# multicom-toolbox/Chromosome3D

Hardware: AMD Instinct MI355X
Metric: SA-steps/sec (replica-steps/s, 20 replicas of chr1_500kb in all: 20 per GPU, weak scaling; regions of 20 steps inside the first 2172 of the schedule's 5172: MD and FIRE steps in front of the final minimisation); wall-clock per chromosome (higher is better)
Workload: dtype f32

## Files before the change

chromosome3d_amd/csrc/c3d_api.cpp:

```cpp
#include <hip/hip_runtime.h>

#include <algorithm>
#include <atomic>
#include <cmath>
#include <cstdio>
#include <cstdlib>
#include <chrono>
#include <cstring>
#include <condition_variable>
#include <map>
#include <mutex>
#include <string>
#include <thread>
#include <tuple>
#include <vector>

#include "../../include/c3d.h"
#include "c3d_host.h"
#include "c3d_internal.h"

using c3d::fail;

namespace {

#define HIP_TRY(expr)                                                                          \
    do {                                                                                       \
        hipError_t e__ = (expr);                                                               \
        if (e__ != hipSuccess)                                                                 \
            return fail(C3D_ERR_HIP, std::string(#expr) + ": " + hipGetErrorString(e__));      \
    } while (0)

template <class T>
struct DevTmp {
    T* p = nullptr;
    ~DevTmp() { if (p) (void)hipFree(p); }
};

struct Op {
    c3d::DevStep p;
    int stage;
    bool counted;
};

struct KernelRecord {
    enum Family { NONE, STEP, LBFGS_EVAL, PAIRS_SYM, STEP64, LBFGS_EVAL64, CLUSTER } family = NONE;
    c3d::StepForm step{};
    c3d::Form64 f64{};
    int pot = 0, rpw = 0, nb = 0, wl = 0;
    bool rs1 = false, late = false, tp = false;
};

inline void philox4x32(const uint32_t ctr_in[4], const uint32_t key_in[2], uint32_t out[4]) {
    uint32_t c[4] = {ctr_in[0], ctr_in[1], ctr_in[2], ctr_in[3]};
    uint32_t k[2] = {key_in[0], key_in[1]};
    for (int r = 0; r < 10; ++r) {
        const uint64_t p0 = (uint64_t)0xD2511F53u * c[0];
        const uint64_t p1 = (uint64_t)0xCD9E8D57u * c[2];
        const uint32_t n0 = (uint32_t)(p1 >> 32) ^ c[1] ^ k[0];
        const uint32_t n1 = (uint32_t)p1;
        const uint32_t n2 = (uint32_t)(p0 >> 32) ^ c[3] ^ k[1];
        const uint32_t n3 = (uint32_t)p0;
        c[0] = n0; c[1] = n1; c[2] = n2; c[3] = n3;
        k[0] += 0x9E3779B9u;
        k[1] += 0xBB67AE85u;
    }
    memcpy(out, c, sizeof(c));
}
inline double u01(uint32_t u) { return ((double)u + 0.5) * (1.0 / 4294967296.0); }
void normals4(uint64_t seed, uint32_t replica, uint32_t bead, uint32_t purpose, double g[4]) {
    const uint32_t ctr[4] = {bead, purpose, 0u, 0u};
    const uint32_t key[2] = {(uint32_t)(seed & 0xFFFFFFFFu) ^ (replica * 0x9E3779B9u), (uint32_t)(seed >> 32) + replica};
    uint32_t r[4];
    philox4x32(ctr, key, r);
    const double two_pi = 6.283185307179586476925286766559;
    double a = sqrt(-2.0 * log(u01(r[0]))), b = two_pi * u01(r[1]);
    g[0] = a * cos(b); g[1] = a * sin(b);
    a = sqrt(-2.0 * log(u01(r[2]))); b = two_pi * u01(r[3]);
    g[2] = a * cos(b); g[3] = a * sin(b);
}

}

struct c3d_ctx {
    int device = 0;
    hipStream_t stream = nullptr;
    static constexpr int kMaxGroups = 4;
    int ngroups = 2;
    hipStream_t gstream[kMaxGroups] = {nullptr, nullptr, nullptr, nullptr};
    hipEvent_t gev[kMaxGroups] = {nullptr, nullptr, nullptr, nullptr};
    hipEvent_t fork_ev = nullptr;
    hipEvent_t ev0 = nullptr, ev1 = nullptr;
    hipEvent_t kev0 = nullptr, kev1 = nullptr;
    int kernel_timing = 0;
    double last_kernel_ms = 0;
    double last_host_launch_us = 0, last_host_sync_us = 0;
    int event_timing = 1;
    bool ev1_recorded = false;

    int n = 0, npad = 0, ntiles = 0, nrep = 0, R = 0;
    c3d_model model;
    std::vector<c3d_stage> stages;
    c3d_fire_params fire;
    float gtol = 0.0f;
    int check_every = 250;
    bool narrow_columns = true;
    bool zero_weight = false;
    bool use_graph = true;
    int rpw = 2;
    int stage_dma = 1;
    int graph_chunk = 256;
    int precision = 32;
    c3d::Buffers64 b64;
    int sym = 0;
    float* d_sym_scratch = nullptr;
    int2* d_sym_tiles = nullptr;
    int start_mode = 0;
    int resident = -1;
    int resident_min_ops = 4;
    double spin_wait_us = 400.0;
    long spin_completions = 0;

    std::vector<int32_t> h_dist10;
    c3d::DevBuffers buf{};
    int eval_rpw = 4;
    bool pair_targets = true;
    bool wide_tiles = true;
    int max_beads = 5120;
    int embed_max_beads = C3D_EMBED_MAX_BEADS_DEFAULT;
    int embed_form = 0;
    int embed_batch = 0;
    int last_embed_form = 0, last_embed_batches = 0;
    int f64_max_beads = C3D_F64_MAX_BEADS_DEFAULT;
    int f64_column_chunk = 0;
    std::vector<int32_t> r_i, r_j, r_t10;
    int column_chunk = 0;
    float* d_feval = nullptr;
    size_t rep_floats = 0;
    bool have_targets = false, have_replicas = false;

    std::vector<Op> program;
    size_t pc = 0;
    int parity = 0;
    long steps_done = 0;
    std::map<std::tuple<long, int, int, int>, hipGraphExec_t> graphs;

    bool inject_timeout = false;
    int resident_fallbacks = 0;
    int resident_skip = 0;
    int resident_backoff = 0;
    int num_cus = 0, num_xcc = 0;
    int cluster_late = -1;
    int cluster_geom = 0;
    int xcd_base = 0, xcd_count = 8;
    bool inject_misplaced = false;
    bool static_place = true;
    int placement_mismatches = 0;
    bool inject_incomplete = false;
    int cluster_incomplete = 0;

    int cluster = -1;
    bool cl_ok = false;
    c3d::ClusterPlan cl_plan{};
    void* d_crec = nullptr;
    size_t crec_bytes = 0;
    static constexpr unsigned kClaimSets = 4096;
    static constexpr unsigned kClaimWords = 16;
    unsigned* d_claim = nullptr;
    unsigned cl_seq = 0;
    c3d::StepRun* d_prog = nullptr;
    size_t prog_cap = 0;
    bool prog_dirty = true;
    std::vector<int> op_run, op_skip;
    std::vector<c3d::StepRun> prog_runs;
    unsigned* h_tmo = nullptr;
    void* h_stage = nullptr;
    void* d_score = nullptr;
    size_t d_score_bytes = 0;
    size_t h_stage_bytes = 0;
    struct IfRanks {
        std::thread worker;
        std::vector<double> matrix, rank;
        size_t m = 0;
        double mean = 0, saa = 0;
        int n = 0, range = 0;
        bool valid = false;
        void join() { if (worker.joinable()) worker.join(); }
        void release() {
            join();
            valid = false;
            std::vector<double>().swap(matrix);
            std::vector<double>().swap(rank);
        }
    } ifr;
    int bb_steps = 1000;
    bool final_bb = true;
    int prefetch_ranks = 1;
    unsigned* h_tmo_dev = nullptr;

    long rank_prefetch_hits = 0;
    int device_ranks = 0;
    long device_rank_runs = 0, score_wide_runs = 0;
    long compare_runs = 0;
    long f64_evals = 0;
    long superpose_runs = 0, rmsd_table_runs = 0;
    long k1_recomputed = 0, k1_patched = 0;
    long graph_captures = 0, graph_launches = 0, step_launches = 0, resident_launches = 0, cluster_launches = 0;
    bool has_two_point = false;
    bool has_lbfgs = false;
    int lbfgs_mem = 5;
    c3d::LbfgsBuffers lb{};
    bool f64_lbfgs = false;
    c3d::LbfgsBuffers64 lb64{};
    long lbfgs_steps = 0;
    int lbfgs_parity = -1;
    int last_path = 0;
    KernelRecord ran;

    double last_ms = 0;
    long last_steps = 0, last_launches = 0;
    uint64_t seed = 82364;
    uint32_t first_rep = 0;
};

namespace {

template <class T>
void dev_free(T*& p) {
    if (!p) return;
    const hipError_t e = hipFree(p);
    if (e != hipSuccess) (void)fail(C3D_ERR_HIP, std::string("hipFree: ") + hipGetErrorString(e));
    p = nullptr;
}

void free_replica_buffers(c3d_ctx* c) {
    for (int k = 0; k < 2; ++k) {
        dev_free(c->buf.X[k]); dev_free(c->buf.V[k]); dev_free(c->buf.P[k]); dev_free(c->buf.S[k]);
    }
    dev_free(c->d_crec);
    c->crec_bytes = 0; c->cl_ok = false;
    dev_free(c->buf.Vinit); dev_free(c->buf.E); dev_free(c->d_feval);
    dev_free(c->d_sym_scratch); dev_free(c->d_sym_tiles);
    dev_free(c->lb.hist); dev_free(c->lb.part); dev_free(c->lb.S[0]); dev_free(c->lb.S[1]);
    dev_free(c->lb64.hist); dev_free(c->lb64.part); dev_free(c->lb64.S[0]); dev_free(c->lb64.S[1]);
    c->lbfgs_parity = -1;
    dev_free(c->b64.T); dev_free(c->b64.t10); dev_free(c->b64.Vinit); dev_free(c->b64.F);
    for (int k = 0; k < 2; ++k) { dev_free(c->b64.X[k]); dev_free(c->b64.V[k]); dev_free(c->b64.P[k]); dev_free(c->b64.S[k]); }
    c->have_replicas = false;
}
void drop_graphs(c3d_ctx* c) {
    for (auto& kv : c->graphs) (void)hipGraphExecDestroy(kv.second);
    c->graphs.clear();
}
void release_context(c3d_ctx* c) {
    for (hipStream_t s : c->gstream) if (s) (void)hipStreamSynchronize(s);
    drop_graphs(c);
    free_replica_buffers(c);
    dev_free(c->buf.tgt); dev_free(c->buf.tgs2);
    dev_free(c->d_prog); dev_free(c->d_claim); dev_free(c->d_score);
    if (c->h_tmo) (void)hipHostFree(c->h_tmo);
    if (c->h_stage) (void)hipHostFree(c->h_stage);
    for (hipEvent_t e : {c->ev0, c->ev1, c->kev0, c->kev1, c->fork_ev}) if (e) (void)hipEventDestroy(e);
    for (hipEvent_t e : c->gev) if (e) (void)hipEventDestroy(e);
    for (hipStream_t s : c->gstream) if (s && s != c->stream) (void)hipStreamDestroy(s);
    if (c->stream) (void)hipStreamDestroy(c->stream);
}

c3d::DevModel dev_model(const c3d_ctx* c) {
    c3d::DevModel m{};
    const c3d_model& h = c->model;
    m.n = c->n; m.npad = c->npad; m.ntiles = c->ntiles; m.nrep = c->nrep;
    m.rep_base = 0; m.nrep_g = c->nrep;
    m.rpw = c->rpw;
    m.stage_dma = c->stage_dma;
    m.noe_pot = h.noe_pot; m.ang_mode = h.ang_mode; m.rep_sep = h.rep_sep;
    m.mexp = h.msoexp == 2 ? 2 : 1;
    m.rs = h.rswitch;
    m.tail_c = h.asym * h.rswitch;
    m.tail_b = (m.tail_c - 2.0f * h.rswitch) * h.rswitch * h.rswitch;
    m.mrs = h.mrswitch; m.nmrs = -h.mrswitch;
    m.inv_rs = 1.0f / h.rswitch; m.nm_rs = -h.mrswitch / h.rswitch;
    if (h.noe_pot == 3 && h.msoexp == 2 && h.masym == 0.0f && m.tail_b == 0.0f && m.tail_c == 2.0f * m.rs) {
        m.noe_pot = 4;
        m.inv_rs = 1.0f / h.mrswitch; m.nm_rs = h.rswitch / h.mrswitch;
    }
    {
        const int cols_last = c->n - (c->npad - 256);
        int wl = cols_last / 64, nleft = cols_last - 64 * wl;
        if (wl == 0 || nleft > 8) { wl = std::min(4, wl + 1); nleft = 0; }
        if (!c->narrow_columns || c->npad > 1024) { wl = 4; nleft = 0; }
        m.wl = wl; m.nleft = nleft; m.jl0 = c->npad - 256 + 64 * wl;
    }
    m.mtail_c = h.masym;
    m.mtail_b = (m.mtail_c - 2.0f * h.mrswitch) * h.mrswitch * h.mrswitch * (m.mexp == 2 ? h.mrswitch : 1.0f);
    m.k_bond2 = 2.0f * h.k_bond; m.b0 = h.b0;
    m.k_ang2 = 2.0f * h.k_ang; m.a0 = h.a0;
    m.acc = c3d::kAccel / h.mass;
    const int ndf = std::max(3 * c->n - 3, 1);
    m.t_fac = h.mass / c3d::kAccel / ((float)ndf * c3d::kBoltz);
    m.fbeta = h.fbeta;
    m.inv_n = 1.0f / (float)c->n;
    return m;
}
c3d::DevFire dev_fire(const c3d_ctx* c) {
    c3d::DevFire f;
    f.dt_start = c->fire.dt_start; f.dt_max = c->fire.dt_max; f.f_inc = c->fire.f_inc; f.f_dec = c->fire.f_dec;
    f.alpha_start = c->fire.alpha_start; f.f_alpha = c->fire.f_alpha; f.max_step = c->fire.max_step;
    f.n_min = c->fire.n_min;
    return f;
}
float clamp_scale(const c3d_ctx* c) { return dev_model(c).noe_pot == 4 ? c->model.mrswitch : c->model.rswitch; }
c3d::DevStep dev_step(const c3d_ctx* c, int kind, float dt, float w_all, float w_vdw, float repel_s, float t_bath) {
    c3d::DevStep p;
    p.kind = kind; p.dt = dt; p.w_all = w_all;
    p.w_noe2n = -2.0f * w_all * c->model.s_noe;
    p.w_rep4 = 4.0f * w_vdw * c->model.k_rep;
    const float rr = repel_s * c->model.r0_rep;
    p.rep_r2 = rr * rr;
    p.inv_rep_r2 = rr > 0.0f ? 1.0f / p.rep_r2 : 0.0f;
    p.w_rep4r2 = p.w_rep4 * p.rep_r2;
    p.w_rs = p.w_noe2n * clamp_scale(c);
    p.kq = p.w_rs != 0.0f ? p.w_rep4r2 / p.w_rs : 0.0f;
    p.t_bath = t_bath;
    return p;
}

bool is_two_point(int kind) { return kind == 5 || kind == 6; }
bool is_lbfgs(int kind) { return kind == 8 || kind == 9; }

void build_program(c3d_ctx* c) {
    c->program.clear();
    int prev_kind = -1;
    for (size_t s = 0; s < c->stages.size(); ++s) {
        const c3d_stage& st = c->stages[s];
        if (st.kind == 2 || st.kind == 5 || st.kind == 8) {
            const bool lbfgs = st.kind == 8;
            const int nbb = (st.kind == 5 && c->final_bb) || lbfgs ? std::min(st.nsteps, c->bb_steps) : 0;
            for (int k = 0; k < st.nsteps; ++k) {
                const int kind = k < nbb ? (k == 0 ? (lbfgs ? 9 : 6) : (lbfgs ? 8 : 5)) : (k == nbb ? 3 : 2);
                c->program.push_back({dev_step(c, kind, 0.0f, st.w_all, st.w_vdw, st.repel_s, 0.0f), (int)s, true});
            }
        } else {
            if (prev_kind == 2 || prev_kind == 5 || prev_kind == 8 || prev_kind == -1)
                c->program.push_back({dev_step(c, 4, 0.0f, st.w_all, st.w_vdw, st.repel_s, st.t_bath), (int)s, false});
            for (int k = 0; k < st.nsteps; ++k)
                c->program.push_back({dev_step(c, st.kind, st.dt, st.w_all, st.w_vdw, st.repel_s, st.t_bath), (int)s, true});
        }
        prev_kind = st.kind;
    }
    c->pc = 0;
    c->zero_weight = false;
    for (const Op& op : c->program) c->zero_weight = c->zero_weight || op.p.w_rs == 0.0f;
    c->has_two_point = false;
    for (const Op& op : c->program) c->has_two_point = c->has_two_point || is_two_point(op.p.kind);
    c->has_lbfgs = false;
    for (const Op& op : c->program) c->has_lbfgs = c->has_lbfgs || is_lbfgs(op.p.kind);
    drop_graphs(c);
    c->prog_runs.clear();
    c->op_run.assign(c->program.size(), 0);
    c->op_skip.assign(c->program.size(), 0);
    for (size_t k = 0; k < c->program.size(); ++k) {
        const c3d::DevStep& p = c->program[k].p;
        if (!c->prog_runs.empty() && memcmp(&c->prog_runs.back().p, &p, sizeof(p)) == 0) ++c->prog_runs.back().count;
        else c->prog_runs.push_back({p, 1});
        c->op_run[k] = (int)c->prog_runs.size() - 1;
        c->op_skip[k] = c->prog_runs.back().count - 1;
    }
    c->prog_dirty = true;
}

enum Stale : unsigned { STALE_REPLICAS = 1, STALE_GRAPHS = 2, STALE_PAIR_TARGETS = 4, STALE_PROGRAM = 8 };
void drop_stale(c3d_ctx* c, unsigned stale) {
    if (stale & STALE_REPLICAS) free_replica_buffers(c);
    if (stale & STALE_PAIR_TARGETS) dev_free(c->buf.tgs2);
    if (stale & STALE_PROGRAM) build_program(c);
    else if (stale & STALE_GRAPHS) drop_graphs(c);
}

int upload_targets(c3d_ctx* c, const std::vector<float>& enc) {
    dev_free(c->buf.tgt); dev_free(c->buf.tgs2);
    HIP_TRY(hipMalloc(&c->buf.tgt, sizeof(float) * enc.size()));
    HIP_TRY(hipMemcpyAsync(c->buf.tgt, enc.data(), sizeof(float) * enc.size(), hipMemcpyHostToDevice, c->stream));
    HIP_TRY(hipStreamSynchronize(c->stream));
    return C3D_OK;
}

void set_dims(c3d_ctx* c, int n) {
    c->n = n;
    c->npad = (n + 255) / 256 * 256;
    c->ntiles = (n + c3d::kTileRows - 1) / c3d::kTileRows;
    c->rep_floats = (size_t)3 * c->npad;
}

void pack(const c3d_ctx* c, const float* aos, std::vector<float>& soa, bool pad_far) {
    soa.assign(c->rep_floats * c->nrep, 0.0f);
    for (int r = 0; r < c->nrep; ++r) {
        float* base = soa.data() + c->rep_floats * r;
        for (int comp = 0; comp < 3; ++comp) {
            for (int i = 0; i < c->n; ++i) base[(size_t)comp * c->npad + i] = aos[((size_t)r * c->n + i) * 3 + comp];
            if (pad_far)
                for (int i = c->n; i < c->npad; ++i) base[(size_t)comp * c->npad + i] = c3d::kPadCoord * (float)(comp + 1) + 16.0f * (float)(i - c->n);
        }
    }
}
void unpack(const c3d_ctx* c, const float* soa, float* aos) {
    for (int r = 0; r < c->nrep; ++r) {
        const float* base = soa + c->rep_floats * r;
        for (int comp = 0; comp < 3; ++comp)
            for (int i = 0; i < c->n; ++i) aos[((size_t)r * c->n + i) * 3 + comp] = base[(size_t)comp * c->npad + i];
    }
}

void group_range(const c3d_ctx* c, int g, int& base, int& count) {
    const int G = std::min(c->ngroups, std::max(c->nrep, 1));
    const int q = c->nrep / G, r = c->nrep % G;
    base = g * q + std::min(g, r);
    count = q + (g < r ? 1 : 0);
}
int active_groups(const c3d_ctx* c) { return std::min(c->ngroups, std::max(c->nrep, 1)); }

enum Unit : unsigned {
    UNIT_DEVICE = 0, UNIT_SCORE, UNIT_CLUSTER_BASE, UNIT_EMBED, UNIT_F64, UNIT_SYM,
    UNIT_CLUSTER_P0, UNIT_CLUSTER_TP0 = UNIT_CLUSTER_P0 + 5, UNIT_COUNT = UNIT_CLUSTER_TP0 + 5
};
constexpr unsigned unit_bit(unsigned u) { return 1u << u; }
constexpr unsigned kUnitsDefault = unit_bit(UNIT_DEVICE) | unit_bit(UNIT_SCORE) | unit_bit(UNIT_CLUSTER_P0 + 4) | unit_bit(UNIT_CLUSTER_TP0 + 4);
constexpr unsigned kUnitsAll = (1u << UNIT_COUNT) - 1u;
constexpr int kMaxDevices = 64;
class LaunchGate {
    std::mutex mu;
    std::condition_variable cv;
    int launching = 0, loads_waiting = 0;
    bool loading = false;
public:
    void lock_shared() {
        std::unique_lock<std::mutex> lk(mu);
        cv.wait(lk, [&] { return !loading && loads_waiting == 0; });
        ++launching;
    }
    void unlock_shared() {
        std::lock_guard<std::mutex> lk(mu);
        if (--launching == 0) cv.notify_all();
    }
    void lock() {
        std::unique_lock<std::mutex> lk(mu);
        ++loads_waiting;
        cv.wait(lk, [&] { return !loading && launching == 0; });
        --loads_waiting;
        loading = true;
    }
    void unlock() {
        std::lock_guard<std::mutex> lk(mu);
        loading = false;
        cv.notify_all();
    }
};
struct Units {
    LaunchGate rw;
    std::atomic<unsigned> loaded[kMaxDevices];
    std::atomic<long> loads{0};
    Units() { for (auto& a : loaded) a.store(0); }
};
Units g_units;
thread_local int t_entry_depth = 0;

const char* unit_name(unsigned u) {
    static const char* const names[] = {"per-step + K1", "scoring", "multi-step planner", "embedding", "fp64", "symmetric tiles"};
    if (u < UNIT_CLUSTER_P0) return names[u];
    return u < UNIT_CLUSTER_TP0 ? "multi-step (k_cluster)" : "multi-step (k_cluster_tp)";
}
hipError_t load_one_unit(unsigned u) {
    switch (u) {
        case UNIT_DEVICE: return c3d::preload_device_unit();
        case UNIT_SCORE: return c3d::preload_score_unit();
        case UNIT_CLUSTER_BASE: return c3d::preload_cluster_base_unit();
        case UNIT_EMBED: return c3d::preload_embed_unit();
        case UNIT_F64: return c3d::preload_f64_unit();
        case UNIT_SYM: return c3d::preload_sym_unit();
        default: break;
    }
    if (u >= UNIT_CLUSTER_TP0 && u < UNIT_COUNT) return c3d::preload_cluster_unit((int)(u - UNIT_CLUSTER_TP0), true);
    if (u >= UNIT_CLUSTER_P0 && u < UNIT_CLUSTER_TP0) return c3d::preload_cluster_unit((int)(u - UNIT_CLUSTER_P0), false);
    return hipErrorInvalidValue;
}
int ensure_units(int device, unsigned mask) {
    if (device < 0 || device >= kMaxDevices) return fail(C3D_ERR_INVALID, "device index beyond the 64 this build keeps code-object state for");
    mask &= kUnitsAll;
    if ((g_units.loaded[device].load(std::memory_order_acquire) & mask) == mask) return C3D_OK;
    if (t_entry_depth > 0) return fail(C3D_ERR_HIP, "internal: a code object is wanted inside an entry that did not name it");
    std::lock_guard<LaunchGate> lk(g_units.rw);
    HIP_TRY(hipSetDevice(device));
    for (unsigned u = 0; u < UNIT_COUNT; ++u) {
        if (!(mask & unit_bit(u)) || (g_units.loaded[device].load(std::memory_order_relaxed) & unit_bit(u))) continue;
        const hipError_t e = load_one_unit(u);
        if (e != hipSuccess) return fail(C3D_ERR_HIP, std::string("loading the code object of the ") + unit_name(u) + " kernels: " + hipGetErrorString(e));
        g_units.loaded[device].fetch_or(unit_bit(u), std::memory_order_release);
        g_units.loads.fetch_add(1);
    }
    return C3D_OK;
}
unsigned units_wanted(const c3d_ctx* c) {
    unsigned m = unit_bit(UNIT_DEVICE) | unit_bit(UNIT_SCORE);
    const int pot = std::min(std::max(dev_model(c).noe_pot, 0), 4);
    if (c->cluster != 0 && c->resident != 0 && c->precision != 64)
        m |= unit_bit(UNIT_CLUSTER_P0 + (unsigned)pot) | unit_bit(UNIT_CLUSTER_TP0 + (unsigned)pot);
    if (c->precision == 64) m |= unit_bit(UNIT_F64);
    if (c->sym > 0) m |= unit_bit(UNIT_SYM);
    return m;
}
struct Entry {
    int rc = C3D_OK;
    bool locked = false;
    Entry(const c3d_ctx* c, unsigned extra, bool launches) {
        if (hipSetDevice(c->device) != hipSuccess) { rc = fail(C3D_ERR_HIP, "hipSetDevice failed"); return; }
        if (launches) rc = ensure_units(c->device, units_wanted(c) | extra);
        if (rc != C3D_OK) return;
        if (t_entry_depth++ == 0) { g_units.rw.lock_shared(); locked = true; }
    }
    ~Entry() {
        if (rc != C3D_OK) return;
        --t_entry_depth;
        if (locked) g_units.rw.unlock_shared();
    }
    Entry(const Entry&) = delete;
    Entry& operator=(const Entry&) = delete;
};
#define C3D_ENTRY(c, extra)                 \
    Entry entry__((c), (extra), true);      \
    if (entry__.rc != C3D_OK) return entry__.rc
#define C3D_GATE(c)                         \
    Entry entry__((c), 0u, false);          \
    if (entry__.rc != C3D_OK) return entry__.rc

int drop_stale_gated(c3d_ctx* c, unsigned stale) {
    const bool device_side = ((stale & STALE_REPLICAS) && (c->buf.X[0] || c->b64.t10)) || ((stale & STALE_PAIR_TARGETS) && c->buf.tgs2) ||
                             ((stale & (STALE_GRAPHS | STALE_PROGRAM)) && !c->graphs.empty());
    if (!device_side) { drop_stale(c, stale); return C3D_OK; }
    C3D_GATE(c);
    drop_stale(c, stale);
    return C3D_OK;
}

bool use_sym(const c3d_ctx* c) {
    return c->sym > 0 && c->d_sym_scratch && !c3d::general_tail(dev_model(c));
}

void model_host64(const c3d_ctx* c, double (&mh)[15]) {
    const c3d_model& h = c->model;
    const double v[15] = {h.s_noe, h.rswitch, h.asym, h.masym, h.mrswitch, h.k_bond, h.b0, h.k_ang, h.a0, h.r0_rep, h.k_rep, h.mass, h.fbeta,
                          (double)h.min_sep, (double)h.msoexp};
    for (int k = 0; k < 15; ++k) mh[k] = v[k];
}
int build_targets64(c3d_ctx* c) {
    double mh[15];
    model_host64(c, mh);
    hipError_t e = c3d::launch_targets64(dev_model(c), mh, c->model.min_sep, c->b64.t10, c->b64.T, c->stream);
    if (e != hipSuccess) return fail(C3D_ERR_HIP, std::string("fp64 targets: ") + hipGetErrorString(e));
    HIP_TRY(hipStreamSynchronize(c->stream));
    return C3D_OK;
}


int ensure_lbfgs(c3d_ctx* c) {
    if (c->lb.hist) return C3D_OK;
    const size_t hist = c3d::lbfgs_hist_floats(c->npad) * c->nrep, part = (size_t)c->nrep * c->ntiles * c3d::kLbfgsQ;
    HIP_TRY(hipMalloc(&c->lb.hist, sizeof(float) * hist));
    HIP_TRY(hipMalloc(&c->lb.part, sizeof(float) * part));
    for (int k = 0; k < 2; ++k) HIP_TRY(hipMalloc(&c->lb.S[k], sizeof(c3d::LbfgsState) * c->nrep));
    HIP_TRY(hipMemsetAsync(c->lb.hist, 0, sizeof(float) * hist, c->stream));
    HIP_TRY(hipMemsetAsync(c->lb.part, 0, sizeof(float) * part, c->stream));
    for (int k = 0; k < 2; ++k) HIP_TRY(hipMemsetAsync(c->lb.S[k], 0, sizeof(c3d::LbfgsState) * c->nrep, c->stream));
    HIP_TRY(hipStreamSynchronize(c->stream));
    return C3D_OK;
}

int ensure_lbfgs64(c3d_ctx* c) {
    if (c->lb64.hist) return C3D_OK;
    const size_t hist = c3d::lbfgs_hist_floats(c3d::cols64(c->n)) * c->nrep, part = (size_t)c->nrep * c->ntiles * c3d::kLbfgsQ;
    HIP_TRY(hipMalloc(&c->lb64.hist, sizeof(double) * hist));
    HIP_TRY(hipMalloc(&c->lb64.part, sizeof(double) * part));
    for (int k = 0; k < 2; ++k) HIP_TRY(hipMalloc(&c->lb64.S[k], sizeof(c3d::LbfgsState) * c->nrep));
    HIP_TRY(hipMemsetAsync(c->lb64.hist, 0, sizeof(double) * hist, c->stream));
    HIP_TRY(hipMemsetAsync(c->lb64.part, 0, sizeof(double) * part, c->stream));
    for (int k = 0; k < 2; ++k) HIP_TRY(hipMemsetAsync(c->lb64.S[k], 0, sizeof(c3d::LbfgsState) * c->nrep, c->stream));
    HIP_TRY(hipStreamSynchronize(c->stream));
    return C3D_OK;
}

int ensure_pair_targets(c3d_ctx* c, const c3d::DevModel& m) {
    if (c->buf.tgs2 || !c->pair_targets || !c3d::pair_targets_fit(m) || c->npad <= 1024 || !c->buf.tgt) return C3D_OK;
    HIP_TRY(hipMalloc(&c->buf.tgs2, sizeof(float) * c3d::pair_targets_floats(c->n, c->npad)));
    hipError_t e = c3d::launch_pair_targets(m, c->buf.tgt, c->buf.tgs2, c->stream);
    if (e != hipSuccess) return fail(C3D_ERR_HIP, std::string("pair targets: ") + hipGetErrorString(e));
    HIP_TRY(hipStreamSynchronize(c->stream));
    return C3D_OK;
}
KernelRecord op_kernel(const c3d_ctx* c, const c3d::DevModel& m, const Op& op) {
    KernelRecord k;
    if (c->precision == 64) {
        double mh[15];
        model_host64(c, mh);
        k.family = is_lbfgs(op.p.kind) ? KernelRecord::LBFGS_EVAL64 : KernelRecord::STEP64;
        k.f64 = c3d::form64(m.noe_pot, mh, c->stages[op.stage].w_all, c->n, c->f64_column_chunk);
    } else if (!is_lbfgs(op.p.kind) && use_sym(c)) {
        k.family = KernelRecord::PAIRS_SYM;
        k.pot = c3d::device_pot(m.noe_pot);
        k.rs1 = c3d::sym_rs1(m);
    } else {
        k.family = is_lbfgs(op.p.kind) ? KernelRecord::LBFGS_EVAL : KernelRecord::STEP;
        k.step = c3d::step_form(m, op.p, c->wide_tiles, c->pair_targets, c->buf.tgs2 != nullptr, c->column_chunk);
    }
    return k;
}
int launch_op(c3d_ctx* c, const Op& op, int g, int par) {
    c3d::DevModel m = dev_model(c);
    group_range(c, g, m.rep_base, m.nrep_g);
    if (c->precision == 64) {
        const c3d_stage& st = c->stages[op.stage];
        double mh[15];
        model_host64(c, mh);
        const double fh[7] = {c->fire.dt_start, c->fire.dt_max, c->fire.f_inc, c->fire.f_dec, c->fire.alpha_start, c->fire.f_alpha, c->fire.max_step};
        const double sh[6] = {(double)op.p.kind, st.dt, st.w_all, st.w_vdw, st.repel_s, st.t_bath};
        if (is_lbfgs(op.p.kind)) {
            hipError_t e = c3d::launch_lbfgs_eval64(m, mh, sh, c->b64, c->lb64, par, c->lbfgs_mem, c->f64_column_chunk, c->gstream[g]);
            if (e == hipSuccess) e = c3d::launch_lbfgs_move64(m, mh, sh, fh, c->fire.n_min, c->b64, c->lb64, par, c->lbfgs_mem, c->gstream[g]);
            if (e != hipSuccess) return fail(C3D_ERR_HIP, std::string("fp64 L-BFGS step launch: ") + hipGetErrorString(e));
            return C3D_OK;
        }
        hipError_t e64 = c3d::launch_step64(m, mh, sh, fh, c->fire.n_min, c->b64, par, c->f64_column_chunk, c->gstream[g]);
        if (e64 != hipSuccess) return fail(C3D_ERR_HIP, std::string("fp64 step launch: ") + hipGetErrorString(e64));
        return C3D_OK;
    }
    const KernelRecord k = op_kernel(c, m, op);
    if (k.family == KernelRecord::LBFGS_EVAL) {
        hipError_t e = c3d::launch_lbfgs_eval(m, op.p, c->buf, c->lb, par, c->lbfgs_mem, k.step, c->gstream[g]);
        if (e == hipSuccess) e = c3d::launch_lbfgs_move(m, op.p, dev_fire(c), c->buf, c->lb, par, c->lbfgs_mem, c->gstream[g]);
        if (e != hipSuccess) return fail(C3D_ERR_HIP, std::string("L-BFGS step launch: ") + hipGetErrorString(e));
        return C3D_OK;
    }
    hipError_t e = k.family == KernelRecord::PAIRS_SYM
                       ? c3d::launch_step_sym(m, op.p, dev_fire(c), c->buf, par, c->d_sym_tiles, c->d_sym_scratch, c->gstream[g])
                       : c3d::launch_step(m, op.p, dev_fire(c), c->buf, par, k.step, c->gstream[g]);
    if (e != hipSuccess) return fail(C3D_ERR_HIP, std::string("step launch: ") + hipGetErrorString(e));
    return C3D_OK;
}

int plan_cluster(c3d_ctx* c) {
    c3d::DevModel m = dev_model(c);
    m.nrep = c->nrep; m.nrep_g = c->nrep; m.rep_base = 0;
    c->cl_ok = false;
    if (!c3d::cluster_plan(m, c->num_cus, c->num_xcc, c->cluster_geom, c->cluster_late, c->xcd_count, &c->cl_plan)) return C3D_OK;
    c->cl_plan.device = c->device;
    const size_t bytes = c3d::cluster_record_bytes(m, c->cl_plan);
    if (!c->d_crec || bytes > c->crec_bytes) {
        if (c->d_crec) { HIP_TRY(hipStreamSynchronize(c->stream)); dev_free(c->d_crec); }
        c->crec_bytes = 0;
        HIP_TRY(hipMalloc(&c->d_crec, bytes));
        c->crec_bytes = bytes;
    }
    c->cl_seq = 0;
    c->cl_ok = true;
    return C3D_OK;
}

bool cluster_ok(c3d_ctx* c) {
    if (!c->resident || !c->cluster || !c->cl_ok || !c->d_crec) return false;
    return !c3d::general_tail(dev_model(c));
}

bool launch_was_abandoned(c3d_ctx* c, unsigned done_mark) {
    if (c->h_tmo[2]) { c->h_tmo[2] = 0; c->static_place = false; ++c->placement_mismatches; }
    const bool complete = c->h_tmo[1] == done_mark;
    if (!*c->h_tmo && complete) { c->resident_backoff = 0; return false; }
    if (!*c->h_tmo) ++c->cluster_incomplete;
    *c->h_tmo = 0;
    c->resident_backoff = std::min(4096, std::max(4, 2 * c->resident_backoff));
    c->resident_skip = c->resident_backoff;
    ++c->resident_fallbacks;
    return true;
}
void account_ops(c3d_ctx* c, size_t nops) {
    c->parity ^= 1;
    for (size_t k = 0; k < nops; ++k)
        if (c->program[c->pc + k].counted) { ++c->steps_done; ++c->last_steps; }
    c->last_launches += 1;
    c->pc += nops;
}


int run_cluster(c3d_ctx* c, size_t nops, bool* ran) {
    if (c->prog_dirty) {
        if (c->prog_runs.size() > c->prog_cap) {
            if (c->d_prog) { HIP_TRY(hipStreamSynchronize(c->stream)); dev_free(c->d_prog); }
            c->prog_cap = std::max<size_t>(c->prog_runs.size(), 256);
            HIP_TRY(hipMalloc(&c->d_prog, sizeof(c3d::StepRun) * c->prog_cap));
        }
        HIP_TRY(hipMemcpyAsync(c->d_prog, c->prog_runs.data(), sizeof(c3d::StepRun) * c->prog_runs.size(), hipMemcpyHostToDevice, c->stream));
        HIP_TRY(hipStreamSynchronize(c->stream));
        c->prog_dirty = false;
    }
    const unsigned seq = c->cl_seq % c3d_ctx::kClaimSets;
    if (seq == 0) {
        HIP_TRY(hipMemsetAsync(c->d_crec, 0, c->crec_bytes, c->stream));
        HIP_TRY(hipMemsetAsync(c->d_claim, 0, sizeof(unsigned) * c3d_ctx::kClaimWords * c3d_ctx::kClaimSets, c->stream));
    }
    ++c->cl_seq;
    if (c->inject_timeout) { *c->h_tmo = 1; c->inject_timeout = false; }
    c->h_tmo[1] = 0;
    const c3d::DevModel m = dev_model(c);
    c3d::ClusterPlan pl = c->cl_plan;
    if (c->inject_incomplete) { ++pl.expected; c->inject_incomplete = false; }
    if (c->kernel_timing) { pl.t0 = c->kev0; pl.t1 = c->kev1; }
    pl.static_place = c->static_place ? (c->inject_misplaced ? 2 : 1) : 0;
    pl.xcd_base = c->xcd_base;
    pl.two_point = false;
    for (size_t k = 0; k < nops && !pl.two_point; ++k) pl.two_point = is_two_point(c->program[c->pc + k].p.kind);
    c->inject_misplaced = false;
    c->h_tmo[2] = 0;
    const auto h0 = std::chrono::steady_clock::now();
    hipError_t e = c3d::launch_cluster(m, dev_fire(c), pl, c3d::anneal_io(c->buf, c->parity), c->buf.tgt, c->d_crec, c->d_prog,
                                       c->op_run[c->pc], c->op_skip[c->pc], (int)nops, seq << 20, c->h_tmo_dev,
                                       c->d_claim + c3d_ctx::kClaimWords * seq, c->stream);
    if (e != hipSuccess) return fail(C3D_ERR_HIP, std::string("cluster launch: ") + hipGetErrorString(e));
    if (c->event_timing) HIP_TRY(hipEventRecord(c->ev1, c->stream));
    const auto h1 = std::chrono::steady_clock::now();
    bool marked = false;
    if (c->spin_wait_us > 0 && !c->kernel_timing) {
        const unsigned mark = (seq << 20) | 1u;
        for (;;) {
            if (__atomic_load_n(&c->h_tmo[1], __ATOMIC_ACQUIRE) == mark) { marked = true; break; }
            if (__atomic_load_n(&c->h_tmo[0], __ATOMIC_RELAXED) || __atomic_load_n(&c->h_tmo[2], __ATOMIC_RELAXED)) break;
            if (std::chrono::duration<double, std::micro>(std::chrono::steady_clock::now() - h1).count() > c->spin_wait_us) break;
            __builtin_ia32_pause();
        }
    }
    if (!marked) HIP_TRY(hipStreamSynchronize(c->stream));
    else ++c->spin_completions;
    const auto h2 = std::chrono::steady_clock::now();
    c->last_host_launch_us += std::chrono::duration<double, std::micro>(h1 - h0).count();
    c->last_host_sync_us += std::chrono::duration<double, std::micro>(h2 - h1).count();
    c->ev1_recorded = true;
    ++c->cluster_launches;
    if (c->kernel_timing) {
        float kms = 0;
        HIP_TRY(hipEventElapsedTime(&kms, c->kev0, c->kev1));
        c->last_kernel_ms += kms;
    }
    if (launch_was_abandoned(c, (seq << 20) | 1u)) { *ran = false; c->ev1_recorded = false; return C3D_OK; }
    *ran = true;
    c->last_path = 2;
    KernelRecord& k = c->ran;
    k = KernelRecord();
    k.family = KernelRecord::CLUSTER;
    k.pot = c3d::device_pot(m.noe_pot); k.rpw = pl.rpw; k.nb = m.npad / 256; k.wl = m.wl; k.late = pl.late_tiles != 0; k.tp = pl.two_point;
    account_ops(c, nops);
    return C3D_OK;
}

int run_ops_segment(c3d_ctx* c, size_t nops, bool zero_w, bool lbfgs = false);

int run_ops(c3d_ctx* c, size_t nops) {
    const bool p64 = c->precision == 64;
    if (p64 ? !c->has_lbfgs : (!c->zero_weight && !c->has_two_point && !c->has_lbfgs)) return run_ops_segment(c, nops, false);
    const size_t end = c->pc + nops;
    while (c->pc < end) {
        const c3d::DevStep& p0 = c->program[c->pc].p;
        const bool z = !p64 && p0.w_rs == 0.0f, tp = !p64 && is_two_point(p0.kind), lb = is_lbfgs(p0.kind);
        size_t k = 1;
        while (c->pc + k < end) {
            const c3d::DevStep& p = c->program[c->pc + k].p;
            if ((!p64 && p.w_rs == 0.0f) != z || (!p64 && is_two_point(p.kind)) != tp || is_lbfgs(p.kind) != lb) break;
            ++k;
        }
        const int rc = run_ops_segment(c, k, z, lb);
        if (rc) return rc;
    }
    return C3D_OK;
}

int ensure_group_streams(c3d_ctx* c, int G) {
    for (int g = 1; g < G && g < c3d_ctx::kMaxGroups; ++g) {
        if (c->gstream[g]) continue;
        HIP_TRY(hipStreamCreateWithFlags(&c->gstream[g], hipStreamNonBlocking));
        HIP_TRY(hipEventCreateWithFlags(&c->gev[g], hipEventDisableTiming));
    }
    return C3D_OK;
}

int run_ops_segment(c3d_ctx* c, size_t nops, bool zero_w, bool lbfgs) {
    if (nops == 0) return C3D_OK;
    if (c->precision == 64 || zero_w || lbfgs) { }
    else if (c->resident_skip > 0 && c->resident < 1) --c->resident_skip;
    else if (nops >= (size_t)c->resident_min_ops && nops < ((size_t)1 << 20)) {
        bool ran = false;
        int rc = C3D_OK;
        if (cluster_ok(c)) rc = run_cluster(c, nops, &ran);
        if (rc != C3D_OK || ran) return rc;
    }
    c->last_path = 0;
    c->ev1_recorded = false;
    if (c->precision != 64 && (!use_sym(c) || lbfgs)) {
        if (int rc = ensure_pair_targets(c, dev_model(c))) return rc;
    }
    if (lbfgs)
        if (int rc = c->precision == 64 ? ensure_lbfgs64(c) : ensure_lbfgs(c)) return rc;
    const int G = active_groups(c);
    if (int rc = ensure_group_streams(c, G)) return rc;
    if (G > 1) {
        HIP_TRY(hipEventRecord(c->fork_ev, c->stream));
        for (int g = 1; g < G; ++g) HIP_TRY(hipStreamWaitEvent(c->gstream[g], c->fork_ev, 0));
    }
    size_t done = 0;
    while (done < nops) {
        const size_t chunk = std::min<size_t>(nops - done, c->use_graph ? (size_t)c->graph_chunk : nops - done);
        if (!c->use_graph || chunk < 4) {
            for (int g = 0; g < G; ++g) {
                int par = c->parity;
                for (size_t k = 0; k < chunk; ++k) {
                    int rc = launch_op(c, c->program[c->pc + k], g, par);
                    if (rc) return rc;
                    par ^= 1;
                }
            }
        } else {
            const Op& first = c->program[c->pc];
            const Op& last = c->program[c->pc + chunk - 1];
            long sig = (long)c->pc;
            if ((first.p.kind == 2 || first.p.kind == 5 || first.p.kind == 8) && last.p.kind == first.p.kind && first.stage == last.stage)
                sig = -(long)(first.stage + 1) - (first.p.kind == 5 ? 1000000L : first.p.kind == 8 ? 2000000L : 0L);
            if (c->graphs.size() >= 2048) {
                for (int g = 0; g < G; ++g) HIP_TRY(hipStreamSynchronize(c->gstream[g]));
                drop_graphs(c);
            }
            for (int g = 0; g < G; ++g) {
                const auto key = std::make_tuple(sig, (int)chunk, c->parity, g);
                auto it = c->graphs.find(key);
                if (it == c->graphs.end()) {
                    hipGraph_t gr = nullptr;
                    HIP_TRY(hipStreamBeginCapture(c->gstream[g], hipStreamCaptureModeThreadLocal));
                    int par = c->parity;
                    int rc = C3D_OK;
                    for (size_t k = 0; k < chunk && rc == C3D_OK; ++k) { rc = launch_op(c, c->program[c->pc + k], g, par); par ^= 1; }
                    hipError_t ce = hipStreamEndCapture(c->gstream[g], &gr);
                    if (rc) { if (gr) (void)hipGraphDestroy(gr); return rc; }
                    if (ce != hipSuccess) return fail(C3D_ERR_HIP, std::string("hipStreamEndCapture: ") + hipGetErrorString(ce));
                    hipGraphExec_t ge = nullptr;
                    hipError_t ie = hipGraphInstantiate(&ge, gr, nullptr, nullptr, 0);
                    (void)hipGraphDestroy(gr);
                    if (ie != hipSuccess) return fail(C3D_ERR_HIP, std::string("hipGraphInstantiate: ") + hipGetErrorString(ie));
                    it = c->graphs.emplace(key, ge).first;
                    ++c->graph_captures;
                }
                HIP_TRY(hipGraphLaunch(it->second, c->gstream[g]));
                ++c->graph_launches;
            }
        }
        c->step_launches += (long)chunk * G;
        if (lbfgs) { c->lbfgs_steps += (long)chunk; c->lbfgs_parity = c->parity ^ (int)(chunk & 1); }
        if (chunk & 1) c->parity ^= 1;
        for (size_t k = 0; k < chunk; ++k)
            if (c->program[c->pc + k].counted) { ++c->steps_done; ++c->last_steps; }
        c->last_launches += (long)chunk;
        c->pc += chunk;
        done += chunk;
    }
    for (int g = 1; g < G; ++g) {
        HIP_TRY(hipEventRecord(c->gev[g], c->gstream[g]));
        HIP_TRY(hipStreamWaitEvent(c->stream, c->gev[g], 0));
    }
    if (c->precision == 64) {
        hipError_t e = c3d::launch_export64(dev_model(c), c->b64, c->parity, c->buf.X[c->parity], c->buf.V[c->parity], c->buf.P[c->parity], c->stream);
        if (e != hipSuccess) return fail(C3D_ERR_HIP, std::string("fp64 export: ") + hipGetErrorString(e));
        c->last_path = 3;
// ... 42 lines not shown
    const float* h = static_cast<const float*>(c->h_stage);
    double worst = 0;
    for (int r = 0; r < c->nrep; ++r) {
        double ff = 0;
        for (int t = 0; t < nparts; ++t) ff += h[((size_t)r * nparts + t) * 4 + 1];
        const double rms = sqrt(ff / (3.0 * c->n));
        if (!(rms <= worst)) worst = rms;
    }
    *out = worst;
    return C3D_OK;
}

int partials_finite(c3d_ctx* c, bool* ok) {
    const size_t cnt = (size_t)c->nrep * c->ntiles * 4;
    if (int rc = read_back(c, c->buf.P[c->parity], sizeof(float) * cnt)) return rc;
    const float* h = static_cast<const float*>(c->h_stage);
    *ok = true;
    for (size_t k = 0; k < cnt; ++k) if (!std::isfinite(h[k])) { *ok = false; break; }
    return C3D_OK;
}

int import64(c3d_ctx* c) {
    hipError_t e = c3d::launch_import64(dev_model(c), c->buf.X[c->parity], c->b64, c->stream);
    if (e != hipSuccess) return fail(C3D_ERR_HIP, std::string("fp64 import: ") + hipGetErrorString(e));
    HIP_TRY(hipStreamSynchronize(c->stream));
    return C3D_OK;
}

}

extern "C" int c3d_device_count(void) {
    int n = 0;
    if (hipGetDeviceCount(&n) != hipSuccess) return 0;
    return n;
}

extern "C" void c3d_default_model(c3d_model* m) {
    if (!m) return;
    m->min_sep = 5; m->noe_pot = 3; m->rep_sep = 2; m->ang_mode = 1;
    m->s_noe = 10.0f; m->rswitch = 0.5f; m->asym = 2.0f;
    m->k_bond = 500.0f; m->b0 = 3.93f;
    m->k_ang = 15.0f; m->a0 = 5.55f;
    m->r0_rep = 5.25f; m->k_rep = 4.0f;
    m->mass = 100.0f; m->fbeta = 10.0f;
    m->mrswitch = 10.0f; m->masym = 0.0f; m->msoexp = 2;
}
extern "C" void c3d_default_fire(c3d_fire_params* f) {
    if (!f) return;
    f->dt_start = 0.002f; f->dt_max = 0.02f; f->f_inc = 1.1f; f->f_dec = 0.5f;
    f->alpha_start = 0.1f; f->f_alpha = 0.99f; f->max_step = 0.5f; f->n_min = 5;
}
extern "C" int c3d_default_schedule(c3d_stage* st, int cap, int min_steps) {
    std::vector<c3d_stage> v;
    v.push_back({2, 200, 0.0f, 1.0f, 20.0f, 0.5f, 0.0f});
    const float hot_t = 2000.0f, hot_dt = 0.003f;
    const int hot_n[5] = {125, 125, 125, 500, 125};
    const float hot_w[5] = {0.1f, 0.2f, 0.2f, 0.4f, 1.0f};
    const float hot_v[5] = {20.0f, 20.0f, 0.01f, 0.003f, 0.003f};
    const float hot_r[5] = {0.5f, 0.5f, 0.9f, 0.9f, 0.9f};
    for (int k = 0; k < 5; ++k) v.push_back({0, hot_n[k], hot_dt, hot_w[k], hot_v[k], hot_r[k], hot_t});
    const int ncycle = (int)(hot_t / 25.0f);
    const int nstep = 1000 / ncycle;
    const double vdw_step = pow(4.0 / 0.003, 1.0 / ncycle);
    const double rad_step = (1.0 - 0.85) / ncycle;
    double radius = 1.0, kv = 0.003, bath = hot_t;
    for (int i = 0; i <= ncycle; ++i) {
        v.push_back({1, nstep, 0.005f, 1.0f, (float)kv, (float)radius, (float)bath});
        radius = std::max(0.85, radius - rad_step);
        kv = std::min(4.0, kv * vdw_step);
        bath -= 25.0;
    }
    v.push_back({5, min_steps, 0.0f, 1.0f, 1.0f, 0.85f, 0.0f});
    if (st) for (int k = 0; k < (int)v.size() && k < cap; ++k) st[k] = v[k];
    return (int)v.size();
}

static std::atomic<int> g_preload{1};

extern "C" int c3d_set_process_option(const char* key, double value) {
    if (!key) return fail(C3D_ERR_INVALID, "c3d_set_process_option: null key");
    if (!strcmp(key, "preload")) {
        if (value != 0 && value != 1 && value != 2) return fail(C3D_ERR_INVALID, "c3d_set_process_option: preload is 0, 1 or 2");
        g_preload.store((int)value);
        return C3D_OK;
    }
    return fail(C3D_ERR_INVALID, std::string("c3d_set_process_option: unknown key ") + key);
}

extern "C" int c3d_create(int device, c3d_ctx** out) {
    if (!out) return fail(C3D_ERR_INVALID, "c3d_create: null out");
    int ndev = 0;
    if (hipGetDeviceCount(&ndev) != hipSuccess || ndev < 1)
        return fail(C3D_ERR_NO_DEVICE, "no HIP device visible: libc3d has no CPU fallback");
    if (device < 0 || device >= ndev) return fail(C3D_ERR_INVALID, "c3d_create: device index out of range");
    HIP_TRY(hipSetDevice(device));
    hipDeviceProp_t prop;
    HIP_TRY(hipGetDeviceProperties(&prop, device));
    if (strncmp(prop.gcnArchName, "gfx950", 6) != 0)
        return fail(C3D_ERR_NO_DEVICE, std::string("device is ") + prop.gcnArchName + ", libc3d is built for gfx950 only");
    int num_xcc = 0;
    if (hipDeviceGetAttribute(&num_xcc, hipDeviceAttributeNumberOfXccs, device) != hipSuccess) num_xcc = 0;
    if (const int pre = g_preload.load())
        if (const int rc = ensure_units(device, pre >= 2 ? kUnitsAll : kUnitsDefault)) return rc;
    c3d_ctx* c = new c3d_ctx();
    c->device = device;
    c->num_cus = prop.multiProcessorCount;
    c->num_xcc = num_xcc;
    c3d_default_model(&c->model);
    c3d_default_fire(&c->fire);
    c->stages.resize(c3d_default_schedule(nullptr, 0, 3000));
    c3d_default_schedule(c->stages.data(), (int)c->stages.size(), 3000);
    Entry gate(c, 0u, false);
    if (gate.rc != C3D_OK) { delete c; return gate.rc; }
    bool ok = hipStreamCreateWithFlags(&c->stream, hipStreamNonBlocking) == hipSuccess &&
              hipEventCreate(&c->ev0) == hipSuccess && hipEventCreate(&c->ev1) == hipSuccess &&
              hipEventCreate(&c->kev0) == hipSuccess && hipEventCreate(&c->kev1) == hipSuccess &&
              hipEventCreateWithFlags(&c->fork_ev, hipEventDisableTiming) == hipSuccess;
    c->gstream[0] = c->stream;
    ok = ok && hipHostMalloc(reinterpret_cast<void**>(&c->h_tmo), 64, hipHostMallocMapped) == hipSuccess;
    if (ok) {
        *c->h_tmo = 0;
        ok = hipHostGetDevicePointer(reinterpret_cast<void**>(&c->h_tmo_dev), c->h_tmo, 0) == hipSuccess &&
             hipMalloc(&c->d_claim, sizeof(unsigned) * c3d_ctx::kClaimWords * c3d_ctx::kClaimSets) == hipSuccess;
        c->h_tmo[1] = 0;
    }
    if (!ok) {
        c3d_destroy(c);
        return fail(C3D_ERR_HIP, "cannot create HIP stream/events");
    }
    *out = c;
    return C3D_OK;
}

extern "C" void c3d_destroy(c3d_ctx* c) {
    if (!c) return;
    c->ifr.release();
    {
        Entry gate(c, 0u, false);
        release_context(c);
    }
    delete c;
}

extern "C" int c3d_set_model(c3d_ctx* c, const c3d_model* m) {
    if (!c || !m) return fail(C3D_ERR_INVALID, "c3d_set_model: null argument");
    const int msoexp = m->msoexp == 0 ? 2 : m->msoexp;
    if (m->mass <= 0 || m->rswitch <= 0 || m->min_sep < 1 || m->rep_sep < 1 || m->rep_sep > 3 || m->noe_pot < 0 || m->noe_pot > 3 || m->mrswitch <= 0 || (msoexp != 1 && msoexp != 2))
        return fail(C3D_ERR_INVALID, "c3d_set_model: parameter out of range");
    if (c->have_targets && m->min_sep != c->model.min_sep)
        return fail(C3D_ERR_INVALID, "c3d_set_model: min_sep must be set before the targets are built");
    const bool targets64 = c->precision == 64 && c->b64.T;
    Entry entry(c, 0u, targets64);
    if (entry.rc != C3D_OK) return entry.rc;
    c->model = *m;
    c->model.msoexp = msoexp;
    drop_stale(c, STALE_PAIR_TARGETS | STALE_PROGRAM);
    if (c->have_replicas)
        if (int rc = plan_cluster(c)) return rc;
    return targets64 ? build_targets64(c) : C3D_OK;
}

extern "C" int c3d_set_schedule(c3d_ctx* c, const c3d_stage* st, int n_stages, const c3d_fire_params* fire, float gtol,
                                int check_every) {
    if (!c || !st || n_stages < 1) return fail(C3D_ERR_INVALID, "c3d_set_schedule: bad arguments");
    for (int k = 0; k < n_stages; ++k) {
        if (st[k].kind < 0 || (st[k].kind > 2 && st[k].kind != 5 && st[k].kind != 8) || st[k].nsteps < 0) return fail(C3D_ERR_INVALID, "c3d_set_schedule: bad stage");
        if (st[k].kind == 8 && c->precision == 64 && !c->f64_lbfgs)
            return fail(C3D_ERR_INVALID, "c3d_set_schedule: a stage of kind 8 (L-BFGS) has no fp64 form; set precision 32 first");
    }
    c->stages.assign(st, st + n_stages);
    if (fire) c->fire = *fire;
    c->gtol = gtol;
    if (check_every > 0) c->check_every = check_every;
    return drop_stale_gated(c, STALE_PROGRAM);
}

extern "C" int c3d_set_option(c3d_ctx* c, const char* key, double value) {
    if (!c || !key) return fail(C3D_ERR_INVALID, "c3d_set_option: null argument");
    unsigned stale = 0;
    if (!strcmp(key, "use_graph")) c->use_graph = value != 0;
    else if (!strcmp(key, "rows_per_wave")) {
        if (value != 1 && value != 2 && value != 4) return fail(C3D_ERR_INVALID, "rows_per_wave must be 1, 2 or 4");
        c->rpw = (int)value;
        stale = STALE_GRAPHS;
    } else if (!strcmp(key, "replica_groups")) {
        if (value < 1 || value > c3d_ctx::kMaxGroups) return fail(C3D_ERR_INVALID, "replica_groups must be 1..4");
        c->ngroups = (int)value;
        stale = STALE_GRAPHS;
    } else if (!strcmp(key, "event_timing")) c->event_timing = value != 0;
    else if (!strcmp(key, "kernel_timing")) c->kernel_timing = value != 0;
    else if (!strcmp(key, "resident")) { c->resident = value < 0 ? -1 : (value != 0); c->resident_skip = 0; }
    else if (!strcmp(key, "precision")) {
        if (value != 32 && value != 64) return fail(C3D_ERR_INVALID, "precision must be 32 or 64");
        if (value == 64 && !c->f64_lbfgs)
            for (const c3d_stage& st : c->stages)
                if (st.kind == 8) return fail(C3D_ERR_INVALID, "precision 64: the schedule holds a stage of kind 8 (L-BFGS), which has no fp64 form");
        c->precision = (int)value;
        stale = STALE_REPLICAS | STALE_GRAPHS;
    } else if (!strcmp(key, "eval_rows_per_wave")) {
        if (value != 2 && value != 4 && value != -2) return fail(C3D_ERR_INVALID, "eval_rows_per_wave must be 4, 2 (packed pair term) or -2 (two rows per wave, scalar pair term)");
        c->eval_rpw = (int)value;
    } else if (!strcmp(key, "pair_targets")) { c->pair_targets = value != 0; stale = STALE_PAIR_TARGETS | STALE_GRAPHS; }
    else if (!strcmp(key, "wide_tiles")) { c->wide_tiles = value != 0; stale = STALE_GRAPHS; }
    else if (!strcmp(key, "symmetric")) { c->sym = value > 0; stale = STALE_REPLICAS | STALE_GRAPHS; }
    else if (!strcmp(key, "start")) {
        if (value != 0 && value != 1) return fail(C3D_ERR_INVALID, "start must be 0 (random coil) or 1 (extended strand)");
        c->start_mode = (int)value;
    } else if (!strcmp(key, "cluster")) c->cluster = value < 0 ? -1 : (value != 0);
    else if (!strcmp(key, "resident_inject_timeout")) c->inject_timeout = value != 0;
    else if (!strcmp(key, "narrow_columns")) { c->narrow_columns = value != 0; stale = STALE_REPLICAS | STALE_GRAPHS; }
    else if (!strcmp(key, "cluster_static_placement")) { c->static_place = value != 0; c->inject_misplaced = value == 2; }
    else if (!strcmp(key, "cluster_inject_incomplete")) c->inject_incomplete = value != 0;
    else if (!strcmp(key, "cluster_num_xcc")) { c->num_xcc = (int)value; stale = STALE_REPLICAS; }
    else if (!strcmp(key, "prefetch_ranks")) c->prefetch_ranks = value != 0;
    else if (!strcmp(key, "device_ranks")) {
        if (value != -1 && value != 0 && value != 1)
            return fail(C3D_ERR_INVALID, "device_ranks is 0 (the device beyond 5120 beads), 1 (the device for every symmetric matrix) or -1 (the host)");
        c->device_ranks = (int)value;
    }
    else if (!strcmp(key, "final_minimiser_steps")) {
        if (value < 2) return fail(C3D_ERR_INVALID, "c3d_set_option: final_minimiser_steps >= 2");
        c->bb_steps = (int)value;
        stale = STALE_PROGRAM;
    } else if (!strcmp(key, "final_minimiser")) {
        if (value != 0 && value != 1) return fail(C3D_ERR_INVALID, "c3d_set_option: final_minimiser is 0 (FIRE) or 1 (two-point step size)");
        c->final_bb = value != 0;
        stale = STALE_PROGRAM;
    } else if (!strcmp(key, "lbfgs_memory")) {
        if (value != (int)value || value < 1 || value > c3d::kLbfgsMaxPairs) return fail(C3D_ERR_INVALID, "c3d_set_option: lbfgs_memory is 1..8");
        c->lbfgs_mem = (int)value;
        stale = STALE_GRAPHS;
    } else if (!strcmp(key, "cluster_xcd_count")) {
        const int v = (int)value;
        if (v < 1 || v > 8 || c->xcd_base + v > 8) return fail(C3D_ERR_INVALID, "cluster_xcd_count: 1..8, and cluster_xcd_base + cluster_xcd_count <= 8");
        c->xcd_count = v;
        stale = STALE_REPLICAS;
    } else if (!strcmp(key, "cluster_xcd_base")) {
        const int v = (int)value;
        if (v < 0 || v + c->xcd_count > 8) return fail(C3D_ERR_INVALID, "cluster_xcd_base: 0 .. 8 - cluster_xcd_count");
        c->xcd_base = v;
    } else if (!strcmp(key, "cluster_late_tiles")) { c->cluster_late = value != 0 ? -1 : 0; stale = STALE_REPLICAS; }
    else if (!strcmp(key, "cluster_geometry")) {
        if (value < 0 || value > 1699) return fail(C3D_ERR_INVALID, "cluster_geometry = 100 compute waves + 10 rows per wave + helper waves");
        c->cluster_geom = (int)value;
        stale = STALE_REPLICAS;
    } else if (!strcmp(key, "spin_wait_us")) c->spin_wait_us = value < 0 ? 0 : value;
    else if (!strcmp(key, "resident_min_ops")) c->resident_min_ops = value < 1 ? 1 : (int)value;
    else if (!strcmp(key, "stage_dma")) { c->stage_dma = value != 0; stale = STALE_GRAPHS; }
    else if (!strcmp(key, "max_beads")) {
        if (value != (int)value || value < C3D_MAX_BEADS_DEFAULT || value > C3D_MAX_BEADS_LIMIT)
            return fail(C3D_ERR_INVALID, "max_beads must be an integer from 5120 to 16384");
        c->max_beads = (int)value;
    } else if (!strcmp(key, "embed_max_beads")) {
        if (value != (int)value || value < C3D_EMBED_MAX_BEADS_DEFAULT || value > C3D_EMBED_MAX_BEADS_LIMIT)
            return fail(C3D_ERR_INVALID, "embed_max_beads must be an integer from 4549 to 16384");
        c->embed_max_beads = (int)value;
    } else if (!strcmp(key, "f64_max_beads")) {
        if (value != (int)value || value < C3D_F64_MAX_BEADS_DEFAULT || value > C3D_F64_MAX_BEADS_LIMIT)
            return fail(C3D_ERR_INVALID, "f64_max_beads must be an integer from 2560 to 16384");
        c->f64_max_beads = (int)value;
    } else if (!strcmp(key, "f64_lbfgs")) {
        if (value != 0 && value != 1) return fail(C3D_ERR_INVALID, "f64_lbfgs must be 0 or 1");
        if (value == 0 && c->precision == 64)
            for (const c3d_stage& st : c->stages)
                if (st.kind == 8) return fail(C3D_ERR_INVALID, "f64_lbfgs: precision is 64 and the schedule holds a stage of kind 8 (L-BFGS); change one of them first");
        c->f64_lbfgs = value != 0;
    } else if (!strcmp(key, "f64_column_chunk")) {
        if (value != (int)value || (value != 0 && !c3d::column_chunk64_valid((int)value)))
            return fail(C3D_ERR_INVALID, "f64_column_chunk must be 0 (by size), 256, 512 or 1024");
        c->f64_column_chunk = (int)value;
        stale = STALE_GRAPHS;
    } else if (!strcmp(key, "embed_form")) {
        if (value != 0 && value != 1) return fail(C3D_ERR_INVALID, "embed_form is 0 (k_dg_eig while it fits, tiled beyond) or 1 (tiled)");
        c->embed_form = (int)value;
    } else if (!strcmp(key, "embed_batch")) {
        if (value != (int)value || value < 0) return fail(C3D_ERR_INVALID, "embed_batch is 0 (by the scratch budget) or a number of replicas");
        c->embed_batch = (int)value;
    } else if (!strcmp(key, "column_chunk")) {
        if (value != (int)value || (value != 0 && !c3d::column_chunk_valid((int)value)))
            return fail(C3D_ERR_INVALID, "column_chunk must be 0 (the library's choice), 256, 1024 or 2048");
        c->column_chunk = (int)value;
        stale = STALE_GRAPHS;
    }
    else if (!strcmp(key, "graph_chunk")) {
        if (value < 8) return fail(C3D_ERR_INVALID, "graph_chunk must be >= 8");
        c->graph_chunk = (int)value & ~1;
        stale = STALE_GRAPHS;
    } else return fail(C3D_ERR_INVALID, std::string("unknown option ") + key);
    return drop_stale_gated(c, stale);
}

static constexpr int kDefaultMaxBeads = C3D_MAX_BEADS_DEFAULT;
static constexpr int kMaxBeadsLimit = C3D_MAX_BEADS_LIMIT;
static_assert(kDefaultMaxBeads == c3d::kMaxStagedCols, "the default limit is the staged form's");
static int too_many_beads(const c3d_ctx* c, const char* fn, int n) {
    char b[192];
    if (c->max_beads == kDefaultMaxBeads)
        snprintf(b, sizeof b, "%s: %d beads: more than %d are accepted only after c3d_set_option(\"max_beads\", n) (up to %d)", fn, n,
                 kDefaultMaxBeads, kMaxBeadsLimit);
    else
        snprintf(b, sizeof b, "%s: %d beads: more than max_beads = %d (the option goes up to %d)", fn, n, c->max_beads, kMaxBeadsLimit);
    return fail(C3D_ERR_INVALID, b);
}
static constexpr int kRankPrefetchBeads = 2048;

extern "C" int c3d_set_if_matrix(c3d_ctx* c, const double* IF, int n, double alpha, double K) {
    if (!c || !IF || n < 2) return fail(C3D_ERR_INVALID, "c3d_set_if_matrix: bad arguments");
    if (n > c->max_beads) return too_many_beads(c, "c3d_set_if_matrix", n);
    C3D_ENTRY(c, 0u);
    free_replica_buffers(c);
    set_dims(c, n);
    const size_t nn = (size_t)n * n;
    c->ifr.join();
    c->ifr.valid = false;
    if (c->prefetch_ranks && n <= kRankPrefetchBeads) {
        try {
            c->ifr.matrix.assign(IF, IF + nn);
            c->ifr.n = n; c->ifr.range = 3;
            c3d_ctx::IfRanks* const w = &c->ifr;
            c->ifr.worker = std::thread([w] {
                try { c3d::if_pair_ranks(w->matrix.data(), w->n, w->range, w->rank, w->m, w->mean, w->saa); w->valid = true; }
                catch (...) { w->valid = false; }
            });
        } catch (...) { c->ifr.release(); }
    } else {
        c->ifr.release();
    }
    DevTmp<double> dIF, dP, dpart;
    DevTmp<int32_t> ddist;
    DevTmp<unsigned char> dflags;
    DevTmp<unsigned> dnflag;
    const int npartial = 64;
    dev_free(c->buf.tgt); dev_free(c->buf.tgs2);
    c->have_targets = false;
    HIP_TRY(hipMalloc(&dIF.p, sizeof(double) * nn));
    HIP_TRY(hipMalloc(&dP.p, sizeof(double) * nn));
    HIP_TRY(hipMalloc(&dpart.p, sizeof(double) * npartial));
    HIP_TRY(hipMalloc(&ddist.p, sizeof(int32_t) * nn));
    HIP_TRY(hipMalloc(&dflags.p, nn));
    HIP_TRY(hipMalloc(&dnflag.p, sizeof(unsigned)));
    HIP_TRY(hipMalloc(&c->buf.tgt, sizeof(float) * (size_t)n * c->npad));
    HIP_TRY(hipMemcpyAsync(dIF.p, IF, sizeof(double) * nn, hipMemcpyHostToDevice, c->stream));
    HIP_TRY(hipMemsetAsync(dnflag.p, 0, sizeof(unsigned), c->stream));
    HIP_TRY(hipMemsetAsync(dflags.p, 0, nn, c->stream));
    hipError_t e = c3d::launch_if_to_target(dIF.p, n, c->npad, alpha, K, c->model.min_sep, c->model.rep_sep, dP.p, dpart.p,
                                            npartial, ddist.p, c->buf.tgt, dflags.p, dnflag.p, c->stream);
    if (e != hipSuccess) return fail(C3D_ERR_HIP, std::string("K1 launch: ") + hipGetErrorString(e));
    c->h_dist10.resize(nn);
    c->r_i.clear(); c->r_j.clear(); c->r_t10.clear();
    unsigned nflag = 0;
    HIP_TRY(hipMemcpyAsync(c->h_dist10.data(), ddist.p, sizeof(int32_t) * nn, hipMemcpyDeviceToHost, c->stream));
    HIP_TRY(hipMemcpyAsync(&nflag, dnflag.p, sizeof(unsigned), hipMemcpyDeviceToHost, c->stream));
    HIP_TRY(hipStreamSynchronize(c->stream));
    c->k1_recomputed = 0;
    if (nflag) {
        std::vector<unsigned char> flags(nn);
        HIP_TRY(hipMemcpyAsync(flags.data(), dflags.p, nn, hipMemcpyDeviceToHost, c->stream));
        HIP_TRY(hipStreamSynchronize(c->stream));
        double sum = 0.0;
        for (size_t k = 0; k < nn; ++k) sum += pow(IF[k], alpha);
        const double mean = sum / ((double)n * (double)n);
        for (size_t k = 0; k < nn; ++k) {
            if (!flags[k]) continue;
            double v = pow(IF[k], alpha) / mean;
            if (v == 0) continue;
            v = K / v;
            char b[64];
            snprintf(b, sizeof b, "%.1f", v);
            char* dot = strchr(b, '.');
            long long t = atoll(b) * 10 + (dot ? dot[1] - '0' : 0);
            if (t > 2000000000LL) t = 2000000000LL;
            ++c->k1_recomputed;
            if ((int32_t)t == c->h_dist10[k]) continue;
            c->h_dist10[k] = (int32_t)t;
            const int i = (int)(k / n), j = (int)(k % n);
            const int sep = i > j ? i - j : j - i;
            const float enc = (sep >= c->model.min_sep && t > 0) ? (float)((double)t / 10.0) : 0.0f;
            HIP_TRY(hipMemcpyAsync(c->buf.tgt + (size_t)i * c->npad + j, &enc, sizeof(float), hipMemcpyHostToDevice, c->stream));
            HIP_TRY(hipStreamSynchronize(c->stream));
            dev_free(c->buf.tgs2);
            ++c->k1_patched;
        }
    }
    int R = 0;
    for (int i = 0; i < n; ++i)
        for (int j = i + 1; j < n; ++j)
            if (j - i >= c->model.min_sep && c->h_dist10[(size_t)i * n + j] > 0) ++R;
    c->R = R;
    c->have_targets = true;
    build_program(c);
    return C3D_OK;
}

extern "C" int c3d_set_restraints(c3d_ctx* c, int n, int R, const int32_t* ri, const int32_t* rj, const int32_t* rt10) {
    if (!c || n < 2 || R < 0 || (R > 0 && (!ri || !rj || !rt10))) return fail(C3D_ERR_INVALID, "c3d_set_restraints: bad arguments");
    if (n > c->max_beads) return too_many_beads(c, "c3d_set_restraints", n);
    C3D_ENTRY(c, 0u);
    free_replica_buffers(c);
    c->ifr.release();
    set_dims(c, n);
    std::vector<float> enc((size_t)n * c->npad);
    std::fill(enc.begin(), enc.end(), 0.0f);
    for (int k = 0; k < R; ++k) {
        const int i = ri[k] - 1, j = rj[k] - 1;
        if (i < 0 || j < 0 || i >= n || j >= n || i == j) return fail(C3D_ERR_INVALID, "c3d_set_restraints: index out of range");
        if (rt10[k] <= 0) continue;
        const float t = (float)((double)rt10[k] / 10.0);
        enc[(size_t)i * c->npad + j] = c3d::encode_target_host(t);
        enc[(size_t)j * c->npad + i] = c3d::encode_target_host(t);
    }
    int rc = upload_targets(c, enc);
    if (rc) return rc;
    c->h_dist10.clear();
    {
        std::vector<std::pair<uint64_t, int>> key;
        key.reserve(R);
        for (int k = 0; k < R; ++k) {
            const int i = std::min(ri[k], rj[k]) - 1, j = std::max(ri[k], rj[k]) - 1;
            key.emplace_back((uint64_t)i * n + j, k);
        }
        std::sort(key.begin(), key.end());
        c->r_i.clear(); c->r_j.clear(); c->r_t10.clear();
        int32_t last = 0;
        for (size_t q = 0; q < key.size(); ++q) {
            if (rt10[key[q].second] > 0) last = rt10[key[q].second];
            if (q + 1 < key.size() && key[q + 1].first == key[q].first) continue;
            if (last > 0) { c->r_i.push_back((int32_t)(key[q].first / n)); c->r_j.push_back((int32_t)(key[q].first % n)); c->r_t10.push_back(last); }
            last = 0;
        }
    }
    c->R = R;
    c->have_targets = true;
    build_program(c);
    return C3D_OK;
}

extern "C" int c3d_get_dist10(c3d_ctx* c, int32_t* out) {
    if (!c || !out) return fail(C3D_ERR_INVALID, "c3d_get_dist10: null argument");
    if (c->h_dist10.empty()) return fail(C3D_ERR_INVALID, "c3d_get_dist10: targets were not built from an IF matrix");
    memcpy(out, c->h_dist10.data(), sizeof(int32_t) * c->h_dist10.size());
    return C3D_OK;
}
extern "C" int c3d_num_beads(const c3d_ctx* c) { return c ? c->n : 0; }
extern "C" int c3d_num_restraints(const c3d_ctx* c) { return c ? c->R : 0; }

extern "C" int c3d_init_replicas(c3d_ctx* c, int nrep, uint64_t seed, uint32_t first_replica) {
    if (!c || nrep < 1) return fail(C3D_ERR_INVALID, "c3d_init_replicas: bad arguments");
    if (!c->have_targets) return fail(C3D_ERR_INVALID, "c3d_init_replicas: set the IF matrix / restraints first");
    if (c->sym > 0 && c->npad > c3d::kMaxStagedCols && c->precision != 64)
        return fail(C3D_ERR_INVALID, "c3d_init_replicas: symmetric tiles stage a replica in LDS and take at most 5120 beads; set symmetric 0");
    if (c->precision == 64) {
        if (c->h_dist10.empty() && c->r_t10.empty())
            return fail(C3D_ERR_INVALID, "precision 64 needs targets built from an IF matrix (integer tenths)");
        if (c->n > c->f64_max_beads) {
            if (c->f64_max_beads == C3D_F64_MAX_BEADS_DEFAULT)
                return fail(C3D_ERR_INVALID, "precision 64: more than 2560 beads are accepted only after c3d_set_option(\"f64_max_beads\", n) (up to " +
                                                 std::to_string(C3D_F64_MAX_BEADS_LIMIT) + ")");
            return fail(C3D_ERR_INVALID, "precision 64: " + std::to_string(c->n) + " beads: more than f64_max_beads = " +
                                             std::to_string(c->f64_max_beads) + " (the option goes up to " + std::to_string(C3D_F64_MAX_BEADS_LIMIT) + ")");
        }
    }
    C3D_ENTRY(c, 0u);
    if (c->have_replicas && nrep != c->nrep) free_replica_buffers(c);
    c->nrep = nrep; c->seed = seed; c->first_rep = first_replica;
    const size_t nf = c->rep_floats * nrep;
    if (!c->have_replicas) {
        drop_graphs(c);
        for (int k = 0; k < 2; ++k) {
            HIP_TRY(hipMalloc(&c->buf.X[k], sizeof(float) * nf));
            HIP_TRY(hipMalloc(&c->buf.V[k], sizeof(float) * nf));
            HIP_TRY(hipMalloc(&c->buf.P[k], sizeof(float) * 4 * (size_t)nrep * c->ntiles * c3d::kTileRows));
            HIP_TRY(hipMalloc(&c->buf.S[k], sizeof(c3d::FireState) * nrep));
        }
        HIP_TRY(hipMalloc(&c->buf.Vinit, sizeof(float) * nf));
        HIP_TRY(hipMalloc(&c->buf.E, sizeof(double) * 4 * nrep));
        HIP_TRY(hipMalloc(&c->d_feval, sizeof(float) * nf));
        {
            c3d::DevModel m = dev_model(c);
            m.nrep = nrep; m.nrep_g = nrep; m.rep_base = 0;
            if (c->sym > 0) {
                int Q, G, od, dg;
                c3d::sym_geometry(m, &Q, &G, &od, &dg);
                std::vector<int2> tl((size_t)od + dg);
                c3d::sym_tile_list(m, tl.data());
                HIP_TRY(hipMalloc(&c->d_sym_tiles, sizeof(int2) * tl.size()));
                HIP_TRY(hipMemcpyAsync(c->d_sym_tiles, tl.data(), sizeof(int2) * tl.size(), hipMemcpyHostToDevice, c->stream));
                HIP_TRY(hipStreamSynchronize(c->stream));
                HIP_TRY(hipMalloc(&c->d_sym_scratch, sizeof(float) * c3d::sym_scratch_floats(m)));
            }
            if (int rc = plan_cluster(c)) return rc;
        }
        c->have_replicas = true;
    }
    const int n = c->n;
    std::vector<float> x((size_t)nrep * n * 3), v((size_t)nrep * n * 3);
    std::vector<double> v64(c->precision == 64 ? (size_t)nrep * n * 3 : 0);
    const double sigma = sqrt((double)c3d::kBoltz * 0.5 * (double)c3d::kAccel / (double)c->model.mass);
    for (int r = 0; r < nrep; ++r) {
        const uint32_t rid = first_replica + (uint32_t)r;
        std::vector<double> xd((size_t)3 * n);
        double px = 0, py = 0, pz = 0;
        for (int i = 0; i < n; ++i) {
            if (c->start_mode == 1) {
                const uint32_t ctr[4] = {(uint32_t)i, 2u, 0u, 0u};
                const uint32_t key[2] = {(uint32_t)(seed & 0xFFFFFFFFu) ^ (rid * 0x9E3779B9u), (uint32_t)(seed >> 32) + rid};
                uint32_t u[4];
                philox4x32(ctr, key, u);
                xd[3 * i] = (double)c->model.b0 * i; xd[3 * i + 1] = 0.5 * u01(u[0]); xd[3 * i + 2] = 0.5 * u01(u[1]);
                continue;
            }
            if (i > 0) {
                double g[4];
                normals4(seed, rid, (uint32_t)i, 0u, g);
                double nrm = sqrt(g[0] * g[0] + g[1] * g[1] + g[2] * g[2]);
                if (nrm < 1e-12) { g[0] = 1; g[1] = g[2] = 0; nrm = 1; }
                px += (double)c->model.b0 * g[0] / nrm; py += (double)c->model.b0 * g[1] / nrm; pz += (double)c->model.b0 * g[2] / nrm;
            }
            xd[3 * i] = px; xd[3 * i + 1] = py; xd[3 * i + 2] = pz;
        }
        double cx = 0, cy = 0, cz = 0;
        for (int i = 0; i < n; ++i) { cx += xd[3 * i]; cy += xd[3 * i + 1]; cz += xd[3 * i + 2]; }
        cx /= n; cy /= n; cz /= n;
        for (int i = 0; i < n; ++i) {
            x[((size_t)r * n + i) * 3 + 0] = (float)(xd[3 * i] - cx);
            x[((size_t)r * n + i) * 3 + 1] = (float)(xd[3 * i + 1] - cy);
            x[((size_t)r * n + i) * 3 + 2] = (float)(xd[3 * i + 2] - cz);
            double g[4];
            normals4(seed, rid, (uint32_t)i, 1u, g);
            v[((size_t)r * n + i) * 3 + 0] = (float)(sigma * g[0]);
            v[((size_t)r * n + i) * 3 + 1] = (float)(sigma * g[1]);
            v[((size_t)r * n + i) * 3 + 2] = (float)(sigma * g[2]);
            if (!v64.empty()) for (int k = 0; k < 3; ++k) v64[((size_t)r * n + i) * 3 + k] = sigma * g[k];
        }
// ... 161 lines not shown
static int need_f64_state(const c3d_ctx* c, const char* fn) {
    if (!c) return fail(C3D_ERR_INVALID, std::string(fn) + ": null context");
    if (c->precision != 64)
        return fail(C3D_ERR_INVALID, std::string(fn) + ": the context holds no fp64 state: its precision is 32 (set precision 64 before c3d_init_replicas)");
    if (!c->have_replicas || !c->b64.X[0])
        return fail(C3D_ERR_INVALID, std::string(fn) + ": the context holds no fp64 state yet: call c3d_init_replicas first");
    return C3D_OK;
}
static int get_soa64(c3d_ctx* c, const double* dev, double* aos) {
    const int n = c->n, np = c3d::cols64(n);
    if (int rc = read_back(c, dev, sizeof(double) * (size_t)c->nrep * 3 * np)) return rc;
    const double* h = static_cast<const double*>(c->h_stage);
    for (int r = 0; r < c->nrep; ++r)
        for (int comp = 0; comp < 3; ++comp) {
            const double* src = h + ((size_t)r * 3 + comp) * np;
            for (int i = 0; i < n; ++i) aos[((size_t)r * n + i) * 3 + comp] = src[i];
        }
    return C3D_OK;
}
extern "C" int c3d_get_coords_f64(c3d_ctx* c, double* xyz) {
    if (int rc = need_f64_state(c, "c3d_get_coords_f64")) return rc;
    if (!xyz) return fail(C3D_ERR_INVALID, "c3d_get_coords_f64: null buffer");
    C3D_ENTRY(c, unit_bit(UNIT_F64));
    return get_soa64(c, c->b64.X[c->parity], xyz);
}
extern "C" int c3d_get_velocities_f64(c3d_ctx* c, double* v) {
    if (int rc = need_f64_state(c, "c3d_get_velocities_f64")) return rc;
    if (!v) return fail(C3D_ERR_INVALID, "c3d_get_velocities_f64: null buffer");
    C3D_ENTRY(c, unit_bit(UNIT_F64));
    return get_soa64(c, c->b64.V[c->parity], v);
}
extern "C" int c3d_set_coords_f64(c3d_ctx* c, const double* xyz) {
    if (int rc = need_f64_state(c, "c3d_set_coords_f64")) return rc;
    if (!xyz) return fail(C3D_ERR_INVALID, "c3d_set_coords_f64: null buffer");
    const int n = c->n, np = c3d::cols64(n);
    const size_t cnt = (size_t)c->nrep * n * 3, n3 = (size_t)c->nrep * 3 * np;
    for (size_t k = 0; k < cnt; ++k)
        if (!std::isfinite(xyz[k])) return fail(C3D_ERR_INVALID, "c3d_set_coords_f64: non-finite coordinate; nothing was copied");
    C3D_ENTRY(c, unit_bit(UNIT_F64));
    HIP_TRY(hipStreamSynchronize(c->stream));
    if (int rc = ensure_stage(c, sizeof(double) * n3)) return rc;
    double* h = static_cast<double*>(c->h_stage);
    for (int r = 0; r < c->nrep; ++r)
        for (int comp = 0; comp < 3; ++comp) {
            double* dst = h + ((size_t)r * 3 + comp) * np;
            for (int i = 0; i < n; ++i) dst[i] = xyz[((size_t)r * n + i) * 3 + comp];
            for (int i = n; i < np; ++i) dst[i] = (double)c3d::kPadCoord * (comp + 1) + 16.0 * (i - n);
        }
    for (int k = 0; k < 2; ++k) {
        HIP_TRY(hipMemcpyAsync(c->b64.X[k], h, sizeof(double) * n3, hipMemcpyHostToDevice, c->stream));
        HIP_TRY(hipMemsetAsync(c->b64.V[k], 0, sizeof(double) * n3, c->stream));
    }
    hipError_t e = c3d::launch_export64(dev_model(c), c->b64, c->parity, c->buf.X[c->parity], c->buf.V[c->parity], c->buf.P[c->parity], c->stream);
    if (e != hipSuccess) return fail(C3D_ERR_HIP, std::string("fp64 export: ") + hipGetErrorString(e));
    HIP_TRY(hipStreamSynchronize(c->stream));
    return C3D_OK;
}

extern "C" long c3d_schedule_length(const c3d_ctx* c) {
    if (!c) return 0;
    long n = 0;
    for (const Op& op : c->program) n += op.counted;
    return n;
}
extern "C" long c3d_steps_done(const c3d_ctx* c) { return c ? c->steps_done : 0; }

extern "C" int c3d_run_steps(c3d_ctx* c, long nsteps, long* done) {
    if (!c || nsteps < 0) return fail(C3D_ERR_INVALID, "c3d_run_steps: bad arguments");
    if (!c->have_replicas) return fail(C3D_ERR_INVALID, "c3d_run_steps: call c3d_init_replicas first");
    C3D_ENTRY(c, 0u);
    size_t nops = 0;
    long counted = 0;
    while (c->pc + nops < c->program.size() && counted < nsteps) {
        counted += c->program[c->pc + nops].counted;
        ++nops;
    }
    int rc = begin_timing(c);
    if (rc) return rc;
    rc = run_ops(c, nops);
    if (rc) return rc;
    rc = end_timing(c);
    if (rc) return rc;
    if (done) *done = counted;
    return C3D_OK;
}

extern "C" int c3d_centre(c3d_ctx* c) {
    if (!c || !c->have_replicas) return fail(C3D_ERR_INVALID, "c3d_centre: bad state");
    C3D_ENTRY(c, 0u);
    hipError_t e = c3d::launch_centre(dev_model(c), c->buf, c->parity, c->stream);
    if (e != hipSuccess) return fail(C3D_ERR_HIP, std::string("centre launch: ") + hipGetErrorString(e));
    HIP_TRY(hipStreamSynchronize(c->stream));
    return C3D_OK;
}

extern "C" int c3d_run(c3d_ctx* c) {
    if (!c) return fail(C3D_ERR_INVALID, "c3d_run: null context");
    if (!c->have_replicas) return fail(C3D_ERR_INVALID, "c3d_run: call c3d_init_replicas first");
    C3D_ENTRY(c, 0u);
    int rc = begin_timing(c);
    if (rc) return rc;
    const int last_stage = (int)c->stages.size() - 1;
    const bool early = c->gtol > 0.0f && last_stage >= 0 && (c->stages[last_stage].kind == 2 || c->stages[last_stage].kind == 5 || c->stages[last_stage].kind == 8);
    size_t nfixed = c->program.size() - c->pc;
    if (early) {
        nfixed = 0;
        while (c->pc + nfixed < c->program.size() && c->program[c->pc + nfixed].stage != last_stage) ++nfixed;
    }
    rc = run_ops(c, nfixed);
    if (rc) return rc;
    if (early) {
        while (c->pc < c->program.size()) {
            const size_t chunk = std::min<size_t>((size_t)(c->check_every & ~1), c->program.size() - c->pc);
            rc = run_ops(c, chunk);
            if (rc) return rc;
            double rms = 0;
            rc = max_rms_force(c, &rms);
            if (rc) return rc;
            if (rms < c->gtol) break;
        }
        c->pc = c->program.size();
    }
    hipError_t e = c3d::launch_centre(dev_model(c), c->buf, c->parity, c->stream);
    if (e != hipSuccess) return fail(C3D_ERR_HIP, std::string("centre launch: ") + hipGetErrorString(e));
    c->ev1_recorded = false;
    rc = end_timing(c);
    if (rc) return rc;
    bool finite = true;
    rc = partials_finite(c, &finite);
    if (rc) return rc;
    if (!finite) return fail(C3D_ERR_DIVERGED, "c3d_run: the trajectory diverged (non-finite forces); reduce the time step or stiffness");
    return C3D_OK;
}

extern "C" int c3d_last_timing(const c3d_ctx* c, double* ms_total, long* steps, long* launches) {
    if (!c) return fail(C3D_ERR_INVALID, "c3d_last_timing: null context");
    if (ms_total) *ms_total = c->last_ms;
    if (steps) *steps = c->last_steps;
    if (launches) *launches = c->last_launches;
    return C3D_OK;
}

extern "C" int c3d_get_stat(const c3d_ctx* c, const char* key, double* value) {
    if (!c || !key || !value) return fail(C3D_ERR_INVALID, "c3d_get_stat: null argument");
    if (!strcmp(key, "graph_captures")) *value = (double)c->graph_captures;
    else if (!strcmp(key, "last_kernel_us")) *value = 1e3 * c->last_kernel_ms;
    else if (!strcmp(key, "last_host_launch_us")) *value = c->last_host_launch_us;
    else if (!strcmp(key, "last_host_sync_us")) *value = c->last_host_sync_us;
    else if (!strcmp(key, "graph_launches")) *value = (double)c->graph_launches;
    else if (!strcmp(key, "graphs_cached")) *value = (double)c->graphs.size();
    else if (!strcmp(key, "step_launches")) *value = (double)c->step_launches;
    else if (!strcmp(key, "resident_launches")) *value = (double)c->resident_launches;
    else if (!strcmp(key, "cluster_launches")) *value = (double)c->cluster_launches;
    else if (!strcmp(key, "resident_fallbacks")) *value = (double)c->resident_fallbacks;
    else if (!strcmp(key, "cluster_incomplete")) *value = (double)c->cluster_incomplete;
    else if (!strcmp(key, "spin_completions")) *value = (double)c->spin_completions;
    else if (!strcmp(key, "cluster_static_placement")) *value = c->static_place ? 1.0 : 0.0;
    else if (!strcmp(key, "cluster_placement_mismatches")) *value = (double)c->placement_mismatches;
    else if (!strcmp(key, "num_xcc")) *value = (double)c->num_xcc;
    else if (!strcmp(key, "rms_force")) {
        double rms = 0;
        if (!c->have_replicas) return fail(C3D_ERR_INVALID, "c3d_get_stat: rms_force needs replicas");
        C3D_ENTRY(c, 0u);
        const int rc = max_rms_force(const_cast<c3d_ctx*>(c), &rms);
        if (rc) return rc;
        *value = rms;
    }
    else if (!strcmp(key, "lbfgs_steps")) *value = (double)c->lbfgs_steps;
    else if (!strcmp(key, "lbfgs_resets")) {
        *value = 0;
        const c3d::LbfgsState* dev = c->lbfgs_parity < 0 ? nullptr : c->precision == 64 ? c->lb64.S[c->lbfgs_parity] : c->lb.S[c->lbfgs_parity];
        if (dev) {
            C3D_ENTRY(c, 0u);
            if (int rc = read_back(const_cast<c3d_ctx*>(c), dev, sizeof(c3d::LbfgsState) * c->nrep)) return rc;
            const c3d::LbfgsState* h = static_cast<const c3d::LbfgsState*>(c->h_stage);
            long r = 0;
            for (int k = 0; k < c->nrep; ++k) r += h[k].resets;
            *value = (double)r;
        }
    }
    else if (!strcmp(key, "k1_recomputed")) *value = (double)c->k1_recomputed;
    else if (!strcmp(key, "k1_patched")) *value = (double)c->k1_patched;
    else if (!strcmp(key, "last_path")) *value = (double)c->last_path;
    else if (!strcmp(key, "rank_prefetch_hits")) *value = (double)c->rank_prefetch_hits;
    else if (!strcmp(key, "device_rank_runs")) *value = (double)c->device_rank_runs;
    else if (!strcmp(key, "score_wide_runs")) *value = (double)c->score_wide_runs;
    else if (!strcmp(key, "compare_runs")) *value = (double)c->compare_runs;
    else if (!strcmp(key, "f64_evals")) *value = (double)c->f64_evals;
    else if (!strcmp(key, "superpose_runs")) *value = (double)c->superpose_runs;
    else if (!strcmp(key, "rmsd_table_runs")) *value = (double)c->rmsd_table_runs;
    else if (!strcmp(key, "cluster_xcd_count")) *value = (double)c->xcd_count;
    else if (!strcmp(key, "cluster_xcd_base")) *value = (double)c->xcd_base;
    else if (!strcmp(key, "cluster_ok")) *value = c->cl_ok ? 1.0 : 0.0;
    else if (!strcmp(key, "cluster_parts")) *value = c->cl_ok ? (double)c->cl_plan.parts : 0.0;
    else if (!strcmp(key, "cluster_rows_per_wave")) *value = c->cl_ok ? (double)c->cl_plan.rpw : 0.0;
    else if (!strcmp(key, "cluster_late_tiles")) *value = c->cl_ok ? (double)c->cl_plan.late_tiles : 0.0;
    else if (!strcmp(key, "cluster_compute_waves")) *value = c->cl_ok ? (double)c->cl_plan.cw : 0.0;
    else if (!strcmp(key, "cluster_helper_waves")) *value = c->cl_ok ? (double)c->cl_plan.helpers : 0.0;
    else if (!strcmp(key, "cluster_wgs_per_cu")) *value = c->cl_ok ? (double)c->cl_plan.wgs_per_cu : 0.0;
    else if (!strcmp(key, "replica_groups")) *value = (double)active_groups(c);
    else if (!strcmp(key, "embed_form")) *value = (double)c->last_embed_form;
    else if (!strcmp(key, "embed_batches")) *value = (double)c->last_embed_batches;
    else if (!strcmp(key, "units_loaded")) *value = (double)g_units.loads.load();
    else if (!strcmp(key, "units_loaded_mask")) *value = (double)g_units.loaded[c->device & (kMaxDevices - 1)].load();
    else return fail(C3D_ERR_INVALID, std::string("c3d_get_stat: unknown key ") + key);
    return C3D_OK;
}

extern "C" const char* c3d_step_kernel_name(const c3d_ctx* c) {
    static thread_local char buf[96];
    if (!c) return "";
    const KernelRecord& k = c->ran;
    auto tf = [](bool b) { return b ? "true" : "false"; };
    switch (k.family) {
        case KernelRecord::CLUSTER:
            snprintf(buf, sizeof(buf), "c3d::k_cluster%s<%d, %d, %d, %d, %s>", k.tp ? "_tp" : "", k.pot, k.rpw, k.nb, k.wl, tf(k.late));
            break;
        case KernelRecord::STEP64:
        case KernelRecord::LBFGS_EVAL64: {
            const char* kernel = k.family == KernelRecord::STEP64 ? "k64_step" : "k64_lbfgs_eval";
            if (k.f64.chunk) snprintf(buf, sizeof(buf), "c3d::%s_chunked<%d, %s, %s, %d>", kernel, k.f64.pot, tf(k.f64.gen), tf(k.f64.fold), k.f64.chunk);
            else snprintf(buf, sizeof(buf), "c3d::%s<%d, %s, %s>", kernel, k.f64.pot, tf(k.f64.gen), tf(k.f64.fold));
            break;
        }
        case KernelRecord::PAIRS_SYM: snprintf(buf, sizeof(buf), "c3d::k_pairs_sym<%d, %s, false>", k.pot, tf(k.rs1)); break;
        case KernelRecord::STEP:
        case KernelRecord::LBFGS_EVAL: {
            const char* kernel = k.family == KernelRecord::STEP ? "k_step" : "k_lbfgs_eval";
            if (k.step.chunk) {
                if (k.step.wide) snprintf(buf, sizeof(buf), "c3d::%s_chunked<4, false, 4, 16, true, %d>", kernel, k.step.chunk);
                else snprintf(buf, sizeof(buf), "c3d::%s_chunked<%d, %s, %d, 8, false, %d>", kernel, k.step.pot, tf(k.step.gen), k.step.rpw, k.step.chunk);
            } else if (k.step.wide) snprintf(buf, sizeof(buf), "c3d::%s<4, false, 4, false, 16, true>", kernel);
            else snprintf(buf, sizeof(buf), "c3d::%s<%d, %s, %d, %s, 8, false>", kernel, k.step.pot, tf(k.step.gen), k.step.rpw, tf(k.step.nc));
            break;
        }
        default: return "";
    }
    return buf;
}

extern "C" int c3d_eval(c3d_ctx* c, float w_all, float w_vdw, float repel_s, float* F, double* e) {
    if (!c || !c->have_replicas) return fail(C3D_ERR_INVALID, "c3d_eval: bad state");
    C3D_ENTRY(c, 0u);
    const c3d::DevModel m = dev_model(c);
    const c3d::DevStep p = dev_step(c, 3, 0.0f, w_all, w_vdw, repel_s, 0.0f);
    if (F) {
        hipError_t err = c3d::launch_eval_forces(m, p, c->buf, c->parity, c->d_feval, c3d::general_step(m, p), c->eval_rpw,
                                                 c3d::column_chunk_for(m, c->column_chunk), c->stream);
        if (err != hipSuccess) return fail(C3D_ERR_HIP, std::string("eval launch: ") + hipGetErrorString(err));
        int rc = get_soa(c, c->d_feval, F);
        if (rc) return rc;
    }
    if (e) {
        const double rr = (double)repel_s * (double)c->model.r0_rep;
        hipError_t err = c3d::launch_energy(m, p, c->buf, c->parity, c->model.s_noe, c->model.k_rep, rr * rr, c->stream);
        if (err != hipSuccess) return fail(C3D_ERR_HIP, std::string("energy launch: ") + hipGetErrorString(err));
        if (int rc = read_back(c, c->buf.E, sizeof(double) * 4 * (size_t)c->nrep)) return rc;
        const double* h = static_cast<const double*>(c->h_stage);
        for (int r = 0; r < c->nrep; ++r) for (int k = 0; k < 3; ++k) e[3 * r + k] = h[4 * r + k];
    }
    return C3D_OK;
}

extern "C" int c3d_eval_f64(c3d_ctx* c, double w_all, double w_vdw, double repel_s, double* F, double* e) {
    if (int rc = need_f64_state(c, "c3d_eval_f64")) return rc;
    if (!F && !e) return fail(C3D_ERR_INVALID, "c3d_eval_f64: F and e are both NULL");
    C3D_ENTRY(c, unit_bit(UNIT_F64));
    const size_t n3 = (size_t)c->nrep * 3 * c3d::cols64(c->n);
    if (!c->b64.F) HIP_TRY(hipMalloc(&c->b64.F, sizeof(double) * (n3 + 4 * (size_t)c->nrep)));
    const c3d::DevModel m = dev_model(c);
    double mh[15];
    model_host64(c, mh);
    if (F) {
        const double sh[6] = {3.0, 0.0, w_all, w_vdw, repel_s, 0.0};
        hipError_t err = c3d::launch_eval_forces64(m, mh, sh, c->b64, c->parity, c->f64_column_chunk, c->b64.F, c->stream);
        if (err != hipSuccess) return fail(C3D_ERR_HIP, std::string("fp64 eval launch: ") + hipGetErrorString(err));
        if (int rc = get_soa64(c, c->b64.F, F)) return rc;
    }
    if (e) {
        const double rr = repel_s * (double)c->model.r0_rep;
        hipError_t err = c3d::launch_energy64(m, mh, rr * rr, c->b64, c->parity, c->b64.F + n3, c->stream);
        if (err != hipSuccess) return fail(C3D_ERR_HIP, std::string("fp64 energy launch: ") + hipGetErrorString(err));
        if (int rc = read_back(c, c->b64.F + n3, sizeof(double) * 4 * (size_t)c->nrep)) return rc;
        const double* h = static_cast<const double*>(c->h_stage);
        for (int r = 0; r < c->nrep; ++r) for (int k = 0; k < 3; ++k) e[3 * r + k] = h[4 * r + k];
    }
    ++c->f64_evals;
    return C3D_OK;
}

extern "C" int c3d_get_energies(c3d_ctx* c, double* e) {
    if (!c || !e) return fail(C3D_ERR_INVALID, "c3d_get_energies: null argument");
    float repel_s = 0.85f;
    if (!c->stages.empty()) repel_s = c->stages.back().repel_s;
    return c3d_eval(c, 1.0f, 1.0f, repel_s, nullptr, e);
}

struct ScoreScratch {
    size_t rank = 0, xr = 0, part = 0, hist = 0, below = 0, ovf = 0, box = 0, keys = 0, saa = 0, asym = 0, total = 0;
};
static ScoreScratch score_layout(int n, int nrep, unsigned nbins, size_t key_slots) {
    auto up = [](size_t b) { return (b + 255) & ~(size_t)255; };
    const size_t b_rank = up(sizeof(double) * (size_t)n * n), b_xr = up(sizeof(double) * 3 * (size_t)n * nrep), b_part = up(sizeof(double) * 4 * (size_t)n * nrep),
                 b_hist = up(sizeof(unsigned) * (size_t)nbins * nrep);
    ScoreScratch L;
    L.xr = b_rank; L.part = L.xr + b_xr; L.hist = L.part + b_part; L.below = L.hist + b_hist; L.ovf = L.below + b_hist;
// ... 454 lines not shown
```

chromosome3d_amd/csrc/c3d_cluster.hip:

```cpp
#include <hip/hip_ext.h>
#include <atomic>
#include <type_traits>
#include <cstdio>
#include <cstdlib>

#include "c3d_step_core.h"

namespace c3d {

typedef unsigned u32x4 __attribute__((ext_vector_type(4)));
constexpr int kClMaxThreads = 1024;

#ifdef C3D_STAMPS
__device__ unsigned long long g_cstamps[64][8];
__device__ unsigned long long g_pstamps[8];
#define CSTAMP(k) do { if (stamper) g_cstamps[s & 63][k] = __builtin_amdgcn_s_memrealtime(); } while (0)
#define CSTAMP_C(k) do { if (cstamper) g_cstamps[s & 63][k] = __builtin_amdgcn_s_memrealtime(); } while (0)
#else
#define CSTAMP(k) do { } while (0)
#define CSTAMP_C(k) do { } while (0)
#endif

template <int POT, int RPW, int NB, int WL, bool LATE, bool TWO>
__device__ __forceinline__ void cluster_body(
    const float* __restrict__ tgt, unsigned* __restrict__ claim, const StepRun* __restrict__ runs, const int P, const int CW, const int NH,
    const int static_place, const int nbeads, const int run0, const int skip0, const int nsteps,
    const unsigned tag_base, u32x4* __restrict__ rec, volatile unsigned* __restrict__ timeout, const unsigned expected,
    const AnnealIO& io, const DevModel& m, const DevFire& fp) {
    constexpr int NPAD = 256 * NB;
    constexpr int MAXT = NPAD / 8;
    constexpr int KUMAX = NB > 2 ? 3 : 2;
    extern __shared__ __attribute__((aligned(16))) float smem[];
    float* xs = smem;
    float* ys = smem + NPAD;
    float* zs = smem + 2 * NPAD;
    float* ps = smem + 3 * NPAD;
    float* fbuf = ps + 4 * MAXT;
    float* cbuf = fbuf + 3 * 64;
    float* lbuf = cbuf + 3 * 64;
    float* lcon = lbuf + 3 * 64;
    float* dump = lcon + 3 * 4 * 2 * 64;
    int* s_slot = reinterpret_cast<int*>(dump + 4);
#ifdef C3D_STAMPS
    const unsigned long long t_entry = __builtin_amdgcn_s_memrealtime();
#endif
    const int tid = threadIdx.x, lane = tid & 63, wave = tid >> 6;
    const int nthreads = (CW + NH) * 64;
    const int RW = CW * RPW;

    const int xcc = (int)(__builtin_amdgcn_s_getreg((3 << 11) | 20) & 0x7);
    const int sp_mode = static_place & 0xff, xcd0 = (static_place >> 8) & 0xff, nxcd = (static_place >> 16) & 0xff;
    int slot;
    if (sp_mode) {
        const unsigned off = ((unsigned)xcc - blockIdx.x + (sp_mode == 2 && blockIdx.x == 0 ? 1u : 0u)) & 7u;
        if (tid == 0) atomicOr(&claim[9], 1u << off);
        slot = (int)(blockIdx.x >> 3);
    } else {
        if (tid == 0) *s_slot = (int)atomicAdd(&claim[xcc], 1u);
        __syncthreads();
        slot = *s_slot;
    }
    const int lxcd = xcc - xcd0;
    const int lrep = lxcd + nxcd * (slot / P), part = slot % P;
#ifdef C3D_STAMPS
    const unsigned long long t_placed = __builtin_amdgcn_s_memrealtime();
#endif
    const bool is_compute = wave >= NH, is_h0 = wave == 0;
    const int cwave = wave - NH;
    const int wg_row0 = part * RW;
    const int row0 = wg_row0 + cwave * RPW;
    const StepRun first_run = runs[run0];
    float4 traw[RPW][NB];
#pragma unroll
    for (int r = 0; r < RPW; ++r)
#pragma unroll
        for (int jb = 0; jb < NB; ++jb) {
            float4 t = make_float4(0, 0, 0, 0);
            if (is_compute) {
                const float* trow = tgt + (size_t)min(row0 + r, nbeads - 1) * NPAD + 256 * jb;
                if (jb < NB - 1 || WL == 4) t = *reinterpret_cast<const float4*>(trow + 4 * lane);
                else if constexpr (WL == 3) {
                    struct F3 { float a, b, c; };
                    const F3 q = *reinterpret_cast<const F3*>(trow + 3 * lane);
                    t = make_float4(q.a, q.b, q.c, 0.0f);
                } else if constexpr (WL == 2) {
                    const float2 q = *reinterpret_cast<const float2*>(trow + 2 * lane);
                    t = make_float4(q.x, q.y, 0.0f, 0.0f);
                } else t = make_float4(trow[lane], 0.0f, 0.0f, 0.0f);
            }
            traw[r][jb] = t;
        }
    if (lxcd < 0 || lxcd >= nxcd || lrep >= m.nrep_g) return;
    const int rep = m.rep_base + lrep;
    const bool solo = P == 1;
    if (!is_compute) __builtin_amdgcn_s_setprio(3);

    const size_t roff = (size_t)rep * 3 * NPAD;
    const int hrow = wg_row0 + lane;
    const bool hfin = is_h0 && lane < RW && hrow < m.n;
#define C3D_HROW_INDEX const size_t ix = roff + hrow, iy = ix + NPAD, iz = iy + NPAD
    constexpr int rec_stride = NPAD + NPAD / 4;
    constexpr int KT = (MAXT + 63) / 64;
    constexpr bool late = LATE;
    const int gthreads = late ? nthreads - 64 : nthreads;
    const int gtid = late ? tid - 64 : tid;
    const int units = late ? m.n : m.n + 2 * m.ntiles;
    const int ku = (units + gthreads - 1) / gthreads;
    const auto rsrc = __builtin_amdgcn_make_buffer_rsrc(rec, 0, (int)(sizeof(u32x4) * 2 * m.nrep_g * rec_stride), 0x00020000);

    float vcx = 0.0f, vcy = 0.0f, vcz = 0.0f;
    FireState st;
    float4 cin[2], pin4 = make_float4(0, 0, 0, 0);
    {
        const float* xin = io.xin;
        const float* pin = io.pin;
        const float* vin = io.vin;
#pragma unroll
        for (int k = 0; k < 2; ++k) {
            const int b = 4 * (tid + k * nthreads);
            cin[k] = b < 3 * NPAD ? *reinterpret_cast<const float4*>(xin + roff + b) : make_float4(0, 0, 0, 0);
        }
        if (tid < m.ntiles) pin4 = reinterpret_cast<const float4*>(pin)[(size_t)rep * m.ntiles + tid];
        if (hfin) { C3D_HROW_INDEX; vcx = vin[ix]; vcy = vin[iy]; vcz = vin[iz]; }
        st = io.sin[rep];
    }
    float* const lc = lcon + (size_t)((wave >= 1 && wave <= 3) ? wave - 1 : 0) * (4 * 2 * 64);
    if (!is_compute && !is_h0 && wave <= 3 && m.nleft > 0) {
        for (int q = 0; q < 4; ++q) {
            const int k = 8 * (wave - 1) + 8 * (NH - 1) * q + (lane >> 3), c = lane & 7;
            float b = 0.0f, a = 0.0f;
            if (k < RW && c < m.nleft && wg_row0 + k < m.n) {
                const float t = tgt[(size_t)(wg_row0 + k) * NPAD + m.jl0 + c];
                b = t * m.inv_rs;
                a = t > 0.0f ? m.inv_rs : 0.0f;
            }
            lc[(2 * q) * 64 + lane] = b; lc[(2 * q + 1) * 64 + lane] = a;
        }
    }
#pragma unroll
    for (int k = 0; k < 2; ++k) {
        const int b = 4 * (tid + k * nthreads);
        if (b < 3 * NPAD) *reinterpret_cast<float4*>(smem + b) = cin[k];
    }
    if (tid < m.ntiles) reinterpret_cast<float4*>(ps)[tid] = pin4;
    if (tid < 3 * 64) lbuf[tid] = 0.0f;
#ifdef C3D_STAMPS
    asm volatile("s_waitcnt lgkmcnt(0)" ::: "memory");
    const unsigned long long t_coords = __builtin_amdgcn_s_memrealtime();
#endif
    constexpr bool PK = POT == 4;
    float4 tv[PK ? 1 : RPW][NB];
    PairConsts2<PK ? RPW : 1, NB> pc;
    float4* const mw = reinterpret_cast<float4*>(dump + 8) + (size_t)(is_compute ? cwave : 0) * (RPW * NB * 64);
    if constexpr (PK) {
        pair_consts2_build<RPW, NB>(m, traw, is_compute, lane, pc, mw);
    } else {
        DevStep p0{};
#pragma unroll
        for (int r = 0; r < RPW; ++r)
#pragma unroll
            for (int jb = 0; jb < NB; ++jb) {
                tv[r][jb] = pair_b<false>(m, traw[r][jb]);
                if (is_compute) mw[(r * NB + jb) * 64 + lane] = pair_a<false>(m, p0, traw[r][jb]);
            }
    }
#ifdef C3D_STAMPS
    asm volatile("s_waitcnt vmcnt(0) lgkmcnt(0)" ::: "memory");
    const unsigned long long t_targets = __builtin_amdgcn_s_memrealtime();
#endif
    int gsrc[KUMAX], gda[KUMAX], gdb[KUMAX], gdc[KUMAX];
    const int dump_off = (int)(dump - smem);
#pragma unroll
    for (int k = 0; k < KUMAX; ++k) {
        const int u = min(max(gtid + gthreads * k, 0), units - 1);
        int src, da, db = dump_off, dc = dump_off;
        if (u < m.n) { src = u; da = u; db = NPAD + u; dc = 2 * NPAD + u; }
        else {
            const int j = u - m.n, t = j >> 1;
            src = NPAD + j;
            if ((j & 1) == 0) { da = 3 * NPAD + 4 * t; db = da + 1; dc = da + 2; }
            else da = 3 * NPAD + 4 * t + 3;
        }
        if (gtid < 0 || gtid + gthreads * k >= units) da = db = dc = dump_off;
        gsrc[k] = src; gda[k] = da; gdb[k] = db; gdc[k] = dc;
    }

#ifdef C3D_STAMPS
    const bool stamper = lrep == 0 && part == 0 && is_h0 && lane == 0;
    const bool cstamper = lrep == 0 && part == 0 && cwave == 0 && lane == 0;
    if (stamper) { g_pstamps[0] = t_entry; g_pstamps[1] = __builtin_amdgcn_s_memrealtime(); g_pstamps[6] = t_placed; }
    if (cstamper) { g_pstamps[4] = t_targets; g_pstamps[5] = t_coords; }
#endif
    auto role_loop = [&](auto role) {
    constexpr int ROLE = decltype(role)::value;
    int s = 0;
    StepRun cur = first_run;
    for (int run = run0;; ++run) {
      if (run != run0) cur = runs[run];
      const DevStep p = cur.p;
      const int count = cur.count;
      const bool needs_partials = p.kind == 0 || p.kind == 1 || p.kind == 2 || (TWO && p.kind == 5);
      for (int it = run == run0 ? skip0 : 0; it < count; ++it, ++s) {
#ifdef C3D_STAMPS
        if (cstamper && s == 0) g_pstamps[7] = __builtin_amdgcn_s_memrealtime();
#endif
        __syncthreads();
        CSTAMP(0);
#ifdef C3D_STAMPS
        if (stamper && s == 0) g_pstamps[2] = __builtin_amdgcn_s_memrealtime();
#endif
        CSTAMP_C(6);

        float hx0 = 0.0f, hy0 = 0.0f, hz0 = 0.0f;
        StepScalars sc;
        sc.lam = 1.0f; sc.cmx = sc.cmy = sc.cmz = 0.0f; sc.keep = 0.0f; sc.mix = 0.0f;
        if constexpr (ROLE == 0) {
            if (p.kind != 4) {
                float Fx, Fy, Fz;
                if constexpr (PK) tile_pair_sums_pk<RPW, NB, WL>(m, p, pc, mw, xs, ys, zs, row0, lane, Fx, Fy, Fz);
                else tile_pair_sums_reg<POT, RPW, NB, WL, 1>(m, p, tv, mw, xs, ys, zs, row0, lane, Fx, Fy, Fz);
                if (lane < RPW) {
                    const int k = cwave * RPW + lane;
                    fbuf[k] = Fx; fbuf[64 + k] = Fy; fbuf[128 + k] = Fz;
                }
                CSTAMP_C(7);
            }
        } else if constexpr (ROLE == 1) {
            if (p.kind != 2 && !(TWO && p.kind == 5)) { st.dt = fp.dt_start; st.alpha = fp.alpha_start; st.npos = 0; st.pad = 0; }
            float4 psum = make_float4(0, 0, 0, 0);
            if (needs_partials) {
                if (late && !solo && s > 0) {
                    const unsigned tagp = tag_base + (unsigned)s;
                    const int basep = ((s & 1) * m.nrep_g + lrep) * rec_stride + NPAD;
                    u32x4 a[KT], b[KT];
                    unsigned spins = 0;
                    for (;;) {
                        bool ok = true;
                        asm volatile("" ::: "memory");
#pragma unroll
                        for (int k = 0; k < KT; ++k) {
                            const int t = min(lane + 64 * k, m.ntiles - 1);
                            a[k] = __builtin_amdgcn_raw_buffer_load_b128(rsrc, (basep + 2 * t) * 16, 0, 16);
                            b[k] = __builtin_amdgcn_raw_buffer_load_b128(rsrc, (basep + 2 * t + 1) * 16, 0, 16);
                        }
#pragma unroll
                        for (int k = 0; k < KT; ++k) ok &= a[k].x == tagp && b[k].x == tagp;
                        if (__all(ok)) break;
                        __builtin_amdgcn_s_sleep(1);
                        ++spins;
                        if (spins > (1u << 18) || ((spins & 1023u) == 0 && *timeout != 0u)) {
                            if (lane == 0) *timeout = 1u;
                            return;
                        }
                    }
#pragma unroll
                    for (int k = 0; k < KT; ++k)
                        if (lane + 64 * k < m.ntiles)
                            reinterpret_cast<float4*>(ps)[lane + 64 * k] = make_float4(__uint_as_float(a[k].y), __uint_as_float(a[k].z), __uint_as_float(a[k].w), __uint_as_float(b[k].y));
                }
                for (int t = lane; t < m.ntiles; t += 64) {
                    const float4 q = reinterpret_cast<const float4*>(ps)[t];
                    psum.x += q.x; psum.y += q.y; psum.z += q.z; psum.w += q.w;
                }
                psum = wave_sum4(psum);
                psum.x = __uint_as_float(__builtin_amdgcn_readfirstlane(__float_as_uint(psum.x)));
                psum.y = __uint_as_float(__builtin_amdgcn_readfirstlane(__float_as_uint(psum.y)));
                psum.z = __uint_as_float(__builtin_amdgcn_readfirstlane(__float_as_uint(psum.z)));
                psum.w = __uint_as_float(__builtin_amdgcn_readfirstlane(__float_as_uint(psum.w)));
            }
            sc = step_scalars<TWO>(m, p, fp, psum, st);
            if (lane < RW && hrow < NPAD) { hx0 = xs[hrow]; hy0 = ys[hrow]; hz0 = zs[hrow]; }
            CSTAMP(1);
        } else if (p.kind != 4) {
            for (int cb = 16 * (wave - 1); cb < RW; cb += 16 * (NH - 1)) {
                const int k = cb + (lane >> 2);
                float cx, cy, cz;
                chain_term(m, p, xs, ys, zs, wg_row0 + k, lane & 3, k < RW, cx, cy, cz);
                cx = quad_chain_sum(cx); cy = quad_chain_sum(cy); cz = quad_chain_sum(cz);
                if ((lane & 3) == 0 && k < RW) { cbuf[k] = cx; cbuf[64 + k] = cy; cbuf[128 + k] = cz; }
            }
            if (m.nleft > 0) {
                const PairK kk = pair_k(m, p);
                for (int q = 0; q < 4; ++q) {
                    const int k = 8 * (wave - 1) + 8 * (NH - 1) * q + (lane >> 3), c = lane & 7;
                    if (8 * (wave - 1) + 8 * (NH - 1) * q < RW) {
                        const bool active = k < RW && c < m.nleft && wg_row0 + k < m.n;
                        float lx, ly, lz;
                        leftover_terms<POT, false>(m, p, kk, xs, ys, zs, min(wg_row0 + k, m.n - 1), c, active, lc[(2 * q) * 64 + lane], lc[(2 * q + 1) * 64 + lane], lx, ly, lz);
                        if (c == 0 && k < RW) { lbuf[k] = lx; lbuf[64 + k] = ly; lbuf[128 + k] = lz; }
                    }
                }
            }
        }
        __syncthreads();
        CSTAMP(2);
        const bool last = s + 1 == nsteps;
        const unsigned tag = tag_base + (unsigned)s + 1u;
        const int base = (((s + 1) & 1) * m.nrep_g + lrep) * rec_stride;

        if constexpr (ROLE == 1) {
            float4 q = make_float4(0, 0, 0, 0);
            float xn = 0.0f, yn = 0.0f, zn = 0.0f;
            auto row_update = [&](auto kc) {
                constexpr int K = decltype(kc)::value;
                DevStep pk = p;
                pk.kind = K;
                if (hfin) {
                    float Fx = 0.0f, Fy = 0.0f, Fz = 0.0f;
                    if constexpr (K != 4) {
                        const float sx0 = fbuf[lane], sy0 = fbuf[64 + lane], sz0 = fbuf[128 + lane];
                        const float lx = lbuf[lane], ly = lbuf[64 + lane], lz = lbuf[128 + lane];
                        const float cx = cbuf[lane], cy = cbuf[64 + lane], cz = cbuf[128 + lane];
                        const bool lo = m.nleft > 0;
                        const float sx = lo ? sx0 + lx : sx0, sy = lo ? sy0 + ly : sy0, sz = lo ? sz0 + lz : sz0;
                        Fx = row_total<false>(pk, sx, cx);
                        Fy = row_total<false>(pk, sy, cy);
                        Fz = row_total<false>(pk, sz, cz);
                    }
                    float vx0 = vcx, vy0 = vcy, vz0 = vcz;
                    if constexpr (K == 3 || K == 6) { vx0 = vy0 = vz0 = 0.0f; }
                    else if constexpr (K == 4) { C3D_HROW_INDEX; const float* vinit = io.vinit; vx0 = vinit[ix]; vy0 = vinit[iy]; vz0 = vinit[iz]; }
                    finish_row(m, pk, fp, sc, st, Fx, Fy, Fz, hx0, hy0, hz0, vx0, vy0, vz0, xn, yn, zn, vcx, vcy, vcz, q);
                    if (!last && !solo) {
                        u32x4 o;
                        o.x = tag; o.y = __float_as_uint(xn); o.z = __float_as_uint(yn); o.w = __float_as_uint(zn);
                        __builtin_amdgcn_raw_buffer_store_b128(o, rsrc, (base + hrow) * 16, 0, 0);
                    }
                } else {
                    xn = hx0; yn = hy0; zn = hz0;
                }
            };
            bool two_point_step = false;
            if constexpr (TWO) {
                two_point_step = p.kind >= 5;
                if (p.kind == 5) row_update(std::integral_constant<int, 5>{});
                else if (p.kind == 6) row_update(std::integral_constant<int, 6>{});
            }
            if (!two_point_step) switch (p.kind) {
                case 0: row_update(std::integral_constant<int, 0>{}); break;
                case 1: row_update(std::integral_constant<int, 1>{}); break;
                case 2: row_update(std::integral_constant<int, 2>{}); break;
                case 3: row_update(std::integral_constant<int, 3>{}); break;
                default: row_update(std::integral_constant<int, 4>{}); break;
            }
            if (late && !last && !solo) { CSTAMP(4); __builtin_amdgcn_s_barrier(); }
            float4 t = q;
            t.x += dpp_mov<0xB1>(t.x); t.y += dpp_mov<0xB1>(t.y); t.z += dpp_mov<0xB1>(t.z); t.w += dpp_mov<0xB1>(t.w);
            t.x += dpp_mov<0x4E>(t.x); t.y += dpp_mov<0x4E>(t.y); t.z += dpp_mov<0x4E>(t.z); t.w += dpp_mov<0x4E>(t.w);
            t.x += dpp_mov<0x12C>(t.x); t.y += dpp_mov<0x12C>(t.y); t.z += dpp_mov<0x12C>(t.z); t.w += dpp_mov<0x12C>(t.w);
            CSTAMP(3);
            if (last) {
                if (hfin) {
                    C3D_HROW_INDEX;
                    float* xout = io.xout;
                    float* vout = io.vout;
                    xout[ix] = xn; xout[iy] = yn; xout[iz] = zn;
                    vout[ix] = vcx; vout[iy] = vcy; vout[iz] = vcz;
                }
                const int tl = (wg_row0 + lane) >> 3;
                if ((lane & 7) == 0 && lane < RW && tl < m.ntiles) reinterpret_cast<float4*>(io.pout)[(size_t)rep * m.ntiles + tl] = t;
                if (lane == 0 && part == 0) io.sout[rep] = st;
                if (lane == 0 && atomicAdd(&claim[8], 1u) + 1u == expected) {
                    const unsigned seen = sp_mode ? atomicOr(&claim[9], 0u) : 1u;
                    if ((seen & (seen - 1u)) == 0u) timeout[1] = tag_base | 1u;
                    else timeout[2] = 1u;
                }
#ifdef C3D_STAMPS
                if (stamper) g_pstamps[3] = __builtin_amdgcn_s_memrealtime();
#endif
                return;
            }
            if (solo) {
                if (lane < RW && hrow < NPAD) { xs[hrow] = xn; ys[hrow] = yn; zs[hrow] = zn; }
                if ((lane & 7) == 0 && lane < RW) reinterpret_cast<float4*>(ps)[lane >> 3] = t;
            } else if ((lane & 7) == 0 && lane < RW && ((wg_row0 + lane) >> 3) < m.ntiles) {
                u32x4 o0, o1;
                o0.x = tag; o0.y = __float_as_uint(t.x); o0.z = __float_as_uint(t.y); o0.w = __float_as_uint(t.z);
                o1.x = tag; o1.y = __float_as_uint(t.w); o1.z = 0u; o1.w = 0u;
                const int u0 = base + NPAD + 2 * ((wg_row0 + lane) >> 3);
                __builtin_amdgcn_raw_buffer_store_b128(o0, rsrc, u0 * 16, 0, 0);
                __builtin_amdgcn_raw_buffer_store_b128(o1, rsrc, (u0 + 1) * 16, 0, 0);
            }
            CSTAMP(5);
            if (solo || late) continue;
        }
        {
            if (last) return;
            if (solo) continue;
            __builtin_amdgcn_s_barrier();
            u32x4 v[KUMAX];
            unsigned spins = 0;
            for (;;) {
                bool ok = true;
                asm volatile("" ::: "memory");
#pragma unroll
                for (int k = 0; k < KUMAX; ++k)
                    if (k < ku) v[k] = __builtin_amdgcn_raw_buffer_load_b128(rsrc, (base + gsrc[k]) * 16, 0, 16);
#pragma unroll
                for (int k = 0; k < KUMAX; ++k)
                    if (k < ku) ok &= v[k].x == tag;
                if (__all(ok)) break;
                __builtin_amdgcn_s_sleep(1);
                ++spins;
                if (spins > (1u << 18) || ((spins & 1023u) == 0 && *timeout != 0u)) {
                    if (lane == 0) *timeout = 1u;
                    return;
                }
            }
#pragma unroll
            for (int k = 0; k < KUMAX; ++k)
                if (k < ku) { smem[gda[k]] = __uint_as_float(v[k].y); smem[gdb[k]] = __uint_as_float(v[k].z); smem[gdc[k]] = __uint_as_float(v[k].w); }
        }
      }
    }
    };
    if (is_compute) role_loop(std::integral_constant<int, 0>{});
    else if (is_h0) role_loop(std::integral_constant<int, 1>{});
    else role_loop(std::integral_constant<int, 2>{});
}

#define C3D_CLUSTER_ARGS                                                                                                                  \
    const float* __restrict__ tgt, unsigned* __restrict__ claim, const StepRun* __restrict__ runs, const int P, const int CW, const int NH, \
    const int static_place, const int nbeads, const int run0, const int skip0, const int nsteps, const unsigned tag_base,                 \
    u32x4* __restrict__ rec, volatile unsigned* __restrict__ timeout, const unsigned expected, const AnnealIO io, const DevModel m, const DevFire fp
#define C3D_CLUSTER_PASS tgt, claim, runs, P, CW, NH, static_place, nbeads, run0, skip0, nsteps, tag_base, rec, timeout, expected, io, m, fp
template <int POT, int RPW, int NB, int WL, bool LATE>
__global__ __launch_bounds__(kClMaxThreads) void k_cluster(C3D_CLUSTER_ARGS) { cluster_body<POT, RPW, NB, WL, LATE, false>(C3D_CLUSTER_PASS); }
template <int POT, int RPW, int NB, int WL, bool LATE>
__global__ __launch_bounds__(kClMaxThreads) void k_cluster_tp(C3D_CLUSTER_ARGS) { cluster_body<POT, RPW, NB, WL, LATE, true>(C3D_CLUSTER_PASS); }
#undef C3D_CLUSTER_ARGS
#undef C3D_CLUSTER_PASS

constexpr bool cluster_late_ok(int pot, int rpw, int nb, int wl) { return pot >= 3 && rpw * (4 * (nb - 1) + wl) >= 6; }
#ifndef C3D_CLUSTER_POT
#ifdef C3D_STAMPS
hipError_t read_cluster_stamps(unsigned long long* out) { return hipMemcpyFromSymbol(out, HIP_SYMBOL(g_cstamps), sizeof(unsigned long long) * 64 * 8); }
hipError_t read_cluster_pstamps(unsigned long long* out) { return hipMemcpyFromSymbol(out, HIP_SYMBOL(g_pstamps), sizeof(unsigned long long) * 8); }
#endif

__global__ __launch_bounds__(kClMaxThreads) void k_tear16(u32x4* buf, unsigned* stop, unsigned long long* stats, int iters) {
    const auto rsrc = __builtin_amdgcn_make_buffer_rsrc(buf, 0, kClMaxThreads * 16, 0x00020000);
    const int tid = threadIdx.x;
    if (blockIdx.x == 0) {
        for (int i = 1; i <= iters; ++i) {
            u32x4 v; v.x = v.y = v.z = v.w = (unsigned)i;
            __builtin_amdgcn_raw_buffer_store_b128(v, rsrc, tid * 16, 0, 0);
        }
        __threadfence();
        if (tid == 0) atomicExch(stop, 1u);
        return;
    }
    const auto ssrc = __builtin_amdgcn_make_buffer_rsrc(stop, 0, 4, 0x00020000);
    unsigned long long reads = 0, torn = 0, fresh = 0;
    unsigned lastv = 0;
    for (unsigned guard = 0; guard < (1u << 26); ++guard) {
        asm volatile("" ::: "memory");
        const u32x4 v = __builtin_amdgcn_raw_buffer_load_b128(rsrc, tid * 16, 0, 16);
        ++reads;
        if (!(v.x == v.y && v.y == v.z && v.z == v.w)) ++torn;
        if (v.x != lastv) { ++fresh; lastv = v.x; }
        if ((reads & 255) == 0 && __builtin_amdgcn_raw_buffer_load_b32(ssrc, 0, 0, 16) != 0u) break;
    }
    atomicAdd(&stats[0], reads); atomicAdd(&stats[1], torn); atomicAdd(&stats[2], fresh);
}
hipError_t launch_tear16(int num_cus, void* buf, unsigned* stop, unsigned long long* stats, int iters, hipStream_t s) {
    hipLaunchKernelGGL(k_tear16, dim3(num_cus), dim3(kClMaxThreads), 0, s, reinterpret_cast<u32x4*>(buf), stop, stats, iters);
    return hipGetLastError();
}


bool cluster_plan(const DevModel& m, int num_cus, int num_xcc, int forced_geom, int forced_late, int xcd_count, ClusterPlan* plan) {
    if (m.npad > 1024 || num_xcc != 8 || num_cus < 8 || num_cus % 8) return false;
    const int cus_per_xcd = num_cus / 8;
    if (xcd_count < 1 || xcd_count > 8) return false;
    const int per_xcd = (m.nrep_g + xcd_count - 1) / xcd_count;
    const int nb = m.npad / 256;
    static const int geoms[][4] = {{8, 1, 4, 1}, {8, 2, 4, 1}, {12, 2, 4, 1}, {8, 4, 4, 1}, {10, 4, 4, 1}, {12, 4, 4, 1}, {8, 3, 4, 1},
                                   {4, 2, 4, 1}, {4, 4, 4, 1}, {6, 4, 4, 1}};
    double best = 1e30;
    bool found = false;
    const int fcw = forced_geom / 100, frpw = forced_geom / 10 % 10, fnh = forced_geom % 10;
    for (const auto& g : geoms) {
        const int cw = g[0], rpw = g[1], nh = g[2], wpc = g[3], rw = cw * rpw;
        if (fcw && (cw != fcw || rpw != frpw || nh != fnh)) continue;
        if (rw % 8 || rw > 64) continue;
        if (rpw * nb > 8) continue;
        if (m.noe_pot < 3 && (m.wl != 4 || m.nleft != 0)) continue;
        if (m.nleft > 0 && (nh != 4 || (rw + 8 * (nh - 1) - 1) / (8 * (nh - 1)) > 4)) continue;
        const int P = (m.n + rw - 1) / rw;
        if (per_xcd * P > cus_per_xcd * wpc) continue;
        const int threads = (cw + nh) * 64;
        const int kumax = nb > 2 ? 3 : 2;
        const int late = P > 1 && forced_late != 0 && cluster_late_ok(m.noe_pot, rpw, nb, m.wl) &&
                         (m.noe_pot != 4 || ((cw + 3) / 4) * rpw * (4 * (nb - 1) + m.wl) >= 12);
        if ((late ? m.n : m.n + 2 * ((m.n + 7) / 8)) > (late ? threads - 64 : threads) * kumax) continue;
        size_t lds = sizeof(float) * (3 * m.npad + 4 * (m.npad / 8) + 9 * 64 + 24 * 64 + 16) + (size_t)cw * rpw * nb * 64 * 16;
        if (wpc == 1) { if (lds < 84 * 1024) lds = 84 * 1024; }
        else if (lds > 78 * 1024 || threads > 512) continue;
        const int wps = (cw * wpc + 3) / 4;
        const double per_slot = m.noe_pot == 4 ? (rpw / 2) * 22.0 + (rpw & 1) * 19.0 : rpw * 15.0;
        const double valu = (wps == 1 ? 1.6 : (wps == 2 ? 1.15 : 1.0)) * wps * ((4 * (nb - 1) + m.wl) * per_slot + 60.0);
        const double serial = 200.0 + (P > 1 ? 140.0 + 0.92 * m.n : 0.0);
        const double cost = wpc == 1 ? valu + serial : (valu > serial ? valu + 0.35 * serial : 0.5 * valu + serial);
        if (cost < best) {
            best = cost; found = true;
            plan->rpw = rpw; plan->cw = cw; plan->helpers = nh; plan->wgs_per_cu = wpc; plan->parts = P; plan->per_xcd = per_xcd;
            plan->grid = num_cus * wpc; plan->threads = threads; plan->units = 2 * rw; plan->device = 0; plan->lds = lds;
            plan->expected = (unsigned)(m.nrep_g * P);
            plan->late_tiles = late;
            plan->xcd_count = xcd_count;
        }
    }
    return found;
}

size_t cluster_record_bytes(const DevModel& m, const ClusterPlan& pl) { (void)pl; return (size_t)2 * m.nrep_g * (m.npad + m.npad / 4) * 16; }

#endif

template <int POT, int RPW, int NB, int WL, bool LATE>
static hipError_t cluster_go(const DevModel& m, const DevFire& fp, const ClusterPlan& pl, const AnnealIO& io, const float* tgt, void* rec,
                             const StepRun* runs, int run0, int skip0, int nsteps, unsigned tag_base, unsigned* timeout, unsigned* claim,
                             hipStream_t s) {
#if defined(C3D_CLUSTER_TP)
    constexpr bool kHasLean = false, kHasTp = true;
#elif defined(C3D_CLUSTER_POT)
    constexpr bool kHasLean = true, kHasTp = false;
#else
    constexpr bool kHasLean = true, kHasTp = true;
#endif
    const int tp = pl.two_point ? 1 : 0;
    if ((tp && !kHasTp) || (!tp && !kHasLean)) return hipErrorInvalidValue;
    const int sp = (pl.static_place & 0xff) | ((pl.xcd_base & 0xff) << 8) | ((pl.xcd_count & 0xff) << 16);
#define C3D_CL_LAUNCH(K)                                                                                                                              \
    do {                                                                                                                                              \
        if (pl.t0 && pl.t1)                                                                                                                           \
            hipExtLaunchKernelGGL((K<POT, RPW, NB, WL, LATE>), dim3(pl.grid), dim3(pl.threads), pl.lds, s, pl.t0, pl.t1, 0, tgt, claim, runs,          \
                                  pl.parts, pl.cw, pl.helpers, sp, m.n, run0, skip0, nsteps, tag_base, reinterpret_cast<u32x4*>(rec), timeout, pl.expected, io, m, fp); \
        else                                                                                                                                          \
            hipLaunchKernelGGL((K<POT, RPW, NB, WL, LATE>), dim3(pl.grid), dim3(pl.threads), pl.lds, s, tgt, claim, runs, pl.parts, pl.cw, pl.helpers, \
                               sp, m.n, run0, skip0, nsteps, tag_base, reinterpret_cast<u32x4*>(rec), timeout, pl.expected, io, m, fp);                \
    } while (0)
    if constexpr (kHasTp) { if (tp) C3D_CL_LAUNCH(k_cluster_tp); }
    if constexpr (kHasLean) { if (!tp) C3D_CL_LAUNCH(k_cluster); }
#undef C3D_CL_LAUNCH
    return hipGetLastError();
}
template <int POT, class F>
static void for_each_cluster_form(F&& f) {
    auto widths = [&](auto R, auto B) {
        auto w = [&](auto W) {
            f(R, B, W, bool_c<false>{});
            if constexpr (cluster_late_ok(POT, R, B, W)) f(R, B, W, bool_c<true>{});
        };
        w(int_c<4>{});
        if constexpr (POT >= 3) { w(int_c<3>{}); w(int_c<2>{}); w(int_c<1>{}); }
    };
    widths(int_c<1>{}, int_c<1>{}); widths(int_c<1>{}, int_c<2>{}); widths(int_c<1>{}, int_c<3>{}); widths(int_c<1>{}, int_c<4>{});
    widths(int_c<2>{}, int_c<1>{}); widths(int_c<2>{}, int_c<2>{}); widths(int_c<2>{}, int_c<3>{}); widths(int_c<2>{}, int_c<4>{});
    widths(int_c<3>{}, int_c<1>{}); widths(int_c<3>{}, int_c<2>{});
    widths(int_c<4>{}, int_c<1>{}); widths(int_c<4>{}, int_c<2>{});
}
template <int POT>
static hipError_t cluster_geom(const DevModel& m, const DevFire& fp, const ClusterPlan& pl, const AnnealIO& io, const float* tgt, void* rec,
                               const StepRun* runs, int run0, int skip0, int nsteps, unsigned tag_base, unsigned* timeout, unsigned* claim,
                               hipStream_t s) {
    hipError_t e = hipErrorInvalidValue;
    for_each_cluster_form<POT>([&](auto R, auto B, auto W, auto L) {
        if (pl.rpw == R && m.npad == 256 * B && m.wl == W && (pl.late_tiles != 0) == L)
            e = cluster_go<POT, R, B, W, L>(m, fp, pl, io, tgt, rec, runs, run0, skip0, nsteps, tag_base, timeout, claim, s);
    });
    return e;
}

template <int POT, bool TP>
static hipError_t cluster_prepare_unit() {
    hipError_t e = hipSuccess;
    for_each_cluster_form<POT>([&](auto R, auto B, auto W, auto L) {
        const void* k;
        if constexpr (TP) k = reinterpret_cast<const void*>(&k_cluster_tp<POT, R, B, W, L>);
        else k = reinterpret_cast<const void*>(&k_cluster<POT, R, B, W, L>);
        if (e == hipSuccess) e = hipFuncSetAttribute(k, hipFuncAttributeMaxDynamicSharedMemorySize, 160 * 1024);
    });
    return e;
}

#define C3D_CL_CAT2(a, b) a##b
#define C3D_CL_CAT(a, b) C3D_CL_CAT2(a, b)
#if defined(C3D_CLUSTER_POT) && defined(C3D_CLUSTER_TP)
hipError_t C3D_CL_CAT(launch_cluster_tp_pot, C3D_CLUSTER_POT)(const DevModel& m, const DevFire& fp, const ClusterPlan& pl, const AnnealIO& io, const float* tgt, void* rec,
                          const StepRun* runs, int run0, int skip0, int nsteps, unsigned tag_base, unsigned* timeout, unsigned* claim,
                          hipStream_t s) {
    return cluster_geom<C3D_CLUSTER_POT>(m, fp, pl, io, tgt, rec, runs, run0, skip0, nsteps, tag_base, timeout, claim, s);
}
hipError_t C3D_CL_CAT(preload_cluster_tp_pot, C3D_CLUSTER_POT)() { return cluster_prepare_unit<C3D_CLUSTER_POT, true>(); }
#elif defined(C3D_CLUSTER_POT)
hipError_t C3D_CL_CAT(launch_cluster_pot, C3D_CLUSTER_POT)(const DevModel& m, const DevFire& fp, const ClusterPlan& pl, const AnnealIO& io, const float* tgt, void* rec,
                          const StepRun* runs, int run0, int skip0, int nsteps, unsigned tag_base, unsigned* timeout, unsigned* claim,
                          hipStream_t s) {
    return cluster_geom<C3D_CLUSTER_POT>(m, fp, pl, io, tgt, rec, runs, run0, skip0, nsteps, tag_base, timeout, claim, s);
}
hipError_t C3D_CL_CAT(preload_cluster_pot, C3D_CLUSTER_POT)() { return cluster_prepare_unit<C3D_CLUSTER_POT, false>(); }
#else
using ClusterLaunch = hipError_t(const DevModel& m, const DevFire& fp, const ClusterPlan& pl, const AnnealIO& io, const float* tgt, void* rec,
                                 const StepRun* runs, int run0, int skip0, int nsteps, unsigned tag_base, unsigned* timeout, unsigned* claim,
                                 hipStream_t s);
#if defined(C3D_CLUSTER_SPLIT)
ClusterLaunch launch_cluster_pot0, launch_cluster_pot1, launch_cluster_pot2, launch_cluster_pot3, launch_cluster_pot4;
ClusterLaunch launch_cluster_tp_pot0, launch_cluster_tp_pot1, launch_cluster_tp_pot2, launch_cluster_tp_pot3, launch_cluster_tp_pot4;
hipError_t preload_cluster_pot0(), preload_cluster_pot1(), preload_cluster_pot2(), preload_cluster_pot3(), preload_cluster_pot4();
hipError_t preload_cluster_tp_pot0(), preload_cluster_tp_pot1(), preload_cluster_tp_pot2(), preload_cluster_tp_pot3(), preload_cluster_tp_pot4();
static ClusterLaunch* const kClusterLaunch[2][5] = {{launch_cluster_pot0, launch_cluster_pot1, launch_cluster_pot2, launch_cluster_pot3, launch_cluster_pot4},
                                                    {launch_cluster_tp_pot0, launch_cluster_tp_pot1, launch_cluster_tp_pot2, launch_cluster_tp_pot3, launch_cluster_tp_pot4}};
static hipError_t (*const kClusterPreload[2][5])() = {{preload_cluster_pot0, preload_cluster_pot1, preload_cluster_pot2, preload_cluster_pot3, preload_cluster_pot4},
                                                      {preload_cluster_tp_pot0, preload_cluster_tp_pot1, preload_cluster_tp_pot2, preload_cluster_tp_pot3, preload_cluster_tp_pot4}};
#endif
hipError_t launch_cluster(const DevModel& m, const DevFire& fp, const ClusterPlan& pl, const AnnealIO& io, const float* tgt, void* rec,
                          const StepRun* runs, int run0, int skip0, int nsteps, unsigned tag_base, unsigned* timeout, unsigned* claim,
                          hipStream_t s) {
#if defined(C3D_CLUSTER_SPLIT)
    return kClusterLaunch[pl.two_point][device_pot(m.noe_pot)](m, fp, pl, io, tgt, rec, runs, run0, skip0, nsteps, tag_base, timeout, claim, s);
#else
    return with_pot(m.noe_pot, [&](auto POT) { return cluster_geom<POT>(m, fp, pl, io, tgt, rec, runs, run0, skip0, nsteps, tag_base, timeout, claim, s); });
#endif
}

AnnealIO anneal_io(const DevBuffers& b, int parity) {
    const int q = parity ^ 1;
    AnnealIO io;
    io.pin = b.P[parity]; io.xin = b.X[parity]; io.vin = b.V[parity]; io.vinit = b.Vinit; io.sin = b.S[parity];
    io.xout = b.X[q]; io.vout = b.V[q]; io.pout = b.P[q]; io.sout = b.S[q];
    return io;
}

hipError_t preload_cluster_unit(int pot, bool two_point) {
    if (pot < 0 || pot > 4) return hipErrorInvalidValue;
#if defined(C3D_CLUSTER_SPLIT)
    return kClusterPreload[two_point][pot]();
#else
    return with_pot(pot, [&](auto POT) { return with_bool(two_point, [&](auto TP) { return cluster_prepare_unit<POT, TP>(); }); });
#endif
}
hipError_t preload_cluster_base_unit() {
    hipFuncAttributes a;
    return hipFuncGetAttributes(&a, reinterpret_cast<const void*>(&k_tear16));
}
#endif

}
```

chromosome3d_amd/csrc/c3d_device.hip:

```cpp
#include "c3d_step_core.h"

namespace c3d {

#ifdef C3D_STAMPS
__device__ unsigned long long g_stamps[16];
#define C3D_STAMP(k)                                                                   \
    do {                                                                               \
        if (blockIdx.x + blockIdx.y + blockIdx.z == 0 && threadIdx.x == 0) g_stamps[k] = __builtin_readcyclecounter(); \
    } while (0)
#else
#define C3D_STAMP(k) do { } while (0)
#endif


__device__ __forceinline__ bool block_to_tile(const DevModel& m, int& tile, int& rep) {
    rep = m.rep_base + blockIdx.y;
    tile = blockIdx.z * 8 + blockIdx.x;
    return tile < m.ntiles;
}
inline dim3 grid_blocks(const DevModel& m, int tiles = 1) { return dim3(8, m.nrep_g, ((m.ntiles + tiles - 1) / tiles + 7) / 8); }



#ifndef C3D_SHARE_SCALARS
#define C3D_SHARE_SCALARS 1
#endif

template <int POT, bool GEN, int RPW, bool NC, int TR = kTileRows, bool WIDE = false>
__global__ __launch_bounds__(64 * TR / RPW) __attribute__((amdgpu_waves_per_eu(WIDE ? 4 : 1))) void k_step(
    const float* __restrict__ pin, const float* __restrict__ xin, const float* __restrict__ tgt,
    const float* __restrict__ vin, const float* __restrict__ vinit, const FireState* __restrict__ sin,
    float* __restrict__ xout, float* __restrict__ vout, float* __restrict__ pout, FireState* __restrict__ sout,
    const DevModel m, const DevStep p, const DevFire fp) {
    using COLS = ColsStaged;
#include "c3d_step_body.inc"
}
template <int POT, bool GEN, int RPW, int TR, bool WIDE, int CHUNK>
__global__ __launch_bounds__(64 * TR / RPW) __attribute__((amdgpu_waves_per_eu(WIDE ? 4 : 1))) void k_step_chunked(
    const float* __restrict__ pin, const float* __restrict__ xin, const float* __restrict__ tgt,
    const float* __restrict__ vin, const float* __restrict__ vinit, const FireState* __restrict__ sin,
    float* __restrict__ xout, float* __restrict__ vout, float* __restrict__ pout, FireState* __restrict__ sout,
    const DevModel m, const DevStep p, const DevFire fp) {
    constexpr bool NC = false;
    using COLS = ColsChunked<CHUNK, 64 * TR / RPW>;
#include "c3d_step_body.inc"
}

#ifdef C3D_STAMPS
hipError_t read_stamps(unsigned long long* out) { return hipMemcpyFromSymbol(out, HIP_SYMBOL(g_stamps), sizeof(unsigned long long) * 16); }
#endif

__global__ __launch_bounds__(256) void k_pair_targets(int n, int npad, float inv_rs, const float* __restrict__ tgt, float* __restrict__ tgs2) {
    const int nblk = npad >> 8, npairs = (n + 1) / 2;
    const size_t idx = (size_t)blockIdx.x * 256 + threadIdx.x;
    if (idx >= (size_t)npairs * nblk * 64) return;
    const int lane = (int)(idx & 63), jb = (int)((idx >> 6) % nblk), q = (int)((idx >> 6) / nblk);
    const int ra = min(2 * q, n - 1), rb = min(2 * q + 1, n - 1);
    const float4 a = *reinterpret_cast<const float4*>(tgt + (size_t)ra * npad + 256 * jb + 4 * lane);
    const float4 b = *reinterpret_cast<const float4*>(tgt + (size_t)rb * npad + 256 * jb + 4 * lane);
    auto enc = [inv_rs](float t) { return t > 0.0f ? t * inv_rs : 1e30f; };
    float4* out = reinterpret_cast<float4*>(tgs2 + idx * 8);
    out[0] = make_float4(enc(a.x), enc(b.x), enc(a.y), enc(b.y));
    out[1] = make_float4(enc(a.z), enc(b.z), enc(a.w), enc(b.w));
}
size_t pair_targets_floats(int n, int npad) { return (size_t)((n + 1) / 2) * (npad >> 8) * 64 * 8; }
hipError_t launch_pair_targets(const DevModel& m, const float* tgt, float* tgs2, hipStream_t s) {
    const size_t items = (size_t)((m.n + 1) / 2) * (m.npad >> 8) * 64;
    hipLaunchKernelGGL(k_pair_targets, dim3((unsigned)((items + 255) / 256)), dim3(256), 0, s, m.n, m.npad, m.inv_rs, tgt, tgs2);
    return hipGetLastError();
}

static size_t step_lds_bytes(const DevModel& m, int chunk, size_t row_floats) {
    return sizeof(float) * ((chunk ? (size_t)6 * chunk : (size_t)3 * m.npad) + row_floats);
}

hipError_t launch_step(const DevModel& m0, const DevStep& p, const DevFire& fp, const DevBuffers& b, int par, const StepForm& f, hipStream_t s) {
    const int q = par ^ 1;
    DevModel m = m0;
    m.tgs2 = f.pairs ? b.tgs2 : nullptr;
    const int tr = f.wide ? 2 * kTileRows : kTileRows;
    const auto go = [&](auto kernel, int rpw) {
        hipLaunchKernelGGL(kernel, grid_blocks(m, tr / kTileRows), dim3(64 * tr / rpw), step_lds_bytes(m, f.chunk, 4 * tr + 12), s,
                           b.P[par], b.X[par], b.tgt, b.V[par], b.Vinit, b.S[par], b.X[q], b.V[q], b.P[q], b.S[q], m, p, fp);
        return hipGetLastError();
    };
    return with_chunk(f.chunk, [&](auto CH) {
        if (f.wide) {
            if constexpr (CH == 0) return go(k_step<4, false, 4, false, 2 * kTileRows, true>, 4);
            else return go(k_step_chunked<4, false, 4, 2 * kTileRows, true, CH>, 4);
        }
        return with_pot(f.pot, [&](auto POT) { return with_bool(f.gen, [&](auto GEN) { return with_rpw(f.rpw, [&](auto RPW) {
            if constexpr (CH == 0) return with_bool(f.nc, [&](auto NC) { return go(k_step<POT, GEN, RPW, NC>, RPW); });
            else return go(k_step_chunked<POT, GEN, RPW, kTileRows, false, CH>, RPW);
        }); }); });
    });
}

template <int POT, bool GEN, int ERPW, bool PACKED = true>
__global__ __launch_bounds__(64 * kTileRows / ERPW) void k_eval_forces(const DevModel m, const DevStep p,
                                                       const float* __restrict__ tgt, const float* __restrict__ xin,
                                                       float* __restrict__ fout) {
    using COLS = ColsStaged;
#include "c3d_eval_forces_body.inc"
}
template <int POT, bool GEN, int ERPW, bool PACKED, int CHUNK>
__global__ __launch_bounds__(64 * kTileRows / ERPW) void k_eval_forces_chunked(const DevModel m, const DevStep p,
                                                               const float* __restrict__ tgt, const float* __restrict__ xin,
                                                               float* __restrict__ fout) {
    using COLS = ColsChunked<CHUNK, 64 * kTileRows / ERPW>;
#include "c3d_eval_forces_body.inc"
}

hipError_t launch_eval_forces(const DevModel& m, const DevStep& p, const DevBuffers& b, int parity, float* Fout,
                              bool general_tail, int rows_per_wave, int chunk, hipStream_t s) {
    static_assert(kEvalRowsPerWave == 4, "the hook's default form is four rows per wave");
    const auto go = [&](auto kernel, int erpw) {
        hipLaunchKernelGGL(kernel, grid_blocks(m), dim3(64 * kTileRows / erpw), step_lds_bytes(m, chunk, 0), s, m, p, b.tgt, b.X[parity], Fout);
        return hipGetLastError();
    };
    return with_chunk(chunk, [&](auto CH) { return with_pot(m.noe_pot, [&](auto POT) { return with_bool(general_tail, [&](auto GEN) {
        if constexpr (POT == 4 && !GEN)
            if (rows_per_wave == 2 || rows_per_wave == -2) return with_bool(rows_per_wave == 2, [&](auto PACKED) {
                if constexpr (CH == 0) return go(k_eval_forces<4, false, 2, PACKED>, 2);
                else return go(k_eval_forces_chunked<4, false, 2, PACKED, CH>, 2);
            });
        if constexpr (CH == 0) return go(k_eval_forces<POT, GEN, 4>, 4);
        else return go(k_eval_forces_chunked<POT, GEN, 4, true, CH>, 4);
    }); }); });
}

__global__ __launch_bounds__(256) void k_energy(const DevModel m, const float s_noe, const float k_rep,
                                               const double rep_r2, const float* __restrict__ tgt,
                                               const float* __restrict__ xin, double* __restrict__ eout) {
    __shared__ double red[3][256];
    const int rep = blockIdx.x, tid = threadIdx.x;
    const float* x = xin + (size_t)rep * 3 * m.npad;
    const float* y = x + m.npad;
    const float* z = y + m.npad;
    double e_noe = 0, e_bond = 0, e_rep = 0;
    const double rs = m.rs, c = m.tail_c, b = m.tail_b;
    const double a = rs * rs - b / rs - c * rs;
    const bool pot3 = m.noe_pot == 3 || m.noe_pot == 4;
    const double mrs = m.mrs, mc = m.mtail_c, mb = m.mexp == 2 ? 0.5 * m.mtail_b : m.mtail_b;
    const double ma = mrs * mrs - (m.mexp == 2 ? mb / (mrs * mrs) : mb / mrs) - mc * mrs;
    for (int i = tid; i < m.n; i += 256) {
        const double xi = x[i], yi = y[i], zi = z[i];
        for (int j = i + 1; j < m.n; ++j) {
            const double dx = xi - x[j], dy = yi - y[j], dz = zi - z[j];
            double r2 = dx * dx + dy * dy + dz * dz;
            if (r2 < 1e-12) r2 = 1e-12;
            const float v = tgt[(size_t)i * m.npad + j];
            const double t = v;
            const int sep = j - i;
            if (t > 0) {
                const double delta = sqrt(r2) - t, ad = fabs(delta);
                bool soft;
                if (m.noe_pot == 0) soft = ad > rs; else if (m.noe_pot == 1 || pot3) soft = delta > rs; else soft = false;
                if (pot3 && delta < -mrs) e_noe += ma + (m.mexp == 2 ? mb / (ad * ad) : mb / ad) + mc * ad;
                else e_noe += soft ? (a + b / ad + c * ad) : delta * delta;
            }
            if (sep == 1) { const double dl = sqrt(r2) - m.b0; e_bond += 0.5 * m.k_bond2 * dl * dl; }
            if (sep == 2 && m.k_ang2 > 0) {
                const double d = sqrt(r2);
                if (m.ang_mode == 1 || d < m.a0) { const double dl = d - m.a0; e_bond += 0.5 * m.k_ang2 * dl * dl; }
            }
            if (sep >= m.rep_sep && r2 < rep_r2) { const double q = rep_r2 - r2; e_rep += q * q; }
        }
    }
    red[0][tid] = e_noe * s_noe; red[1][tid] = e_bond; red[2][tid] = e_rep * k_rep;
    __syncthreads();
    for (int s = 128; s > 0; s >>= 1) {
        if (tid < s) { red[0][tid] += red[0][tid + s]; red[1][tid] += red[1][tid + s]; red[2][tid] += red[2][tid + s]; }
        __syncthreads();
    }
    if (tid == 0) { eout[rep * 4 + 0] = red[0][0]; eout[rep * 4 + 1] = red[1][0]; eout[rep * 4 + 2] = red[2][0]; eout[rep * 4 + 3] = 0; }
}

hipError_t launch_energy(const DevModel& m, const DevStep& p, const DevBuffers& b, int parity, float s_noe, float k_rep,
                         double rep_r2, hipStream_t s) {
    hipLaunchKernelGGL(k_energy, dim3(m.nrep), dim3(256), 0, s, m, s_noe, k_rep, rep_r2, b.tgt, b.X[parity], b.E);
    return hipGetLastError();
}

__global__ __launch_bounds__(256) void k_centre(const DevModel m, float* __restrict__ xio) {
    __shared__ double red[3][256];
    const int rep = blockIdx.x, tid = threadIdx.x;
    float* x = xio + (size_t)rep * 3 * m.npad;
    double s[3] = {0, 0, 0};
    for (int i = tid; i < m.n; i += 256) { s[0] += x[i]; s[1] += x[m.npad + i]; s[2] += x[2 * m.npad + i]; }
    for (int c = 0; c < 3; ++c) red[c][tid] = s[c];
    __syncthreads();
    for (int k = 128; k > 0; k >>= 1) {
        if (tid < k) for (int c = 0; c < 3; ++c) red[c][tid] += red[c][tid + k];
        __syncthreads();
    }
    const float cx = (float)(red[0][0] / m.n), cy = (float)(red[1][0] / m.n), cz = (float)(red[2][0] / m.n);
    for (int i = tid; i < m.n; i += 256) { x[i] -= cx; x[m.npad + i] -= cy; x[2 * m.npad + i] -= cz; }
}
hipError_t launch_centre(const DevModel& m, const DevBuffers& b, int parity, hipStream_t s) {
    hipLaunchKernelGGL(k_centre, dim3(m.nrep), dim3(256), 0, s, m, b.X[parity]);
    return hipGetLastError();
}

__global__ __launch_bounds__(256) void k_if_pow_sum(const double* __restrict__ IF, size_t nn, double alpha,
                                                   double* __restrict__ P, double* __restrict__ partial) {
    __shared__ double red[256];
    double s = 0;
    const size_t per = (nn + gridDim.x - 1) / gridDim.x;
    const size_t lo = per * blockIdx.x, hi = lo + per < nn ? lo + per : nn;
    for (size_t k = lo + threadIdx.x; k < hi; k += 256) {
        const double v = pow(IF[k], alpha);
        P[k] = v;
        s += v;
    }
    red[threadIdx.x] = s;
    __syncthreads();
    for (int k = 128; k > 0; k >>= 1) {
        if ((int)threadIdx.x < k) red[threadIdx.x] += red[threadIdx.x + k];
        __syncthreads();
    }
    if (threadIdx.x == 0) partial[blockIdx.x] = red[0];
// ... 78 lines not shown
```

chromosome3d_amd/csrc/c3d_internal.h:

```cpp
#pragma once
#include <hip/hip_runtime.h>
#include <stdint.h>
#include <type_traits>

#include "c3d_superpose.h"

namespace c3d {

constexpr float kBoltz = 0.0019872f;
constexpr float kAccel = 418.4f;

constexpr int kTileRows = 8;
constexpr int kEvalRowsPerWave = 4;
constexpr int kEvalBlock = 64 * kTileRows / kEvalRowsPerWave;

constexpr float kPadCoord = 1.0e4f;

struct DevModel {
    int n, npad, ntiles, nrep;
    int rep_base, nrep_g;
    int stage_dma;
    int rpw;
    int noe_pot, ang_mode, rep_sep;
    int mexp;
    float rs, tail_c, tail_b;
    float mrs, mtail_c, mtail_b;
    float nmrs;
    float inv_rs, nm_rs;
    int wl, nleft, jl0;
    float k_bond2, b0;
    float k_ang2, a0;
    float acc;
    float t_fac;
    float fbeta;
    float inv_n;
    const float* tgs2;
};

struct DevStep {
    int kind;
    float dt;
    float w_all;
    float w_noe2n;
    float w_rep4;
    float rep_r2;
    float inv_rep_r2;
    float w_rep4r2;
    float w_rs;
    float kq;
    float t_bath;
};

struct DevFire {
    float dt_start, dt_max, f_inc, f_dec, alpha_start, f_alpha, max_step;
    int n_min;
};

struct FireState {
    float dt, alpha;
    int npos, pad;
};

struct DevBuffers {
    float* tgt;
    float* tgs2;
    float* X[2];
    float* V[2];
    float* Vinit;
    float* P[2];
    FireState* S[2];
    double* E;
};

template <int V> using int_c = std::integral_constant<int, V>;
template <bool V> using bool_c = std::integral_constant<bool, V>;
inline int device_pot(int noe_pot) { return noe_pot == 0 || noe_pot == 1 || noe_pot == 3 || noe_pot == 4 ? noe_pot : 2; }
template <class F> hipError_t with_pot(int pot, F&& f) {
    switch (device_pot(pot)) {
        case 0: return f(int_c<0>{});
        case 1: return f(int_c<1>{});
        case 3: return f(int_c<3>{});
        case 4: return f(int_c<4>{});
        default: return f(int_c<2>{});
    }
}
template <class F> hipError_t with_rpw(int rpw, F&& f) { return rpw == 1 ? f(int_c<1>{}) : rpw == 2 ? f(int_c<2>{}) : f(int_c<4>{}); }
template <class F> hipError_t with_bool(bool b, F&& f) { return b ? f(bool_c<true>{}) : f(bool_c<false>{}); }

inline bool general_tail(const DevModel& m) {
    if (!(m.tail_b == 0.0f && m.tail_c == 2.0f * m.rs)) return true;
    return m.noe_pot == 3 && !(m.mtail_b == 0.0f && m.mtail_c == 2.0f * m.mrs);
}
inline bool general_step(const DevModel& m, const DevStep& p) { return general_tail(m) || p.w_rs == 0.0f; }
inline bool pair_targets_fit(const DevModel& m) { return device_pot(m.noe_pot) == 4 && m.rpw == 2 && m.wl == 4 && m.nleft == 0; }

struct StepForm {
    int pot;
    bool gen;
    int rpw;
    bool nc, pairs, wide;
    int chunk;
};
constexpr int kMaxStagedCols = 5120;
constexpr int kDefaultColumnChunk = 1024;
inline bool column_chunk_valid(int chunk) { return chunk == 256 || chunk == 1024 || chunk == 2048; }
inline int column_chunk_for(const DevModel& m, int option) {
    if (!(m.wl == 4 && m.nleft == 0)) return 0;
    if (option > 0) return option;
    return m.npad <= kMaxStagedCols ? 0 : kDefaultColumnChunk;
}
inline StepForm step_form(const DevModel& m, const DevStep& p, bool wide_tiles, bool pair_targets, bool tgs2_built, int column_chunk) {
    StepForm f;
    f.pot = device_pot(m.noe_pot);
    f.rpw = m.rpw == 1 || m.rpw == 2 ? m.rpw : 4;
    f.gen = general_step(m, p);
    f.nc = !(m.wl == 4 && m.nleft == 0);
    f.pairs = !f.gen && pair_targets_fit(m) && tgs2_built;
    f.wide = wide_tiles && pair_targets && f.pairs && m.npad > 1024;
    f.chunk = column_chunk_for(m, column_chunk);
    return f;
}
inline bool sym_rs1(const DevModel& m) { return m.rs == 1.0f; }

hipError_t launch_step(const DevModel& m, const DevStep& p, const DevFire& fp, const DevBuffers& b, int parity, const StepForm& f, hipStream_t s);
hipError_t launch_eval_forces(const DevModel& m, const DevStep& p, const DevBuffers& b, int parity, float* Fout,
                              bool general_tail, int rows_per_wave, int chunk, hipStream_t s);
hipError_t launch_energy(const DevModel& m, const DevStep& p, const DevBuffers& b, int parity, float s_noe,
                         float k_rep, double rep_r2, hipStream_t s);
hipError_t launch_centre(const DevModel& m, const DevBuffers& b, int parity, hipStream_t s);
constexpr int kLbfgsMaxPairs = 8;
constexpr int kLbfgsQ = 4 * kLbfgsMaxPairs + 4;
struct LbfgsState {
    int cnt, head, mem, resets;
    double gamma;
    double SY[kLbfgsMaxPairs][kLbfgsMaxPairs];
    double YY[kLbfgsMaxPairs][kLbfgsMaxPairs];
};
struct LbfgsBuffers {
    float* hist;
    float* part;
    LbfgsState* S[2];
};
__host__ __device__ inline size_t lbfgs_hist_floats(int npad) { return (size_t)2 * kLbfgsMaxPairs * 3 * npad; }
hipError_t launch_lbfgs_eval(const DevModel& m, const DevStep& p, const DevBuffers& b, const LbfgsBuffers& lb, int parity, int mem,
                             const StepForm& f, hipStream_t s);
hipError_t launch_lbfgs_move(const DevModel& m, const DevStep& p, const DevFire& fp, const DevBuffers& b, const LbfgsBuffers& lb, int parity,
                             int mem, hipStream_t s);
size_t pair_targets_floats(int n, int npad);
hipError_t launch_pair_targets(const DevModel& m, const float* tgt, float* tgs2, hipStream_t s);
struct StepRun {
    DevStep p;
    int count;
};
struct AnnealIO {
    const float *pin, *xin, *vin, *vinit;
    const FireState* sin;
    float *xout, *vout, *pout;
    FireState* sout;
};
AnnealIO anneal_io(const DevBuffers& b, int parity);
struct ClusterPlan {
    int rpw, cw, helpers, wgs_per_cu, parts, per_xcd, grid, threads, units, device;
    int static_place = 1;
    int xcd_base = 0, xcd_count = 8;
    bool two_point = false;
    int late_tiles = 0;
    unsigned expected = 0;
    size_t lds;
    hipEvent_t t0 = nullptr, t1 = nullptr;
};
bool cluster_plan(const DevModel& m, int num_cus, int num_xcc, int forced_geom, int forced_late, int xcd_count, ClusterPlan* plan);
size_t cluster_record_bytes(const DevModel& m, const ClusterPlan& pl);
hipError_t launch_cluster(const DevModel& m, const DevFire& fp, const ClusterPlan& pl, const AnnealIO& io, const float* tgt, void* rec,
                          const StepRun* runs, int run0, int skip0, int nsteps, unsigned tag_base, unsigned* timeout,
                          unsigned* claim, hipStream_t s);
hipError_t preload_device_unit();
hipError_t preload_cluster_base_unit();
hipError_t preload_cluster_unit(int pot, bool two_point);
hipError_t preload_score_unit();
hipError_t preload_embed_unit();
hipError_t preload_f64_unit();
hipError_t preload_sym_unit();
hipError_t launch_tear16(int num_cus, void* buf, unsigned* stop, unsigned long long* stats, int iters, hipStream_t s);
void sym_geometry(const DevModel& m, int* Q, int* G, int* ntiles_offdiag, int* ntiles_diag);
size_t sym_scratch_floats(const DevModel& m);
void sym_tile_list(const DevModel& m, int2* out);
hipError_t launch_step_sym(const DevModel& m, const DevStep& p, const DevFire& fp, const DevBuffers& b, int parity, const void* tiles,
                           float* scratch, hipStream_t s);
struct Buffers64 {
    int32_t* t10 = nullptr;
    double* T = nullptr;
    double* X[2] = {nullptr, nullptr};
    double* V[2] = {nullptr, nullptr};
    double* Vinit = nullptr;
    double* P[2] = {nullptr, nullptr};
    void* S[2] = {nullptr, nullptr};
    double* F = nullptr;
};
int cols64(int n);
constexpr int kMaxStagedBeads64 = 2560;
constexpr int kDefaultColumnChunk64 = 512;
inline bool column_chunk64_valid(int chunk) { return chunk == 256 || chunk == 512 || chunk == 1024; }
inline int column_chunk64_for(int n, int option) {
    if (option > 0) return n > option ? option : 0;
    return n <= kMaxStagedBeads64 ? 0 : kDefaultColumnChunk64;
}
struct Form64 {
    int pot;
    bool gen, fold;
    int chunk;
};
inline Form64 form64(int noe_pot, const double* model_host, double w_all, int n = 0, int column_chunk = 0) {
    const double* h = model_host;
    const int mexp = (int)h[14] == 2 ? 2 : 1;
    const double rs = h[1], tail_c = h[2] * h[1], tail_b = (tail_c - 2.0 * rs) * rs * rs;
    const double mrs = h[4], mtail_c = h[3], mtail_b = (mtail_c - 2.0 * mrs) * mrs * mrs * (mexp == 2 ? mrs : 1.0);
    Form64 f;
    f.pot = noe_pot == 4 && !(mexp == 2 && mtail_c == 0.0 && tail_b == 0.0 && tail_c == 2.0 * rs) ? 3 : device_pot(noe_pot);
    f.gen = !(tail_b == 0.0 && tail_c == 2.0 * rs) || (f.pot == 3 && !(mtail_b == 0.0 && mtail_c == 2.0 * mrs));
    f.fold = f.pot == 4 && !f.gen && w_all != 0.0;
    f.chunk = column_chunk64_for(n, column_chunk);
    return f;
}
hipError_t launch_step64(const DevModel& d, const double* model_host, const double* step_host, const double* fire_host, int fire_n_min,
                         const Buffers64& b, int parity, int column_chunk, hipStream_t s);
struct LbfgsBuffers64 {
    double* hist = nullptr;
    double* part = nullptr;
    LbfgsState* S[2] = {nullptr, nullptr};
};
hipError_t launch_lbfgs_eval64(const DevModel& d, const double* model_host, const double* step_host, const Buffers64& b, const LbfgsBuffers64& lb,
                               int parity, int mem, int column_chunk, hipStream_t s);
hipError_t launch_lbfgs_move64(const DevModel& d, const double* model_host, const double* step_host, const double* fire_host, int fire_n_min,
                               const Buffers64& b, const LbfgsBuffers64& lb, int parity, int mem, hipStream_t s);
hipError_t launch_targets64(const DevModel& d, const double* model_host, int min_sep, const int32_t* t10, double* T, hipStream_t s);
hipError_t launch_tenths64(int n, int R, const int32_t* ri, const int32_t* rj, const int32_t* rt10, int32_t* t10, hipStream_t s);
hipError_t launch_import64(const DevModel& d, const float* Xf, const Buffers64& b, hipStream_t s);
hipError_t launch_export64(const DevModel& d, const Buffers64& b, int parity, float* Xf, float* Vf, float* Pf, hipStream_t s);
hipError_t launch_eval_forces64(const DevModel& d, const double* model_host, const double* step_host, const Buffers64& b, int parity,
                                int column_chunk, double* Fout, hipStream_t s);
hipError_t launch_energy64(const DevModel& d, const double* model_host, double rep_r2, const Buffers64& b, int parity, double* Eout, hipStream_t s);
size_t fire_state64_bytes();
hipError_t launch_if_to_target(const double* IF, int n, int npad, double alpha, double K, int min_sep, int rep_sep,
                               double* scratchP, double* partial, int npartial, int32_t* dist10, float* tgt,
                               unsigned char* flags, unsigned* nflag, hipStream_t s);

constexpr int kDgEigMaxBeads = (int)((160 * 1024 / sizeof(float) - 16) / 9);
hipError_t launch_dg_smooth(const float* tgt, int n, int npad, float b0, float lower, float* U, float* L, hipStream_t s);
hipError_t launch_dg_embed(const float* U, const float* L, int n, int npad, int nrep, uint64_t seed, uint32_t first_replica, int iters,
                           float* v, float* D2, float* wt, float* x0, float* x1, bool tiled, int batch, hipStream_t s);

hipError_t launch_score(const float* xin, const float* tgt, const double* rankA, int n, int npad, int nrep, int range, int min_sep,
                        unsigned nbins, double ma, double mb, double relax, double* xr, unsigned* hist, unsigned* below,
                        double* partial, int* overflow, hipStream_t s);
hipError_t launch_score_bbox(const double* xr, int n, int nrep, double* box, hipStream_t s);
hipError_t launch_score_wide(const double* xr, const float* tgt, const double* rankA, int n, int npad, int nrep, int range, int min_sep,
                             unsigned nbins, double ma, double mb, double relax, unsigned* hist, unsigned* below, double* partial,
                             int* overflow, hipStream_t s);
constexpr int kRankTile = 4096;
inline size_t if_rank_key_slots(size_t mh) {
    size_t slots = kRankTile;
    while (slots < mh) slots <<= 1;
    return slots;
}
hipError_t launch_if_rank_keys(const double* M, int n, int range, unsigned long long* keys, size_t mh, size_t slots, int* asym, hipStream_t s);
hipError_t launch_if_rank_sort(double* M, int n, int range, unsigned long long* keys, size_t mh, size_t slots, double ma, double* saa_rows,
                               hipStream_t s);
constexpr int kCmpModels = 16;
inline size_t compare_chunk_pairs(size_t m, int K) {
    const size_t nb = (size_t)(K + kCmpModels - 1) / kCmpModels, want = 2048 / (nb * nb) > 64 ? 2048 / (nb * nb) : 64;
    return ((m + want - 1) / want + 63) / 64 * 64;
}
inline int compare_table_chunks(size_t m, int K) {
    const size_t per = compare_chunk_pairs(m, K);
    return (int)((m + per - 1) / per);
}
hipError_t launch_compare_coords(const float* xin, int n, int npad, int nrep, double* xyz, hipStream_t s);
hipError_t launch_compare_ranks(const double* x, int n, unsigned long long* keys, size_t m, size_t slots, unsigned* ke, double* rowsum,
                                hipStream_t s);
hipError_t launch_compare_table(const double* xyz, const unsigned* ke, const double* rowsum, int n, int K, size_t m, double* sums,
                                double* partial, double* table, hipStream_t s);
constexpr int kSupNoIdent = -(1 << 30);
inline int superpose_chunks(int n) { return (n + 63) / 64; }
inline size_t superpose_partial_doubles(int n, int KB) {
    return (size_t)superpose_chunks(n) * (size_t)((KB + kCmpModels - 1) / kCmpModels) * 256 * kSupCov;
}
hipError_t launch_superpose_gather64(const double* X, int n, int np, int nrep, double* xyz, hipStream_t s);
hipError_t launch_superpose_centre(double* xyz, int n, int K, double* cent, hipStream_t s);
hipError_t launch_superpose_fit(const double* A, int KA, const double* B, int KB, int n, int ident, bool mirror, const int* fixed, double* partial,
                                double* cov, double* fit, int* mirrored, double* res, hipStream_t s);
hipError_t launch_superpose_apply(const double* A, int K, int n, const double* fit, const double* shift, double* fitted, hipStream_t s);
hipError_t launch_superpose_mean(const double* fitted, int K, int n, double* mean, double* rmsf, double* dev, hipStream_t s);
hipError_t launch_superpose_store32(const double* fitted, int n, int npad, int nrep, float* X, hipStream_t s);
hipError_t launch_superpose_store64(const double* fitted, int n, int np, int nrep, double* X0, double* X1, hipStream_t s);

inline float encode_target_host(float t) { return t > 0 ? t : 0.0f; }

}
```

Measured before the change: 4.643 million.

## Precompute encoded pair constants once and load them directly in cluster kernel

Adds a cached device buffer of pre-encoded pair target constants, built by k_pair_targets and keyed on inv_rs/n/npad/wl, so the resident cluster kernel loads ready-made float4 pairs instead of loading raw targets and building pair constants each launch. It also skips re-planning the cluster when set_model does not change geometry-relevant fields, and moves the replica-range early exit ahead of the target loads. The cache adds invalidation paths on every target change, and a stale cache would give wrong constants.

```diff
diff --git a/chromosome3d_amd/csrc/c3d_api.cpp b/chromosome3d_amd/csrc/c3d_api.cpp
--- a/chromosome3d_amd/csrc/c3d_api.cpp
+++ b/chromosome3d_amd/csrc/c3d_api.cpp
@@ -163,6 +163,10 @@
     c3d::ClusterPlan cl_plan{};
     void* d_crec = nullptr;
     size_t crec_bytes = 0;
+    float* d_ccon = nullptr;
+    size_t ccon_floats = 0;
+    bool ccon_valid = false;
+    struct { float inv_rs; int n, npad, wl; } ccon_key{};
     static constexpr unsigned kClaimSets = 4096;
     static constexpr unsigned kClaimWords = 16;
     unsigned* d_claim = nullptr;
@@ -205,6 +209,7 @@
     long superpose_runs = 0, rmsd_table_runs = 0;
     long k1_recomputed = 0, k1_patched = 0;
     long graph_captures = 0, graph_launches = 0, step_launches = 0, resident_launches = 0, cluster_launches = 0;
+    long cluster_record_wipes = 0, cluster_const_builds = 0;
     bool has_two_point = false;
     bool has_lbfgs = false;
     int lbfgs_mem = 5;
@@ -238,6 +243,8 @@
     }
     dev_free(c->d_crec);
     c->crec_bytes = 0; c->cl_ok = false;
+    dev_free(c->d_ccon);
+    c->ccon_floats = 0; c->ccon_valid = false;
     dev_free(c->buf.Vinit); dev_free(c->buf.E); dev_free(c->d_feval);
     dev_free(c->d_sym_scratch); dev_free(c->d_sym_tiles);
     dev_free(c->lb.hist); dev_free(c->lb.part); dev_free(c->lb.S[0]); dev_free(c->lb.S[1]);
@@ -378,6 +385,7 @@
 
 int upload_targets(c3d_ctx* c, const std::vector<float>& enc) {
     dev_free(c->buf.tgt); dev_free(c->buf.tgs2);
+    c->ccon_valid = false;
     HIP_TRY(hipMalloc(&c->buf.tgt, sizeof(float) * enc.size()));
     HIP_TRY(hipMemcpyAsync(c->buf.tgt, enc.data(), sizeof(float) * enc.size(), hipMemcpyHostToDevice, c->stream));
     HIP_TRY(hipStreamSynchronize(c->stream));
@@ -662,6 +670,27 @@
     return C3D_OK;
 }
 
+int ensure_cluster_consts(c3d_ctx* c, const c3d::DevModel& m) {
+    if (!c3d::cluster_preencoded(c3d::device_pot(m.noe_pot), c->cl_plan.rpw)) return C3D_OK;
+    auto& k = c->ccon_key;
+    if (c->ccon_valid && c->d_ccon && memcmp(&k.inv_rs, &m.inv_rs, sizeof(float)) == 0 && k.n == m.n && k.npad == m.npad && k.wl == m.wl) return C3D_OK;
+    c->ccon_valid = false;
+    const size_t floats = c3d::pair_targets_floats(m.n, m.npad);
+    HIP_TRY(hipStreamSynchronize(c->stream));
+    if (!c->d_ccon || floats > c->ccon_floats) {
+        dev_free(c->d_ccon);
+        c->ccon_floats = 0;
+        HIP_TRY(hipMalloc(&c->d_ccon, sizeof(float) * floats));
+        c->ccon_floats = floats;
+    }
+    hipError_t e = c3d::launch_pair_targets(m, c->buf.tgt, c->d_ccon, c->stream);
+    if (e != hipSuccess) return fail(C3D_ERR_HIP, std::string("cluster pair constants: ") + hipGetErrorString(e));
+    k.inv_rs = m.inv_rs; k.n = m.n; k.npad = m.npad; k.wl = m.wl;
+    ++c->cluster_const_builds;
+    c->ccon_valid = true;
+    return C3D_OK;
+}
+
 bool cluster_ok(c3d_ctx* c) {
     if (!c->resident || !c->cluster || !c->cl_ok || !c->d_crec) return false;
     return !c3d::general_tail(dev_model(c));
@@ -701,12 +730,14 @@
     const unsigned seq = c->cl_seq % c3d_ctx::kClaimSets;
     if (seq == 0) {
         HIP_TRY(hipMemsetAsync(c->d_crec, 0, c->crec_bytes, c->stream));
+        ++c->cluster_record_wipes;
         HIP_TRY(hipMemsetAsync(c->d_claim, 0, sizeof(unsigned) * c3d_ctx::kClaimWords * c3d_ctx::kClaimSets, c->stream));
     }
+    const c3d::DevModel m = dev_model(c);
+    if (int rc = ensure_cluster_consts(c, m)) { c->cl_ok = false; return rc; }
     ++c->cl_seq;
     if (c->inject_timeout) { *c->h_tmo = 1; c->inject_timeout = false; }
     c->h_tmo[1] = 0;
-    const c3d::DevModel m = dev_model(c);
     c3d::ClusterPlan pl = c->cl_plan;
     if (c->inject_incomplete) { ++pl.expected; c->inject_incomplete = false; }
     if (c->kernel_timing) { pl.t0 = c->kev0; pl.t1 = c->kev1; }
@@ -717,7 +748,7 @@
     c->inject_misplaced = false;
     c->h_tmo[2] = 0;
     const auto h0 = std::chrono::steady_clock::now();
-    hipError_t e = c3d::launch_cluster(m, dev_fire(c), pl, c3d::anneal_io(c->buf, c->parity), c->buf.tgt, c->d_crec, c->d_prog,
+    hipError_t e = c3d::launch_cluster(m, dev_fire(c), pl, c3d::anneal_io(c->buf, c->parity), c->buf.tgt, c->d_ccon, c->d_crec, c->d_prog,
                                        c->op_run[c->pc], c->op_skip[c->pc], (int)nops, seq << 20, c->h_tmo_dev,
                                        c->d_claim + c3d_ctx::kClaimWords * seq, c->stream);
     if (e != hipSuccess) return fail(C3D_ERR_HIP, std::string("cluster launch: ") + hipGetErrorString(e));
@@ -1066,10 +1097,13 @@
     const bool targets64 = c->precision == 64 && c->b64.T;
     Entry entry(c, 0u, targets64);
     if (entry.rc != C3D_OK) return entry.rc;
+    const c3d::DevModel before = dev_model(c);
     c->model = *m;
     c->model.msoexp = msoexp;
+    const c3d::DevModel after = dev_model(c);
     drop_stale(c, STALE_PAIR_TARGETS | STALE_PROGRAM);
-    if (c->have_replicas)
+    if (c->have_replicas && (before.noe_pot != after.noe_pot || before.wl != after.wl || before.nleft != after.nleft || before.npad != after.npad ||
+                             before.n != after.n))
         if (int rc = plan_cluster(c)) return rc;
     return targets64 ? build_targets64(c) : C3D_OK;
 }
@@ -1246,6 +1280,7 @@
     DevTmp<unsigned> dnflag;
     const int npartial = 64;
     dev_free(c->buf.tgt); dev_free(c->buf.tgs2);
+    c->ccon_valid = false;
     c->have_targets = false;
     HIP_TRY(hipMalloc(&dIF.p, sizeof(double) * nn));
     HIP_TRY(hipMalloc(&dP.p, sizeof(double) * nn));
@@ -1293,6 +1328,7 @@
             HIP_TRY(hipMemcpyAsync(c->buf.tgt + (size_t)i * c->npad + j, &enc, sizeof(float), hipMemcpyHostToDevice, c->stream));
             HIP_TRY(hipStreamSynchronize(c->stream));
             dev_free(c->buf.tgs2);
+            c->ccon_valid = false;
             ++c->k1_patched;
         }
     }
@@ -1760,6 +1796,8 @@
     else if (!strcmp(key, "step_launches")) *value = (double)c->step_launches;
     else if (!strcmp(key, "resident_launches")) *value = (double)c->resident_launches;
     else if (!strcmp(key, "cluster_launches")) *value = (double)c->cluster_launches;
+    else if (!strcmp(key, "cluster_record_wipes")) *value = (double)c->cluster_record_wipes;
+    else if (!strcmp(key, "cluster_const_builds")) *value = (double)c->cluster_const_builds;
     else if (!strcmp(key, "resident_fallbacks")) *value = (double)c->resident_fallbacks;
     else if (!strcmp(key, "cluster_incomplete")) *value = (double)c->cluster_incomplete;
     else if (!strcmp(key, "spin_completions")) *value = (double)c->spin_completions;
diff --git a/chromosome3d_amd/csrc/c3d_cluster.hip b/chromosome3d_amd/csrc/c3d_cluster.hip
--- a/chromosome3d_amd/csrc/c3d_cluster.hip
+++ b/chromosome3d_amd/csrc/c3d_cluster.hip
@@ -13,7 +13,7 @@
 
 #ifdef C3D_STAMPS
 __device__ unsigned long long g_cstamps[64][8];
-__device__ unsigned long long g_pstamps[8];
+__device__ unsigned long long g_pstamps[16];
 #define CSTAMP(k) do { if (stamper) g_cstamps[s & 63][k] = __builtin_amdgcn_s_memrealtime(); } while (0)
 #define CSTAMP_C(k) do { if (cstamper) g_cstamps[s & 63][k] = __builtin_amdgcn_s_memrealtime(); } while (0)
 #else
@@ -23,10 +23,12 @@
 
 template <int POT, int RPW, int NB, int WL, bool LATE, bool TWO>
 __device__ __forceinline__ void cluster_body(
-    const float* __restrict__ tgt, unsigned* __restrict__ claim, const StepRun* __restrict__ runs, const int P, const int CW, const int NH,
+    const float* __restrict__ tgt, unsigned* __restrict__ claim, const StepRun* __restrict__ runs, const int geom, const int nrep_g,
     const int static_place, const int nbeads, const int run0, const int skip0, const int nsteps,
     const unsigned tag_base, u32x4* __restrict__ rec, volatile unsigned* __restrict__ timeout, const unsigned expected,
-    const AnnealIO& io, const DevModel& m, const DevFire& fp) {
+    const float* __restrict__ traw_g, const AnnealIO& io, const DevModel& m, const DevFire& fp) {
+    const int P = geom & 0xff, CW = (geom >> 8) & 0xff, NH = (geom >> 16) & 0xff;
+    constexpr bool PRE = cluster_preencoded(POT, RPW);
     constexpr int NPAD = 256 * NB;
     constexpr int MAXT = NPAD / 8;
     constexpr int KUMAX = NB > 2 ? 3 : 2;
@@ -69,8 +71,25 @@
     const int cwave = wave - NH;
     const int wg_row0 = part * RW;
     const int row0 = wg_row0 + cwave * RPW;
+    if (lxcd < 0 || lxcd >= nxcd || lrep >= nrep_g) return;
     const StepRun first_run = runs[run0];
-    float4 traw[RPW][NB];
+    float4 pre[PRE ? RPW / 2 : 1][NB][2];
+    float4 traw[PRE ? 1 : RPW][NB];
+    if constexpr (PRE) {
+#pragma unroll
+        for (int q = 0; q < RPW / 2; ++q)
+#pragma unroll
+            for (int jb = 0; jb < NB; ++jb) {
+                float4 a = make_float4(0, 0, 0, 0), b = a;
+                if (is_compute) {
+                    const int gq = min((row0 >> 1) + q, (nbeads - 1) >> 1);
+                    const float4* src = reinterpret_cast<const float4*>(tgt + (((size_t)gq * NB + jb) * 64 + lane) * 8);
+                    a = src[0];
+                    if (jb < NB - 1 || WL > 2) b = src[1];
+                }
+                pre[q][jb][0] = a; pre[q][jb][1] = b;
+            }
+    } else {
 #pragma unroll
     for (int r = 0; r < RPW; ++r)
 #pragma unroll
@@ -90,7 +109,7 @@
             }
             traw[r][jb] = t;
         }
-    if (lxcd < 0 || lxcd >= nxcd || lrep >= m.nrep_g) return;
+    }
     const int rep = m.rep_base + lrep;
     const bool solo = P == 1;
     if (!is_compute) __builtin_amdgcn_s_setprio(3);
@@ -130,7 +149,7 @@
             const int k = 8 * (wave - 1) + 8 * (NH - 1) * q + (lane >> 3), c = lane & 7;
             float b = 0.0f, a = 0.0f;
             if (k < RW && c < m.nleft && wg_row0 + k < m.n) {
-                const float t = tgt[(size_t)(wg_row0 + k) * NPAD + m.jl0 + c];
+                const float t = traw_g[(size_t)(wg_row0 + k) * NPAD + m.jl0 + c];
                 b = t * m.inv_rs;
                 a = t > 0.0f ? m.inv_rs : 0.0f;
             }
@@ -147,12 +166,26 @@
 #ifdef C3D_STAMPS
     asm volatile("s_waitcnt lgkmcnt(0)" ::: "memory");
     const unsigned long long t_coords = __builtin_amdgcn_s_memrealtime();
+#endif
+#ifdef C3D_STAMPS
+    const unsigned long long t_left = __builtin_amdgcn_s_memrealtime();
+    asm volatile("s_waitcnt vmcnt(0)" ::: "memory");
+    const unsigned long long t_traw = __builtin_amdgcn_s_memrealtime();
 #endif
     constexpr bool PK = POT == 4;
     float4 tv[PK ? 1 : RPW][NB];
     PairConsts2<PK ? RPW : 1, NB> pc;
     float4* const mw = reinterpret_cast<float4*>(dump + 8) + (size_t)(is_compute ? cwave : 0) * (RPW * NB * 64);
-    if constexpr (PK) {
+    if constexpr (PRE) {
+#pragma unroll
+        for (int q = 0; q < RPW / 2; ++q)
+#pragma unroll
+            for (int jb = 0; jb < NB; ++jb) {
+                const float4 a = pre[q][jb][0], b = pre[q][jb][1];
+                pc.p[q][jb][0] = float2v{a.x, a.y}; pc.p[q][jb][1] = float2v{a.z, a.w};
+                pc.p[q][jb][2] = float2v{b.x, b.y}; pc.p[q][jb][3] = float2v{b.z, b.w};
+            }
+    } else if constexpr (PK) {
         pair_consts2_build<RPW, NB>(m, traw, is_compute, lane, pc, mw);
     } else {
         DevStep p0{};
@@ -189,7 +222,11 @@
     const bool stamper = lrep == 0 && part == 0 && is_h0 && lane == 0;
     const bool cstamper = lrep == 0 && part == 0 && cwave == 0 && lane == 0;
     if (stamper) { g_pstamps[0] = t_entry; g_pstamps[1] = __builtin_amdgcn_s_memrealtime(); g_pstamps[6] = t_placed; }
-    if (cstamper) { g_pstamps[4] = t_targets; g_pstamps[5] = t_coords; }
+    if (cstamper) { g_pstamps[4] = t_targets; g_pstamps[5] = t_coords; g_pstamps[8] = t_traw; }
+    const bool lstamper = lrep == 0 && part == 0 && cwave == CW - 1 && lane == 0;
+    const bool hstamper = lrep == 0 && part == 0 && wave == 1 && lane == 0;
+    if (lstamper) { g_pstamps[9] = t_traw; g_pstamps[10] = t_targets; }
+    if (hstamper) g_pstamps[12] = t_left;
 #endif
     auto role_loop = [&](auto role) {
     constexpr int ROLE = decltype(role)::value;
@@ -203,6 +240,8 @@
       for (int it = run == run0 ? skip0 : 0; it < count; ++it, ++s) {
 #ifdef C3D_STAMPS
         if (cstamper && s == 0) g_pstamps[7] = __builtin_amdgcn_s_memrealtime();
+        if (lstamper && s == 0) g_pstamps[11] = __builtin_amdgcn_s_memrealtime();
+        if (hstamper && s == 0) g_pstamps[13] = __builtin_amdgcn_s_memrealtime();
 #endif
         __syncthreads();
         CSTAMP(0);
@@ -420,10 +459,11 @@
 }
 
 #define C3D_CLUSTER_ARGS                                                                                                                  \
-    const float* __restrict__ tgt, unsigned* __restrict__ claim, const StepRun* __restrict__ runs, const int P, const int CW, const int NH, \
+    const float* __restrict__ tgt, unsigned* __restrict__ claim, const StepRun* __restrict__ runs, const int geom, const int nrep_g,       \
     const int static_place, const int nbeads, const int run0, const int skip0, const int nsteps, const unsigned tag_base,                 \
-    u32x4* __restrict__ rec, volatile unsigned* __restrict__ timeout, const unsigned expected, const AnnealIO io, const DevModel m, const DevFire fp
-#define C3D_CLUSTER_PASS tgt, claim, runs, P, CW, NH, static_place, nbeads, run0, skip0, nsteps, tag_base, rec, timeout, expected, io, m, fp
+    u32x4* __restrict__ rec, volatile unsigned* __restrict__ timeout, const unsigned expected, const float* __restrict__ traw_g,          \
+    const AnnealIO io, const DevModel m, const DevFire fp
+#define C3D_CLUSTER_PASS tgt, claim, runs, geom, nrep_g, static_place, nbeads, run0, skip0, nsteps, tag_base, rec, timeout, expected, traw_g, io, m, fp
 template <int POT, int RPW, int NB, int WL, bool LATE>
 __global__ __launch_bounds__(kClMaxThreads) void k_cluster(C3D_CLUSTER_ARGS) { cluster_body<POT, RPW, NB, WL, LATE, false>(C3D_CLUSTER_PASS); }
 template <int POT, int RPW, int NB, int WL, bool LATE>
@@ -435,7 +475,7 @@
 #ifndef C3D_CLUSTER_POT
 #ifdef C3D_STAMPS
 hipError_t read_cluster_stamps(unsigned long long* out) { return hipMemcpyFromSymbol(out, HIP_SYMBOL(g_cstamps), sizeof(unsigned long long) * 64 * 8); }
-hipError_t read_cluster_pstamps(unsigned long long* out) { return hipMemcpyFromSymbol(out, HIP_SYMBOL(g_pstamps), sizeof(unsigned long long) * 8); }
+hipError_t read_cluster_pstamps(unsigned long long* out) { return hipMemcpyFromSymbol(out, HIP_SYMBOL(g_pstamps), sizeof(unsigned long long) * 16); }
 #endif
 
 __global__ __launch_bounds__(kClMaxThreads) void k_tear16(u32x4* buf, unsigned* stop, unsigned long long* stats, int iters) {
@@ -519,7 +559,7 @@
 #endif
 
 template <int POT, int RPW, int NB, int WL, bool LATE>
-static hipError_t cluster_go(const DevModel& m, const DevFire& fp, const ClusterPlan& pl, const AnnealIO& io, const float* tgt, void* rec,
+static hipError_t cluster_go(const DevModel& m, const DevFire& fp, const ClusterPlan& pl, const AnnealIO& io, const float* tgt, const float* pcon, void* rec,
                              const StepRun* runs, int run0, int skip0, int nsteps, unsigned tag_base, unsigned* timeout, unsigned* claim,
                              hipStream_t s) {
 #if defined(C3D_CLUSTER_TP)
@@ -532,14 +572,20 @@
     const int tp = pl.two_point ? 1 : 0;
     if ((tp && !kHasTp) || (!tp && !kHasLean)) return hipErrorInvalidValue;
     const int sp = (pl.static_place & 0xff) | ((pl.xcd_base & 0xff) << 8) | ((pl.xcd_count & 0xff) << 16);
+    const int geom = (pl.parts & 0xff) | ((pl.cw & 0xff) << 8) | ((pl.helpers & 0xff) << 16);
+    const float* src = tgt;
+    if constexpr (cluster_preencoded(POT, RPW)) {
+        if (!pcon) return hipErrorInvalidValue;
+        src = pcon;
+    }
 #define C3D_CL_LAUNCH(K)                                                                                                                              \
     do {                                                                                                                                              \
         if (pl.t0 && pl.t1)                                                                                                                           \
-            hipExtLaunchKernelGGL((K<POT, RPW, NB, WL, LATE>), dim3(pl.grid), dim3(pl.threads), pl.lds, s, pl.t0, pl.t1, 0, tgt, claim, runs,          \
-                                  pl.parts, pl.cw, pl.helpers, sp, m.n, run0, skip0, nsteps, tag_base, reinterpret_cast<u32x4*>(rec), timeout, pl.expected, io, m, fp); \
+            hipExtLaunchKernelGGL((K<POT, RPW, NB, WL, LATE>), dim3(pl.grid), dim3(pl.threads), pl.lds, s, pl.t0, pl.t1, 0, src, claim, runs,          \
+                                  geom, m.nrep_g, sp, m.n, run0, skip0, nsteps, tag_base, reinterpret_cast<u32x4*>(rec), timeout, pl.expected, tgt, io, m, fp); \
         else                                                                                                                                          \
-            hipLaunchKernelGGL((K<POT, RPW, NB, WL, LATE>), dim3(pl.grid), dim3(pl.threads), pl.lds, s, tgt, claim, runs, pl.parts, pl.cw, pl.helpers, \
-                               sp, m.n, run0, skip0, nsteps, tag_base, reinterpret_cast<u32x4*>(rec), timeout, pl.expected, io, m, fp);                \
+            hipLaunchKernelGGL((K<POT, RPW, NB, WL, LATE>), dim3(pl.grid), dim3(pl.threads), pl.lds, s, src, claim, runs, geom, m.nrep_g,           \
+                               sp, m.n, run0, skip0, nsteps, tag_base, reinterpret_cast<u32x4*>(rec), timeout, pl.expected, tgt, io, m, fp);           \
     } while (0)
     if constexpr (kHasTp) { if (tp) C3D_CL_LAUNCH(k_cluster_tp); }
     if constexpr (kHasLean) { if (!tp) C3D_CL_LAUNCH(k_cluster); }
@@ -562,13 +608,13 @@
     widths(int_c<4>{}, int_c<1>{}); widths(int_c<4>{}, int_c<2>{});
 }
 template <int POT>
-static hipError_t cluster_geom(const DevModel& m, const DevFire& fp, const ClusterPlan& pl, const AnnealIO& io, const float* tgt, void* rec,
+static hipError_t cluster_geom(const DevModel& m, const DevFire& fp, const ClusterPlan& pl, const AnnealIO& io, const float* tgt, const float* pcon, void* rec,
                                const StepRun* runs, int run0, int skip0, int nsteps, unsigned tag_base, unsigned* timeout, unsigned* claim,
                                hipStream_t s) {
     hipError_t e = hipErrorInvalidValue;
     for_each_cluster_form<POT>([&](auto R, auto B, auto W, auto L) {
         if (pl.rpw == R && m.npad == 256 * B && m.wl == W && (pl.late_tiles != 0) == L)
-            e = cluster_go<POT, R, B, W, L>(m, fp, pl, io, tgt, rec, runs, run0, skip0, nsteps, tag_base, timeout, claim, s);
+            e = cluster_go<POT, R, B, W, L>(m, fp, pl, io, tgt, pcon, rec, runs, run0, skip0, nsteps, tag_base, timeout, claim, s);
     });
     return e;
 }
@@ -588,21 +634,21 @@
 #define C3D_CL_CAT2(a, b) a##b
 #define C3D_CL_CAT(a, b) C3D_CL_CAT2(a, b)
 #if defined(C3D_CLUSTER_POT) && defined(C3D_CLUSTER_TP)
-hipError_t C3D_CL_CAT(launch_cluster_tp_pot, C3D_CLUSTER_POT)(const DevModel& m, const DevFire& fp, const ClusterPlan& pl, const AnnealIO& io, const float* tgt, void* rec,
+hipError_t C3D_CL_CAT(launch_cluster_tp_pot, C3D_CLUSTER_POT)(const DevModel& m, const DevFire& fp, const ClusterPlan& pl, const AnnealIO& io, const float* tgt, const float* pcon, void* rec,
                           const StepRun* runs, int run0, int skip0, int nsteps, unsigned tag_base, unsigned* timeout, unsigned* claim,
                           hipStream_t s) {
-    return cluster_geom<C3D_CLUSTER_POT>(m, fp, pl, io, tgt, rec, runs, run0, skip0, nsteps, tag_base, timeout, claim, s);
+    return cluster_geom<C3D_CLUSTER_POT>(m, fp, pl, io, tgt, pcon, rec, runs, run0, skip0, nsteps, tag_base, timeout, claim, s);
 }
 hipError_t C3D_CL_CAT(preload_cluster_tp_pot, C3D_CLUSTER_POT)() { return cluster_prepare_unit<C3D_CLUSTER_POT, true>(); }
 #elif defined(C3D_CLUSTER_POT)
-hipError_t C3D_CL_CAT(launch_cluster_pot, C3D_CLUSTER_POT)(const DevModel& m, const DevFire& fp, const ClusterPlan& pl, const AnnealIO& io, const float* tgt, void* rec,
+hipError_t C3D_CL_CAT(launch_cluster_pot, C3D_CLUSTER_POT)(const DevModel& m, const DevFire& fp, const ClusterPlan& pl, const AnnealIO& io, const float* tgt, const float* pcon, void* rec,
                           const StepRun* runs, int run0, int skip0, int nsteps, unsigned tag_base, unsigned* timeout, unsigned* claim,
                           hipStream_t s) {
-    return cluster_geom<C3D_CLUSTER_POT>(m, fp, pl, io, tgt, rec, runs, run0, skip0, nsteps, tag_base, timeout, claim, s);
+    return cluster_geom<C3D_CLUSTER_POT>(m, fp, pl, io, tgt, pcon, rec, runs, run0, skip0, nsteps, tag_base, timeout, claim, s);
 }
 hipError_t C3D_CL_CAT(preload_cluster_pot, C3D_CLUSTER_POT)() { return cluster_prepare_unit<C3D_CLUSTER_POT, false>(); }
 #else
-using ClusterLaunch = hipError_t(const DevModel& m, const DevFire& fp, const ClusterPlan& pl, const AnnealIO& io, const float* tgt, void* rec,
+using ClusterLaunch = hipError_t(const DevModel& m, const DevFire& fp, const ClusterPlan& pl, const AnnealIO& io, const float* tgt, const float* pcon, void* rec,
                                  const StepRun* runs, int run0, int skip0, int nsteps, unsigned tag_base, unsigned* timeout, unsigned* claim,
                                  hipStream_t s);
 #if defined(C3D_CLUSTER_SPLIT)
@@ -615,13 +661,13 @@
 static hipError_t (*const kClusterPreload[2][5])() = {{preload_cluster_pot0, preload_cluster_pot1, preload_cluster_pot2, preload_cluster_pot3, preload_cluster_pot4},
                                                       {preload_cluster_tp_pot0, preload_cluster_tp_pot1, preload_cluster_tp_pot2, preload_cluster_tp_pot3, preload_cluster_tp_pot4}};
 #endif
-hipError_t launch_cluster(const DevModel& m, const DevFire& fp, const ClusterPlan& pl, const AnnealIO& io, const float* tgt, void* rec,
+hipError_t launch_cluster(const DevModel& m, const DevFire& fp, const ClusterPlan& pl, const AnnealIO& io, const float* tgt, const float* pcon, void* rec,
                           const StepRun* runs, int run0, int skip0, int nsteps, unsigned tag_base, unsigned* timeout, unsigned* claim,
                           hipStream_t s) {
 #if defined(C3D_CLUSTER_SPLIT)
-    return kClusterLaunch[pl.two_point][device_pot(m.noe_pot)](m, fp, pl, io, tgt, rec, runs, run0, skip0, nsteps, tag_base, timeout, claim, s);
+    return kClusterLaunch[pl.two_point][device_pot(m.noe_pot)](m, fp, pl, io, tgt, pcon, rec, runs, run0, skip0, nsteps, tag_base, timeout, claim, s);
 #else
-    return with_pot(m.noe_pot, [&](auto POT) { return cluster_geom<POT>(m, fp, pl, io, tgt, rec, runs, run0, skip0, nsteps, tag_base, timeout, claim, s); });
+    return with_pot(m.noe_pot, [&](auto POT) { return cluster_geom<POT>(m, fp, pl, io, tgt, pcon, rec, runs, run0, skip0, nsteps, tag_base, timeout, claim, s); });
 #endif
 }
 
diff --git a/chromosome3d_amd/csrc/c3d_device.hip b/chromosome3d_amd/csrc/c3d_device.hip
--- a/chromosome3d_amd/csrc/c3d_device.hip
+++ b/chromosome3d_amd/csrc/c3d_device.hip
@@ -50,14 +50,22 @@
 hipError_t read_stamps(unsigned long long* out) { return hipMemcpyFromSymbol(out, HIP_SYMBOL(g_stamps), sizeof(unsigned long long) * 16); }
 #endif
 
-__global__ __launch_bounds__(256) void k_pair_targets(int n, int npad, float inv_rs, const float* __restrict__ tgt, float* __restrict__ tgs2) {
+__global__ __launch_bounds__(256) void k_pair_targets(int n, int npad, int wl, float inv_rs, const float* __restrict__ tgt, float* __restrict__ tgs2) {
     const int nblk = npad >> 8, npairs = (n + 1) / 2;
     const size_t idx = (size_t)blockIdx.x * 256 + threadIdx.x;
     if (idx >= (size_t)npairs * nblk * 64) return;
     const int lane = (int)(idx & 63), jb = (int)((idx >> 6) % nblk), q = (int)((idx >> 6) / nblk);
     const int ra = min(2 * q, n - 1), rb = min(2 * q + 1, n - 1);
-    const float4 a = *reinterpret_cast<const float4*>(tgt + (size_t)ra * npad + 256 * jb + 4 * lane);
-    const float4 b = *reinterpret_cast<const float4*>(tgt + (size_t)rb * npad + 256 * jb + 4 * lane);
+    const int width = jb == nblk - 1 ? wl : 4;
+    const float* pa = tgt + (size_t)ra * npad + 256 * jb + width * lane;
+    const float* pb = tgt + (size_t)rb * npad + 256 * jb + width * lane;
+    float4 a = make_float4(0, 0, 0, 0), b = a;
+    if (width == 4) { a = *reinterpret_cast<const float4*>(pa); b = *reinterpret_cast<const float4*>(pb); }
+    else {
+        a.x = pa[0]; b.x = pb[0];
+        if (width > 1) { a.y = pa[1]; b.y = pb[1]; }
+        if (width > 2) { a.z = pa[2]; b.z = pb[2]; }
+    }
     auto enc = [inv_rs](float t) { return t > 0.0f ? t * inv_rs : 1e30f; };
     float4* out = reinterpret_cast<float4*>(tgs2 + idx * 8);
     out[0] = make_float4(enc(a.x), enc(b.x), enc(a.y), enc(b.y));
@@ -66,7 +74,7 @@
 size_t pair_targets_floats(int n, int npad) { return (size_t)((n + 1) / 2) * (npad >> 8) * 64 * 8; }
 hipError_t launch_pair_targets(const DevModel& m, const float* tgt, float* tgs2, hipStream_t s) {
     const size_t items = (size_t)((m.n + 1) / 2) * (m.npad >> 8) * 64;
-    hipLaunchKernelGGL(k_pair_targets, dim3((unsigned)((items + 255) / 256)), dim3(256), 0, s, m.n, m.npad, m.inv_rs, tgt, tgs2);
+    hipLaunchKernelGGL(k_pair_targets, dim3((unsigned)((items + 255) / 256)), dim3(256), 0, s, m.n, m.npad, m.wl, m.inv_rs, tgt, tgs2);
     return hipGetLastError();
 }
 
diff --git a/chromosome3d_amd/csrc/c3d_internal.h b/chromosome3d_amd/csrc/c3d_internal.h
--- a/chromosome3d_amd/csrc/c3d_internal.h
+++ b/chromosome3d_amd/csrc/c3d_internal.h
@@ -171,7 +171,15 @@
 };
 bool cluster_plan(const DevModel& m, int num_cus, int num_xcc, int forced_geom, int forced_late, int xcd_count, ClusterPlan* plan);
 size_t cluster_record_bytes(const DevModel& m, const ClusterPlan& pl);
-hipError_t launch_cluster(const DevModel& m, const DevFire& fp, const ClusterPlan& pl, const AnnealIO& io, const float* tgt, void* rec,
+#ifndef C3D_CLUSTER_PREENC
+#if defined(C3D_PAIR_NONE_AS_FAR) && !C3D_PAIR_NONE_AS_FAR
+#define C3D_CLUSTER_PREENC 0
+#else
+#define C3D_CLUSTER_PREENC 1
+#endif
+#endif
+constexpr bool cluster_preencoded(int pot, int rpw) { return C3D_CLUSTER_PREENC && pot == 4 && (rpw & 1) == 0; }
+hipError_t launch_cluster(const DevModel& m, const DevFire& fp, const ClusterPlan& pl, const AnnealIO& io, const float* tgt, const float* pcon, void* rec,
                           const StepRun* runs, int run0, int skip0, int nsteps, unsigned tag_base, unsigned* timeout,
                           unsigned* claim, hipStream_t s);
 hipError_t preload_device_unit();
```

Measured after the change: 4.519 million. -2.7%, worse.
